# crowsonkb/style_transfer2

Hardware: AMD Instinct MI355X
Metric: style-transfer iters/sec @1024px VGG19 (higher is better)
Workload: dtype f32; 1 GPU; configs[1]: 1024x1024 single image per GPU, VGG19 to conv5_1, content conv4_2 + 5 style layers, adam fp32, 500 iterations per image; jobs=1, parallelism=independent jobs, 1 per GPU, no collective (replicas)

## Files before the change

style_transfer2_amd/csrc/engine.cpp:

```cpp
#include "engine.h"

#include <atomic>

namespace st2e {
static thread_local char g_err[1024] = "";
int fail(int code, const char* fmt, ...)
{
    va_list ap;
    va_start(ap, fmt);
    vsnprintf(g_err, sizeof g_err, fmt, ap);
    va_end(ap);
    return code;
}
const char* const kProfNames[P_COUNT] = {"conv3x3_fwd_mfma_f32", "conv3x3_dgrad_mfma_f32", "maxpool_fwd", "maxpool_bwd",
                                          "gram_partial_mfma_f32", "gram_reduce", "style_grad_mfma_f32", "layer_elem",
                                          "image_pass", "finalize", "vector_ops", "misc", "conv3x3_fwd_wino_f32", "conv3x3_dgrad_wino_f32",
                                          "conv3x3_fwd_mfma_bf16", "conv3x3_dgrad_mfma_bf16", "tile_comm",
                                          "gram_partial_mfma_bf16", "style_grad_mfma_bf16", "conv3x3_fwd_wino_split_bf16x6", "conv3x3_dgrad_wino_split_bf16x6",
                                          "style_grad_fused_in_conv_dgrad_bf16", "avepool_fwd", "avepool_bwd",
                                          "gram_partial_split_bf16x6", "style_grad_split_bf16x6", "avepool_bwd_map16"};

static const struct { int kind; const char* name; int cin, cout; } kVgg19[] = {
    {0, "conv1_1", 3, 64}, {0, "conv1_2", 64, 64}, {1, "pool1", 0, 0},
    {0, "conv2_1", 64, 128}, {0, "conv2_2", 128, 128}, {1, "pool2", 0, 0},
// ... 142 lines not shown
            }
            if (r.pack16) ST_TRY(pack16(c, a.data[i], a.data16[i], C, hw));
            break;
        }
        case F_BY_CONV_BELOW:
            break;
        case F_AVEPOOL: {
            if (!plan[i - 1].out32) return fail(ST_ERR_STATE, "internal: the input blob of average pool %s is not materialised", L.name.c_str());
            ProfScope ps(c, P_AVEPOOL_FWD, 0, 4.0 * n_in + (r.out32 ? 4.0 * C * hw : 0.0) + (r.out16 ? 2.0 * act16_elems(C, hw) : 0.0));
            HIP_TRY(launch_avepool_fwd(a.data[i - 1], r.out32 ? a.data[i] : nullptr, r.out16 ? a.data16[i] : nullptr, C, a.h[i - 1], a.w[i - 1], c->stream));
            break;
        }
        case F_MAXPOOL: {
            { ProfScope ps(c, P_POOL_FWD, 0, 4.0 * n_in * 1.25);
              HIP_TRY(launch_maxpool_fwd(a.data[i - 1], a.data[i], C, a.h[i - 1], a.w[i - 1], c->stream)); }
            if (r.pack16) ST_TRY(pack16(c, a.data[i], a.data16[i], C, hw));
            break;
        }
        case F_NONE:
            return fail(ST_ERR_STATE, "internal: no route for layer %s", L.name.c_str());
        }
    }
    a.valid_to = last;
    return ST_OK;
}

int backward_chain(st_ctx* c, int top, const float* top_diff, const std::vector<const float*>& inj, const float** out, bool lean)
{
    ActSet& a = c->act;
    plan_backward(c, a, top, inj, c->sf_w, lean, a.plan.bwd);
    const std::vector<FwdRoute>& fwd = a.plan.fwd;
    const float* cur = top_diff;
    const unsigned short* cur16 = nullptr;
    if (c->bf16 && !c->diff16A) {
        const size_t cap = c->max_blob + 8 * (size_t)a.h[0] * a.w[0];
        ST_TRY(c->diff16A.alloc(cap)); ST_TRY(c->diff16B.alloc(cap));
    }
    for (int i = top; i >= 1; --i) {
        const Layer& L = c->topo[i - 1];
        const BwdRoute& r = a.plan.bwd[i];
        const int below = i - 1;
        const int Cb = a.C[below], Hb = a.h[below], Wb = a.w[below];
        const int H = a.h[i], W = a.w[i];
        const size_t hw = (size_t)H * W;
        const double px = (double)hw, n_below = (double)Cb * Hb * Wb;
        float* dst = (cur == c->diffA) ? c->diffB : c->diffA;
        const float* inject = inj[below];
        if (r.in16 ? !(cur16 || cur) : !cur) return fail(ST_ERR_STATE, "internal: no %s diff above %s", r.in16 ? "bf16 or fp32" : "fp32", L.name.c_str());
        if (r.pack_in16) {
            unsigned short* tmp16 = (cur16 == c->diff16A) ? c->diff16B : c->diff16A;
            ST_TRY(pack16(c, cur, tmp16, a.C[i], hw));
            cur16 = tmp16;
        }
        unsigned short* dst16 = (cur16 == c->diff16A) ? c->diff16B : c->diff16A;
        if ((r.mask == MASK_F32 || r.kind == B_POOL_CLASSIC) && !fwd[below].out32)
            return fail(ST_ERR_STATE, "internal: blob %d, which the backward of %s reads, is not materialised in fp32", below, L.name.c_str());
        const unsigned char* unpool_amap = r.unpool ? a.amap[i + 1] : nullptr;
        const bool unpool_ave = r.unpool && fwd[i + 1].amap == AMAP_BLOCKED16_AVE;
        const double conv_flops = 2.0 * 9 * L.cin * L.cout * px;
        switch (r.kind) {
        case B_SMALLM16: {
            ProfScope ps(c, P_CONV_DGRAD, conv_flops, px * (2.0 * L.cout + 4.0 * L.cin));
            HIP_TRY(launch_conv3x3_dgrad_smallM16(cur16, L.w_raw_r, dst, inject, L.cout, L.cin, H, W, c->stream));
            break;
        }
        case B_SMALLM: {
            ProfScope ps(c, P_CONV_DGRAD, conv_flops, 4.0 * px * (L.cin + L.cout));
            HIP_TRY(launch_conv3x3_dgrad_smallM(cur, L.w_raw, dst, inject, L.cout, L.cin, H, W, c->stream));
            break;
        }
        case B_CONV16: {
            Conv16Problem p{};
            p.in16 = cur16; p.wpack16 = L.w16_bwd; p.bias = nullptr;
            p.out = r.out32 ? dst : nullptr; p.out16 = r.out16 ? dst16 : nullptr;
            p.inject = inject;
            if (r.mask == MASK_F32) p.mask_src = a.data[below];
            if (r.mask == MASK_BF16) p.mask16 = a.data16[below];
            if (r.mask == MASK_BITS) p.mask_bits = a.bits[below];
            if (r.style) {
                p.s_in16 = c->sf_in[below]; p.s_wpack16 = c->sf_w[below];
                prof_note(c, P_STYLE_FUSED_BF16, 2.0 * L.cin * L.cin * px);
            }
            p.K = L.cout; p.M = L.cin; p.MPad = conv_mpad(L.cin); p.H = H; p.W = W; p.relu = 0;
            p.unpool_amap = unpool_amap;
            p.unpool_ave = unpool_ave;
            const double mask_bytes = r.mask == MASK_BITS ? 0.125 : r.mask == MASK_BF16 ? 2.0 : r.mask == MASK_F32 ? 4.0 : 0.0;
            ProfScope ps(c, P_CONV_DGRAD_BF16, conv_flops,
                         px * ((r.unpool ? 0.75 : 2.0) * L.cout + (r.style ? 2.0 : 0.0) * L.cin + (r.out32 ? 4.0 : 0.0) * L.cin + (r.out16 ? 2.0 : 0.0) * L.cin + mask_bytes * L.cin));
            HIP_TRY(launch_conv3x3_bf16(p, c->stream));
            break;
        }
        case B_WINO: case B_WINO_SPLIT: case B_DIRECT: {
            ConvProblem p{};
            p.in = cur; p.wpack = L.w_bwd; p.bias = nullptr; p.out = dst;
            p.mask_src = r.mask == MASK_F32 ? a.data[below] : nullptr; p.inject = inject;
            p.K = L.cout; p.M = L.cin; p.MPad = conv_mpad(L.cin); p.H = H; p.W = W; p.relu = 0;
            p.unpool_amap = unpool_amap;
            ProfScope ps(c, r.kind == B_WINO_SPLIT ? P_CONV_DGRAD_WSPLIT : r.kind == B_WINO ? P_CONV_DGRAD_WINO : P_CONV_DGRAD, conv_flops,
                         4.0 * px * (L.cin + (r.unpool ? 0.3125 : 1.0) * L.cout));
            if (r.kind == B_WINO_SPLIT) { p.wpack = reinterpret_cast<const float*>(L.us_bwd.get()); ST_TRY(wino_scratch(c, p, wino_split_resolve(p.K, p.M, H, W).splits)); HIP_TRY(launch_conv3x3_wino_split(p, c->stream)); }
            else if (r.kind == B_WINO) { p.wpack = L.u_bwd; ST_TRY(wino_scratch(c, p, wino_resolve(p.K, p.M, H, W).splits)); HIP_TRY(launch_conv3x3_wino(p, c->stream)); }
            else HIP_TRY(launch_conv3x3(p, c->stream));
            break;
        }
        case B_AVEPOOL: {
            ProfScope ps(c, P_AVEPOOL_BWD, 0, 4.0 * (double)Cb * H * W +
                         n_below * (4.0 * ((r.mask != MASK_NONE ? 1 : 0) + (inject ? 1 : 0) + (r.out32 ? 1 : 0)) + (r.out16 ? 2.0 : 0.0)));
            HIP_TRY(launch_avepool_bwd(cur, r.mask != MASK_NONE ? a.data[below] : nullptr, inject, r.out32 ? dst : nullptr, r.out16 ? dst16 : nullptr, Cb, Hb, Wb, c->stream));
            break;
        }
        case B_POOL_IDX16: {
            ProfScope ps(c, P_POOL_BWD, 0, (double)Cb * (hw * 3.0 + (size_t)Hb * Wb * 2.0));
            HIP_TRY(launch_maxpool_bwd_idx16(cur16, a.amap[i], dst16, Cb, Hb, Wb, c->stream));
            break;
        }
        case B_AVEPOOL_MAP16: {
            if (fwd[i].amap != AMAP_BLOCKED16_AVE) return fail(ST_ERR_STATE, "internal: the forward of %s wrote no sign map", L.name.c_str());
            ProfScope ps(c, P_AVEPOOL_BWD_MAP16, 0, (double)Cb * (hw * 3.0 + (size_t)Hb * Wb * 2.0));
            HIP_TRY(launch_avepool_bwd_map16(cur16, a.amap[i], dst16, Cb, Hb, Wb, c->stream));
            break;
        }
        case B_POOL_AMAP: {
            ProfScope ps(c, P_POOL_BWD, 0, (double)Cb * (px * 5.0 + (double)Hb * Wb * 4.0));
            HIP_TRY(launch_maxpool_bwd_amap(cur, a.amap[i], dst, Cb, Hb, Wb, c->stream));
            break;
        }
        case B_POOL_CLASSIC: {
            ProfScope ps(c, P_POOL_BWD, 0, 4.0 * n_below * 2.25);
            HIP_TRY(launch_maxpool_bwd(cur, a.data[below], dst, inject, r.mask != MASK_NONE, Cb, Hb, Wb, c->stream));
            break;
        }
        case B_IN_DGRAD_BELOW:
            continue;
        case B_NONE:
            return fail(ST_ERR_STATE, "internal: no route for the backward of layer %s", L.name.c_str());
        }
        cur = r.out32 ? dst : nullptr;
        cur16 = r.out16 ? dst16 : nullptr;
    }
    if (!cur) return fail(ST_ERR_STATE, "internal: the backward chain ended without an fp32 image gradient");
    *out = cur;
    return ST_OK;
}

int ensure_input_buffers(st_ctx* c, int H, int W)
{
    if (c->H == H && c->W == W && c->x[0]) return ST_OK;
    c->act.valid_to = -1;
    if (c->lt.any) { c->lt.any = false; c->lt.resized = true; }
    const size_t n3 = (size_t)3 * H * W;
    for (int i = 0; i < 2; ++i) ST_TRY(c->x[i].alloc(n3));
    ST_TRY(c->grad.alloc(n3));
    c->m.reset(); c->v.reset();
    ST_TRY(c->m.alloc(n3)); ST_TRY(c->v.alloc(n3));
    c->g_cur.reset(); c->pvec.reset();
    for (int i = 0; i <= st_ctx::kCorr; ++i) { c->hs[i].reset(); c->hy[i].reset(); }
    ST_TRY(c->hwc_dev.alloc(n3));
    c->avg.reset(); c->avg_items = 0;
    if (c->avg_decay > 0) ST_TRY(c->avg.alloc(n3));
    c->H = H; c->W = W; c->cur = 0;
    for (auto& p : c->inject) p.reset();
    std::fill(c->inject_roi_zero.begin(), c->inject_roi_zero.end(), 0);
    c->diffA.reset(); c->diffB.reset(); c->stmp.reset(); c->diff16A.reset(); c->diff16B.reset();
    std::vector<int> C, h, w;
    shapes_for(c, H, W, C, h, w);
    c->max_blob = 0;
    for (int i = 0; i < c->nb; ++i) c->max_blob = std::max(c->max_blob, (size_t)C[i] * h[i] * w[i]);
    return ST_OK;
}

int stage_upload(st_ctx* c, const void* host, size_t bytes)
{
    ST_TRY(c->stage_dev.reserve(bytes));
    HIP_TRY(hipMemcpyAsync(c->stage_dev, host, bytes, hipMemcpyHostToDevice, c->stream));
    return ST_OK;
}

int preprocess_into(st_ctx* c, const void* hwc, int H, int W, int is_u8, float* dst)
{
    if (!hwc || H <= 0 || W <= 0) return fail(ST_ERR_ARG, "bad image (%p, %d x %d)", hwc, H, W);
    const size_t n = (size_t)H * W * 3;
    ST_TRY(stage_upload(c, hwc, n * (is_u8 ? 1 : 4)));
    ProfScope ps(c, P_MISC, 0, 0);
    if (is_u8) HIP_TRY(launch_preprocess_u8(c->stage_dev, dst, H, W, c->stream));
    else HIP_TRY(launch_preprocess_f32((const float*)c->stage_dev.get(), dst, H, W, c->stream));
    return ST_OK;
}

void iterate_overwritten(st_ctx* c)
{
    if (!c->act.data.empty() && c->act.data[0] && (c->act.data[0] == c->x[0] || c->act.data[0] == c->x[1])) c->act.valid_to = -1;
}

int set_input_common(st_ctx* c, int H, int W)
{
    const bool reshaped = !(c->H == H && c->W == W && c->x[0]);
    ST_TRY(ensure_input_buffers(c, H, W));
    if (reshaped) {
        c->m_zero = c->v_zero = true;
        c->lb_clear = true;
        c->have_cur = false;
    }
    return ST_OK;
}
int content_from_device(st_ctx* c, const float* xdev, int H, int W)
{
    ST_TRY(act_ensure(c, c->act, H, W));
    std::vector<char> used(c->nb, 0);
    int deepest = -1;
    for (const ActiveLayer& al : c->active) if (al.c) { used[al.blob] = 1; deepest = std::max(deepest, al.blob); }
    if (deepest > 0) ST_TRY(forward_range(c, c->act, xdev, deepest));
    for (int i = 0; i < c->nb; ++i) {
        if (!used[i]) { c->content_feat[i].reset(); continue; }
        const size_t n = (size_t)c->act.C[i] * c->act.h[i] * c->act.w[i];
        if (c->cH != H || c->cW != W || !c->content_feat[i]) ST_TRY(c->content_feat[i].alloc(n));
        HIP_TRY(hipMemcpyAsync(c->content_feat[i], i == 0 ? xdev : c->act.data[i], n * sizeof(float), hipMemcpyDeviceToDevice, c->stream));
    }
    c->act.valid_to = -1;
    if (xdev != c->content_x) {
        if (c->cH != H || c->cW != W || !c->content_x) ST_TRY(c->content_x.alloc((size_t)3 * H * W));
        HIP_TRY(hipMemcpyAsync(c->content_x, xdev, (size_t)3 * H * W * sizeof(float), hipMemcpyDeviceToDevice, c->stream));
    }
    c->cH = H; c->cW = W;
    c->have_content = true;
    HIP_TRY(hipStreamSynchronize(c->stream));
    return ST_OK;
}

int ensure_content_features(st_ctx* c)
{
    int need = -1;
    for (const ActiveLayer& al : c->active) if (al.c && !c->content_feat[al.blob]) need = std::max(need, al.blob);
    if (need < 0) return ST_OK;
    if (!c->have_content || !c->content_x) return fail(ST_ERR_STATE, "content image missing");
    ST_TRY(act_ensure(c, c->act, c->cH, c->cW));
    if (need > 0) ST_TRY(forward_range(c, c->act, c->content_x, need));
    for (const ActiveLayer& al : c->active) {
        const int b = al.blob;
        if (!al.c || c->content_feat[b]) continue;
        const size_t n = (size_t)c->act.C[b] * c->act.h[b] * c->act.w[b];
        ST_TRY(c->content_feat[b].alloc(n));
        HIP_TRY(hipMemcpyAsync(c->content_feat[b], b == 0 ? c->content_x : c->act.data[b], n * sizeof(float), hipMemcpyDeviceToDevice, c->stream));
    }
    c->act.valid_to = -1;
    return ST_OK;
}
}

extern "C" const char* st_last_error(void) { return st2e::g_err; }

extern "C" {

int st_create(st_ctx** out, int device_id, const st_layer_desc* layers, int n_layers)
{
    if (!out) return fail(ST_ERR_ARG, "out is NULL");
    int ndev = 0;
    HIP_TRY(hipGetDeviceCount(&ndev));
    if (ndev <= 0) return fail(ST_ERR_HIP, "no HIP device visible");
    if (device_id < 0 || device_id >= ndev) return fail(ST_ERR_ARG, "device %d out of range (%d visible)", device_id, ndev);
    HIP_TRY(hipSetDevice(device_id));
    std::unique_ptr<st_ctx, int (*)(st_ctx*)> c(new st_ctx(), st_destroy);
    c->device = device_id;
    c->wino = env_int("ST2_WINO", c->wino) != 0;
    c->graphs = env_int("ST2_GRAPH", c->graphs) != 0;
    { const size_t side = (size_t)env_int("ST2_GRAPH_MAX_PX", 768); c->graph_max_px = side * side; }
    if (n_layers <= 0) {
        for (const auto& l : kVgg19) {
            Layer L; L.is_conv = l.kind == 0; L.name = l.name; L.cin = l.cin; L.cout = l.cout;
            c->topo.push_back(std::move(L));
        }
    } else {
        int cprev = 3;
        for (int i = 0; i < n_layers; ++i) {
            const int kind = layers[i].kind;
            if (kind != ST_LAYER_CONV && kind != ST_LAYER_POOL && kind != ST_LAYER_AVEPOOL)
                return fail(ST_ERR_ARG, "layer %d (%s): unknown kind %d", i, layers[i].name ? layers[i].name : "", kind);
            Layer L; L.is_conv = kind == ST_LAYER_CONV; L.ave = kind == ST_LAYER_AVEPOOL; L.name = layers[i].name ? layers[i].name : "";
            if (L.is_conv) {
                L.cin = layers[i].cin; L.cout = layers[i].cout;
                if (L.cin != cprev || L.cout <= 0) return fail(ST_ERR_ARG, "layer %s: cin %d does not follow %d", L.name.c_str(), L.cin, cprev);
                cprev = L.cout;
            }
            c->topo.push_back(std::move(L));
        }
    }
    if ((int)c->topo.size() + 1 > kMaxTraceLayers) return fail(ST_ERR_ARG, "too many layers");
    c->blob_names.push_back("data");
    for (const Layer& L : c->topo) c->blob_names.push_back(L.name);
    c->nb = (int)c->blob_names.size();
    HIP_TRY(hipStreamCreate(&c->stream));
    c->content_feat.resize(c->nb);
    c->style_gram.resize(c->nb);
    c->style_valid.assign(c->nb, 0);
    c->inject.resize(c->nb);
    c->inject_roi_zero.assign(c->nb, 0);
    c->layer_part.resize(c->nb);
    c->s2_part.resize(c->nb);
    c->sfuse_w.resize(c->nb);
    c->cnt.assign(c->nb * 6, 0);
    c->norm_valid.assign(c->nb * 3, 0);
    ST_TRY(c->norms.alloc(c->nb * 3));
    ST_TRY(c->image_part.alloc(6 * kMaxPartials));
    ST_TRY(c->trace_dev.alloc(kMaxTraceLayers * 6 + 8));
    ST_TRY(c->trace_sums.alloc(kMaxTraceLayers * kLayerSlots + kImageSlots));
    ST_TRY(c->lb_dev.alloc(1));
    HIP_TRY(hipMemset(c->lb_dev, 0, sizeof(LbfgsDev)));
    ST_TRY(c->lb_part.alloc(4 * kMaxPartials));
    ST_TRY(c->trace_host.alloc(kMaxTraceLayers * 6 + 8));
    for (int b = 0; b < c->nb; ++b) c->rows.push_back(ActiveLayer{b, 1.f, 1.f, 1.f, true, true, true});
    c->active = c->rows;
    *out = c.release();
    return ST_OK;
}

int st_destroy(st_ctx* c)
{
    if (!c) return ST_OK;
    (void)hipSetDevice(c->device);
    if (c->stream) (void)hipStreamSynchronize(c->stream);
    if (c->pipe.copy) (void)hipStreamSynchronize(c->pipe.copy);
    for (int i = 0; i < 2; ++i) if (c->gexec[i]) (void)hipGraphExecDestroy(c->gexec[i]);
    for (int i = 0; i < st_ctx::Pipe::kSlots; ++i) {
        if (c->pipe.ready[i]) (void)hipEventDestroy(c->pipe.ready[i]);
        if (c->pipe.done[i]) (void)hipEventDestroy(c->pipe.done[i]);
    }
    for (hipEvent_t e : c->ev_pool) (void)hipEventDestroy(e);
    comm_free(c);
    const hipStream_t stream = c->stream, copy = c->pipe.copy;
    delete c;
    if (copy) (void)hipStreamDestroy(copy);
    if (stream) (void)hipStreamDestroy(stream);
    return ST_OK;
}

static int make_split_packs(Layer& L, const float* w)
{
    for (int dir = 0; dir < 2; ++dir) {
        const int K = dir ? L.cout : L.cin, M = dir ? L.cin : L.cout;
        DevBuf<unsigned short>& dst = dir ? L.us_bwd : L.us_fwd;
        if (dst || !wino_split_resolve(K, M, 4, 4).ok) continue;
        std::vector<unsigned short> hu(wino_split_pack_elems(K, M), 0);
        if (dir) pack_wino_split_weights_dgrad(w, L.cout, L.cin, hu.data()); else pack_wino_split_weights_fwd(w, L.cout, L.cin, hu.data());
        ST_TRY(dst.alloc(hu.size()));
        HIP_TRY(hipMemcpy(dst, hu.data(), hu.size() * 2, hipMemcpyHostToDevice));
    }
    return ST_OK;
}

int st_load_conv_weights(st_ctx* c, const char* layer, const float* w, const float* bias)
{
    if (c) c->epoch++;
    if (!c || !layer || !w) return fail(ST_ERR_ARG, "NULL argument");
    HIP_TRY(hipSetDevice(c->device));
    for (Layer& L : c->topo) {
        if (!L.is_conv || L.name != layer) continue;
        const size_t nf = conv_pack_floats(L.cin, L.cout), nb = conv_pack_floats(L.cout, L.cin);
        std::vector<float> pf(nf), pb(nb), bp(conv_mpad(L.cout), 0.f);
        pack_conv_weights_fwd(w, L.cout, L.cin, pf.data());
        pack_conv_weights_dgrad(w, L.cout, L.cin, pb.data());
        if (bias) memcpy(bp.data(), bias, L.cout * sizeof(float));
        L.loaded = false;
        static_cast<LayerPacks&>(L) = LayerPacks{};
        for (int dir = 0; dir < 2; ++dir) {
            const int K = dir ? L.cout : L.cin, M = dir ? L.cin : L.cout;
            if (!wino_resolve(K, M, 4, 4).ok) continue;
            std::vector<float> hu(wino_pack_floats(K, M));
            if (dir) pack_wino_weights_dgrad(w, L.cout, L.cin, hu.data()); else pack_wino_weights_fwd(w, L.cout, L.cin, hu.data());
            DevBuf<float>& dst = dir ? L.u_bwd : L.u_fwd;
            ST_TRY(dst.alloc(hu.size()));
            HIP_TRY(hipMemcpy(dst, hu.data(), hu.size() * sizeof(float), hipMemcpyHostToDevice));
        }
        {
            const size_t n16f = conv16_pack_elems(L.cin, L.cout), n16b = conv16_pack_elems(L.cout, L.cin);
            std::vector<unsigned short> hf(n16f), hb(n16b);
            pack_conv_weights16_fwd(w, L.cout, L.cin, hf.data());
            pack_conv_weights16_dgrad(w, L.cout, L.cin, hb.data());
            ST_TRY(L.w16_fwd.alloc(n16f)); ST_TRY(L.w16_bwd.alloc(n16b));
            HIP_TRY(hipMemcpy(L.w16_fwd, hf.data(), n16f * 2, hipMemcpyHostToDevice));
            HIP_TRY(hipMemcpy(L.w16_bwd, hb.data(), n16b * 2, hipMemcpyHostToDevice));
        }
        if (L.cin == 3 && L.cout % 32 == 0) {
            std::vector<unsigned short> hs(conv_first_split_pack_elems(L.cout));
            pack_conv_first_split(w, bias, L.cout, L.cin, hs.data());
            ST_TRY(L.w_split.alloc(hs.size()));
            HIP_TRY(hipMemcpy(L.w_split, hs.data(), hs.size() * 2, hipMemcpyHostToDevice));
        }
        ST_TRY(L.w_fwd.alloc(nf)); ST_TRY(L.w_bwd.alloc(nb));
        ST_TRY(L.w_raw.alloc((size_t)L.cout * L.cin * 9)); ST_TRY(L.bias.alloc(bp.size()));
        HIP_TRY(hipMemcpy(L.w_fwd, pf.data(), nf * sizeof(float), hipMemcpyHostToDevice));
        HIP_TRY(hipMemcpy(L.w_bwd, pb.data(), nb * sizeof(float), hipMemcpyHostToDevice));
        HIP_TRY(hipMemcpy(L.w_raw, w, (size_t)L.cout * L.cin * 9 * sizeof(float), hipMemcpyHostToDevice));
        if (conv_dgrad_smallM_ok(L.cout, L.cin) && L.cout % 8 == 0) {
            std::vector<float> wr((size_t)L.cout * L.cin * 9);
            for (size_t k = 0; k < wr.size(); ++k) {
                unsigned u; memcpy(&u, &w[k], 4);
                u = (u + 0x7fffu + ((u >> 16) & 1u)) & 0xffff0000u;
                memcpy(&wr[k], &u, 4);
            }
            ST_TRY(L.w_raw_r.alloc(wr.size()));
            HIP_TRY(hipMemcpy(L.w_raw_r, wr.data(), wr.size() * sizeof(float), hipMemcpyHostToDevice));
        }
        HIP_TRY(hipMemcpy(L.bias, bp.data(), bp.size() * sizeof(float), hipMemcpyHostToDevice));
        if (c->wino_split) ST_TRY(make_split_packs(L, w));
        L.loaded = true;
        return ST_OK;
    }
    return fail(ST_ERR_ARG, "no conv layer named %s", layer);
}

int st_set_conv_algo(st_ctx* c, int winograd)
{
    if (c) c->epoch++;
    if (!c) return fail(ST_ERR_ARG, "ctx is NULL");
    if (winograd < 0 || winograd > 2) return fail(ST_ERR_ARG, "conv algorithm %d: 0 direct, 1 Winograd (fp32 matrix cores), 2 split-operand Winograd (bf16 matrix cores, fp32 results)", winograd);
    c->wino = winograd != 0;
    c->wino_split = winograd == 2;
    if (c->wino_split) {
        HIP_TRY(hipSetDevice(c->device));
        for (Layer& L : c->topo) {
            if (!L.is_conv || !L.loaded || !L.w_raw) continue;
            std::vector<float> w((size_t)L.cout * L.cin * 9);
            HIP_TRY(hipMemcpy(w.data(), L.w_raw, w.size() * sizeof(float), hipMemcpyDeviceToHost));
            ST_TRY(make_split_packs(L, w.data()));
        }
    }
    return ST_OK;
}

int st_set_gram_algo(st_ctx* c, int algo)
{
    if (!c) return fail(ST_ERR_ARG, "ctx is NULL");
    if (algo != 0 && algo != 1) return fail(ST_ERR_ARG, "gram algorithm %d: 0 fp32 matrix cores, 1 split operands (bf16 matrix cores, fp32 results)", algo);
    if (algo == 1) {
        std::vector<int> C, h, w;
        shapes_for(c, 16, 16, C, h, w);
        size_t need = 0;
        for (int i = 0; i < c->nb; ++i) need = std::max(need, style_split_scratch(C[i], 4));
        if (need > c->dsplit.cap()) {
            HIP_TRY(hipSetDevice(c->device));
            DevBuf<unsigned short> p;
            ST_TRY(p.alloc(need));
            HIP_TRY(hipStreamSynchronize(c->stream));
            c->dsplit = std::move(p);
        }
    }
    c->epoch++;
    c->gram_split = algo == 1;
    return ST_OK;
}

int st_set_pool_algo(st_ctx* c, int algo)
{
    if (!c) return fail(ST_ERR_ARG, "ctx is NULL");
    if (algo != 0 && algo != 1) return fail(ST_ERR_ARG, "pool algorithm %d: 0 every average pool a stand-alone pass, 1 fused into the bf16 conv launches around it where a build exists", algo);
    c->epoch++;
    c->pool_algo = algo;
    return ST_OK;
}

int st_get_pool_algo(st_ctx* c, int* algo)
{
    if (!c || !algo) return fail(ST_ERR_ARG, "NULL argument");
    *algo = c->pool_algo;
    return ST_OK;
}

int st_get_algos(st_ctx* c, int* conv, int* gram)
{
    if (!c) return fail(ST_ERR_ARG, "ctx is NULL");
    if (conv) *conv = c->wino_split ? 2 : c->wino ? 1 : 0;
    if (gram) *gram = c->gram_split ? 1 : 0;
    return ST_OK;
}

int st_set_precision(st_ctx* c, int bf16_features)
{
    if (c) c->epoch++;
    if (!c) return fail(ST_ERR_ARG, "ctx is NULL");
    c->bf16 = bf16_features != 0;
    c->lean = bf16_features == 1 && !env_off("ST2_BF16_LEAN");
    return ST_OK;
}

int st_num_blobs(st_ctx* c) { return c ? c->nb : 0; }
const char* st_blob_name(st_ctx* c, int i) { return (c && i >= 0 && i < c->nb) ? c->blob_names[i].c_str() : nullptr; }

int st_blob_shape(st_ctx* c, int index, int H, int W, int* oc, int* oh, int* ow)
{
    if (!c || index < 0 || index >= c->nb) return fail(ST_ERR_ARG, "bad blob index %d", index);
    std::vector<int> C, h, w;
    shapes_for(c, H, W, C, h, w);
    if (oc) *oc = C[index];
    if (oh) *oh = h[index];
    if (ow) *ow = w[index];
    return ST_OK;
}

int st_forward(st_ctx* c, const float* x_nchw, int H, int W, int last_blob)
{
    if (c) c->epoch++;
    if (!c || !x_nchw || H <= 0 || W <= 0) return fail(ST_ERR_ARG, "bad argument");
    HIP_TRY(hipSetDevice(c->device));
    ST_TRY(set_input_common(c, H, W));
    ST_TRY(act_ensure(c, c->act, H, W));
    const size_t n3 = (size_t)3 * H * W;
    ST_TRY(c->fwd_x.reserve(n3));
    HIP_TRY(hipMemcpyAsync(c->fwd_x, x_nchw, n3 * sizeof(float), hipMemcpyHostToDevice, c->stream));
    if (last_blob < 0 || last_blob >= c->nb) last_blob = c->nb - 1;
    ST_TRY(forward_range(c, c->act, c->fwd_x, last_blob));
    HIP_TRY(hipStreamSynchronize(c->stream));
    return ST_OK;
}

int st_get_blob(st_ctx* c, int index, float* out)
{
    if (!c || index < 0 || index >= c->nb || !out) return fail(ST_ERR_ARG, "bad argument");
    if (index > c->act.valid_to) return fail(ST_ERR_STATE, "blob %d was not computed by the last forward", index);
    if (!c->act.plan.fwd[index].out32) return fail(ST_ERR_STATE, "blob %d (%s) is not materialised in fp32 by the lean evaluation of an iteration (st_opfunc / st_forward write every fp32 blob; bf16: st_set_precision(ctx, 2))", index, c->blob_names[index].c_str());
    const size_t n = (size_t)c->act.C[index] * c->act.h[index] * c->act.w[index];
    HIP_TRY(hipMemcpy(out, c->act.data[index], n * sizeof(float), hipMemcpyDeviceToHost));
    return ST_OK;
}

int st_backward(st_ctx* c, int n, const int* blob_index, const float* const* diffs, float* out_grad)
{
    if (c) c->epoch++;
    if (!c || !out_grad || n < 0) return fail(ST_ERR_ARG, "bad argument");
    if (c->act.valid_to < 0) return fail(ST_ERR_STATE, "st_forward first");
    HIP_TRY(hipSetDevice(c->device));
    const size_t n3 = (size_t)3 * c->H * c->W;
    std::vector<const float*> inj(c->nb, nullptr);
    int top = -1;
    for (int i = 0; i < n; ++i) {
        const int b = blob_index[i];
        if (b < 0 || b > c->act.valid_to) return fail(ST_ERR_ARG, "diff for blob %d which the last forward did not reach", b);
        const size_t nb = (size_t)c->act.C[b] * c->act.h[b] * c->act.w[b];
        if (!c->inject[b]) ST_TRY(c->inject[b].alloc(nb));
        HIP_TRY(hipMemcpyAsync(c->inject[b], diffs[i], nb * sizeof(float), hipMemcpyHostToDevice, c->stream));
        c->inject_roi_zero[b] = 0;
        if ((int)c->lt.diff.size() == c->nb) c->lt.diff[b] = LT_OVERWRITTEN;
        inj[b] = c->inject[b];
        top = std::max(top, b);
    }
    if (top < 0) { memset(out_grad, 0, n3 * sizeof(float)); return ST_OK; }
    if (!c->diffA) { ST_TRY(c->diffA.alloc(c->max_blob)); ST_TRY(c->diffB.alloc(c->max_blob)); }
    const float* g = inj[0];
    if (top > 0) ST_TRY(backward_chain(c, top, inj[top], inj, &g));
    HIP_TRY(hipMemcpyAsync(out_grad, g, n3 * sizeof(float), hipMemcpyDeviceToHost, c->stream));
    HIP_TRY(hipStreamSynchronize(c->stream));
    return ST_OK;
}

int st_gram(st_ctx* c, int index, float* out)
{
    if (c) c->epoch++;
    if (!c || index < 0 || index >= c->nb || !out) return fail(ST_ERR_ARG, "bad argument");
    if (index > c->act.valid_to) return fail(ST_ERR_STATE, "blob %d was not computed by the last forward", index);
    if (!c->act.plan.fwd[index].out32) return fail(ST_ERR_STATE, "blob %d (%s) is not materialised in fp32 by the lean evaluation of an iteration: no Gram of it (st_opfunc / st_forward write every fp32 blob; bf16: st_set_precision(ctx, 2))", index, c->blob_names[index].c_str());
    HIP_TRY(hipSetDevice(c->device));
    const int C = c->act.C[index], hw = c->act.h[index] * c->act.w[index];
    DevBuf<float> g;
    ST_TRY(g.alloc((size_t)C * C));
    int r = style_gram(c, c->act, style_term(c, c->act, index, nullptr, true), nullptr, g, C, (double)C * hw, nullptr, nullptr);
    if (r == ST_OK) {
        hipError_t e = hipMemcpyAsync(out, g, (size_t)C * C * sizeof(float), hipMemcpyDeviceToHost, c->stream);
        if (e == hipSuccess) e = hipStreamSynchronize(c->stream);
        if (e != hipSuccess) r = fail(ST_ERR_HIP, "gram copy: %s", hipGetErrorString(e));
    }
    return r;
}

int st_set_input(st_ctx* c, const void* hwc, int H, int W, int is_u8)
{
    if (c) c->epoch++;
    if (!c) return fail(ST_ERR_ARG, "ctx is NULL");
    HIP_TRY(hipSetDevice(c->device));
    ST_TRY(set_input_common(c, H, W));
    iterate_overwritten(c);
    c->avg_items = 0;
    ST_TRY(preprocess_into(c, hwc, H, W, is_u8, c->x[c->cur]));
    HIP_TRY(hipStreamSynchronize(c->stream));
    return ST_OK;
}

int st_set_input_nchw(st_ctx* c, const float* x, int H, int W)
{
    if (c) c->epoch++;
    if (!c || !x || H <= 0 || W <= 0) return fail(ST_ERR_ARG, "bad argument");
    HIP_TRY(hipSetDevice(c->device));
    ST_TRY(set_input_common(c, H, W));
    iterate_overwritten(c);
    c->avg_items = 0;
    HIP_TRY(hipMemcpy(c->x[c->cur], x, (size_t)3 * H * W * sizeof(float), hipMemcpyHostToDevice));
    return ST_OK;
}

int st_get_input_nchw(st_ctx* c, float* out)
{
    if (!c || !out || !c->x[0]) return fail(ST_ERR_STATE, "no input image");
    HIP_TRY(hipStreamSynchronize(c->stream));
    HIP_TRY(hipMemcpy(out, c->x[c->cur], (size_t)3 * c->H * c->W * sizeof(float), hipMemcpyDeviceToHost));
    return ST_OK;
}

int st_input_shape(st_ctx* c, int* H, int* W)
{
    if (!c) return fail(ST_ERR_ARG, "ctx is NULL");
// ... 132 lines not shown
```

style_transfer2_amd/csrc/engine.h:

```cpp
#pragma once
#include "../../include/st2.h"
#include "st2_kernels.h"
#include "env.h"
#include "devbuf.h"

#include <hip/hip_runtime.h>
#include <math.h>
#include <stdarg.h>
#include <stdio.h>
#include <string.h>

#include <algorithm>
#include <memory>
#include <string>
#include <vector>

namespace st2e {
using namespace st2;

int fail(int code, const char* fmt, ...);
#define HIP_TRY(expr)                                                                               \
    do {                                                                                            \
        hipError_t e_ = (expr);                                                                     \
        if (e_ != hipSuccess)                                                                       \
            return st2e::fail(ST_ERR_HIP, "%s failed: %s (%s:%d)", #expr, hipGetErrorString(e_), __FILE__, __LINE__); \
    } while (0)
#define ST_TRY(expr)                    \
    do {                                \
        int r_ = (expr);                \
        if (r_ != ST_OK) return r_;     \
    } while (0)

enum ProfClass { P_CONV_FWD, P_CONV_DGRAD, P_POOL_FWD, P_POOL_BWD, P_GRAM, P_GRAM_REDUCE, P_STYLE_GRAD,
                 P_LAYER_ELEM, P_IMAGE_PASS, P_FINALIZE, P_VECTOR, P_MISC, P_CONV_FWD_WINO, P_CONV_DGRAD_WINO,
                 P_CONV_FWD_BF16, P_CONV_DGRAD_BF16, P_COMM, P_GRAM_BF16, P_STYLE_GRAD_BF16, P_CONV_FWD_WSPLIT, P_CONV_DGRAD_WSPLIT, P_STYLE_FUSED_BF16,
                 P_AVEPOOL_FWD, P_AVEPOOL_BWD, P_GRAM_SPLIT, P_STYLE_GRAD_SPLIT, P_AVEPOOL_BWD_MAP16, P_COUNT };
extern const char* const kProfNames[P_COUNT];
struct ProfRec { int cls; hipEvent_t a, b; double flops, bytes; };

struct LayerPacks {
    DevBuf<float> w_fwd, w_bwd, w_raw, w_raw_r, bias;
    DevBuf<unsigned short> w16_fwd, w16_bwd;
    DevBuf<unsigned short> w_split;
    DevBuf<float> u_fwd, u_bwd;
    DevBuf<unsigned short> us_fwd, us_bwd;
};
struct Layer : LayerPacks {
    bool is_conv = false;
    bool ave = false;
    std::string name;
    int cin = 0, cout = 0;
    bool loaded = false;
};

enum FwdKind : unsigned char { F_NONE, F_CONV16, F_WINO, F_WINO_SPLIT, F_DIRECT, F_FIRST_SPLIT, F_MAXPOOL, F_AVEPOOL,
                               F_BY_CONV_BELOW };
enum AmapLayout : unsigned char { AMAP_NONE, AMAP_BLOCKED16,
                                  AMAP_PLANAR32,
                                  AMAP_BLOCKED16_AVE };
enum BwdKind : unsigned char { B_NONE, B_SMALLM, B_SMALLM16, B_CONV16, B_WINO, B_WINO_SPLIT, B_DIRECT, B_AVEPOOL, B_POOL_IDX16,
                               B_POOL_AMAP, B_POOL_CLASSIC,
                               B_IN_DGRAD_BELOW,
                               B_AVEPOOL_MAP16 };
enum MaskSrc : unsigned char { MASK_NONE, MASK_F32, MASK_BF16, MASK_BITS };

struct FwdRoute {
    FwdKind kind = F_NONE;
    bool out32 = false, out16 = false, bits = false;
    AmapLayout amap = AMAP_NONE;
    bool pack16 = false;
    bool pools_next = false;
    bool style16 = false;
    bool style_all16 = false;
};
struct BwdRoute {
    BwdKind kind = B_NONE;
    bool in16 = false;
    bool pack_in16 = false;
    bool out32 = false, out16 = false;
    MaskSrc mask = MASK_NONE;
    bool unpool = false;
    bool style = false;
};
struct RoutePlan { std::vector<FwdRoute> fwd; std::vector<BwdRoute> bwd; };

struct ActSet {
    int H = 0, W = 0;
    std::vector<int> C, h, w;
    std::vector<DevBuf<float>> own;
    std::vector<float*> data;
    std::vector<DevBuf<unsigned short>> data16;
    std::vector<DevBuf<unsigned char>> amap;
    std::vector<DevBuf<unsigned short>> bits;
    RoutePlan plan;
    int valid_to = -1;
};

struct ActiveLayer { int blob; float cw, sw, dw; bool c, s, d; };

inline bool nonzero(float w) { return fabsf(w) > 1e-15f; }

struct TileGeom { int gH = 0, gW = 0, wy0 = 0, wx0 = 0, ty0 = 0, tx0 = 0, ty1 = 0, tx1 = 0; };
struct BlobRoi { int y0, x0, y1, x1; double n_global; };
struct BlobSize { int h, w, stride; double n; };

struct ObjTerm {
    ActiveLayer al; int b, C;
    size_t n;
    double n_norm;
    BlobRoi roi; bool has_roi;
    size_t sums;
    size_t gram;
    int k;
    const BlobRoi* region() const { return has_roi ? &roi : nullptr; }
};
constexpr size_t kNoSlot = ~(size_t)0;
struct ObjTerms { std::vector<ObjTerm> t; int last = -1; size_t n1 = 0; int n_style = 0; };

struct StyleShape { bool grad16, gram16; };
enum StyleOps : unsigned char { OPS_F32, OPS_SPLIT, OPS_BF16,
                                OPS_FUSED };
struct StyleLaunch { StyleOps ops; int cls; double flops, bytes; };
struct StyleTerm {
    int b, C, hw;
    bool roi; GramRoi groi; PixRoi proi;
    StyleLaunch gram, grad, pack;
    GramPlan plan;
    int slots;
    size_t d16, sfuse;
    bool reads32, reads16, missing32;
    bool book;
};

enum LtDiff : char { LT_NONE, LT_WRITTEN, LT_RODE_ON_CONV, LT_OVERWRITTEN };
struct LayerTerms {
    bool any = false;
    bool resized = false;
    int style_blob = -1;
    int raw_blob = -1;
    std::vector<size_t> n;
    std::vector<int> C;
    std::vector<char> diff;
    std::vector<char> norm_ok;
    void begin(int nb) { any = resized = false; style_blob = raw_blob = -1; n.assign(nb, 0); C.assign(nb, 0); diff.assign(nb, LT_NONE); norm_ok.assign((size_t)nb * 3, 0); }
};
}

using namespace st2e;

struct st_ctx {
    int device = 0;
    hipStream_t stream = nullptr;
    bool bf16 = false;
    bool lean = false;
    bool in_step = false;
    bool wino = true;
    bool wino_split = false;
    int pool_algo = 0;
    bool gram_split = false;
    DevBuf<unsigned short> dsplit;
    DevBuf<unsigned short> diff16A, diff16B;
    std::vector<Layer> topo;
    std::vector<std::string> blob_names;
    int nb = 0;

    ActSet act;
    int H = 0, W = 0;
    DevBuf<float> x[2];
    int cur = 0;
    DevBuf<float> fwd_x;
    DevBuf<float> grad;
    int cH = 0, cW = 0;
    std::vector<DevBuf<float>> content_feat;
    DevBuf<float> content_x;
    std::vector<DevBuf<float>> style_gram;
    std::vector<char> style_valid;
    bool have_content = false, have_style = false;
    std::vector<ActiveLayer> rows;
    std::vector<ActiveLayer> active;
    float tv_w = 1, tv_pow = 1, p_w = 1, p_pow = 1;
    DevBuf<float> norms;
    std::vector<char> norm_valid;
    std::vector<DevBuf<float>> inject;
    std::vector<char> inject_roi_zero;
    DevBuf<float> diffA, diffB, stmp;
    size_t max_blob = 0;
    DevBuf<float> gram_slabs, gram_fold, dbuf;
    DevBuf<unsigned short> d16;
    std::vector<DevBuf<unsigned short>> sfuse_w;
    std::vector<const unsigned short*> sf_in, sf_w;
    LayerTerms lt;
    DevBuf<float> conv_scratch;
    unsigned long long epoch = 0;
    hipGraphExec_t gexec[2] = {nullptr, nullptr};
    unsigned long long gepoch[2] = {0, 0};
    DevBuf<float> adam_dyn;
    bool capturing = false, graphs = false;
    int plain_steps = 0;
    unsigned long long plain_epoch = ~0ull;
    size_t graph_max_px = 768 * 768;
    long long graph_replays = 0;
    std::vector<DevBuf<float>> layer_part;
    std::vector<DevBuf<float>> s2_part;
    std::vector<int> cnt;
    DevBuf<float> image_part;
    int image_cnt = 0;
    DevBuf<float> trace_dev;
    DevBuf<double> trace_sums;
    PinBuf<float> trace_host;
    int trace_len_last = 8;
    DevBuf<float> hwc_dev;
    struct Pipe {
        static constexpr int kSlots = 6;
        hipStream_t copy = nullptr;
        DevBuf<float> hwc[kSlots]; float* img_pin[kSlots] = {}; PinBuf<float> trace_pin[kSlots];
        PinBuf<char> pin_base[kSlots];
        hipEvent_t ready[kSlots] = {}, done[kSlots] = {};
        size_t cap = 0; long long head = 0; int count = 0, tlen[kSlots] = {}, H[kSlots] = {}, W[kSlots] = {};
        size_t want_head = 0, want_tail = 0, have_head = 0, have_tail = 0;
        struct Retired { PinBuf<char> buf; long long at; };
        std::vector<Retired> retired;
        long long begins = 0;
    } pipe;
    DevBuf<unsigned char> stage_dev;
    int opt_kind = ST_OPT_NONE;
    double step_size = 1.0;
    DevBuf<float> m, v;
    int items1 = 0, items2 = 0;
    bool m_zero = true, v_zero = true;
    static const int kCorr = kLbfgsCorr;
    DevBuf<float> hs[kLbfgsSlots];
    DevBuf<float> hy[kLbfgsSlots];
    DevBuf<LbfgsDev> lb_dev;
    bool lb_clear = true;
    DevBuf<float> lb_part;
    DevBuf<LbfgsGram> lb_gram;
    DevBuf<float> lb_gpart;
    DevBuf<float> lb_dots;
    bool lb_gram_form = false;
    DevBuf<float> g_cur, pvec;
    bool have_cur = false;
    float last_loss = 0.f;
    DevBuf<float> avg;
    double avg_decay = 0.0;
    int avg_items = 0;
    bool orig_colors = false;
    int style_match = 0;
    float xf_A[9] = {1, 0, 0, 0, 1, 0, 0, 0, 1}, xf_b[3] = {0, 0, 0};
    DevBuf<double> mom_part, mom_out;
    struct Tile : TileGeom {
        bool on = false;
        DevBuf<float> p1, p2, p3, pd;
        bool s2_in_p2 = false;
        bool evaluated = false;
        DevBuf<float> wgrad;
        bool fused = false;
        DevBuf<float> lb_x, lb_sums;
        DevBuf<float> sp; int sp_n = 0, sp_last = -1, sp_gH = 0, sp_gW = 0;
    } tile;
    struct Comm {
        void* lib = nullptr;
        void* comm = nullptr;
        int rank = 0, world = 1;
        bool set = false;
        st_allreduce_fn ar = nullptr; st_exchange_fn ex = nullptr; void* user = nullptr;
        struct Peer { int peer = 0; std::vector<int> send, recv; DevBuf<float> sbuf, rbuf; size_t sn = 0, rn = 0; };
        std::vector<Peer> plan[3];
        bool planned[3] = {false, false, false};
        bool self_via_rccl = false;
        DevBuf<float> ring;
        long long steps = 0;
        std::vector<float> h1, h2, h3, hd, hn;
        DevBuf<float> tile_chw, tile_hwc;
        DevBuf<float> tile_cx;
    } comm;
    bool prof_on = false;
    std::vector<ProfRec> prof;
    std::vector<hipEvent_t> ev_pool;
    size_t ev_used = 0;

    int blob_c(int i) const { return act.C[i]; }
    int blob_c_topo(int i) const
    {
        for (int k = i; k >= 1; --k) if (topo[k - 1].is_conv) return topo[k - 1].cout;
        return 3;
    }
};

namespace st2e {
inline size_t act16_elems(int C, size_t hw) { return (size_t)((C + 7) / 8) * hw * 8; }
inline bool conv16_ok(const st_ctx* c, int K) { (void)c; return K >= 8 && K % 8 == 0; }
int wino_scratch(st_ctx* c, ConvProblem& p, int splits);

struct ProfScope {
    st_ctx* c; int idx = -1;
    ProfScope(st_ctx* ctx, int cls, double flops, double bytes, bool book = true) : c(ctx)
    {
        if (!c->prof_on || !book) return;
        auto get = [&]() {
            if (c->ev_used == c->ev_pool.size()) {
                hipEvent_t e;
                (void)hipEventCreate(&e);
                c->ev_pool.push_back(e);
            }
            return c->ev_pool[c->ev_used++];
        };
        ProfRec r{cls, get(), get(), flops, bytes};
        (void)hipEventRecord(r.a, c->stream);
        c->prof.push_back(r);
        idx = (int)c->prof.size() - 1;
    }
    ~ProfScope()
    {
        if (idx >= 0) (void)hipEventRecord(c->prof[idx].b, c->stream);
    }
};

inline void prof_note(st_ctx* c, int cls, double flops)
{
    if (!c->prof_on) return;
    if (c->ev_used == c->ev_pool.size()) { hipEvent_t e; (void)hipEventCreate(&e); c->ev_pool.push_back(e); }
    hipEvent_t e = c->ev_pool[c->ev_used++];
    (void)hipEventRecord(e, c->stream);
    c->prof.push_back(ProfRec{cls, e, e, flops, 0.0});
}

void shapes_for(const st_ctx* c, int H, int W, std::vector<int>& C, std::vector<int>& h, std::vector<int>& w);
int act_ensure(st_ctx* c, ActSet& a, int H, int W);
int forward_range(st_ctx* c, ActSet& a, const float* x, int last, bool lean = false);
int backward_chain(st_ctx* c, int top, const float* top_diff, const std::vector<const float*>& inj, const float** out, bool lean = false);
int ensure_input_buffers(st_ctx* c, int H, int W);
int stage_upload(st_ctx* c, const void* host, size_t bytes);
int preprocess_into(st_ctx* c, const void* hwc, int H, int W, int is_u8, float* dst);
int set_input_common(st_ctx* c, int H, int W);
void iterate_overwritten(st_ctx* c);
int content_from_device(st_ctx* c, const float* xdev, int H, int W);
int style_from_device(st_ctx* c, const float* xdev, int H, int W);
int ensure_content_features(st_ctx* c);
void plan_forward(const st_ctx* c, const ActSet& a, int last, bool lean, std::vector<FwdRoute>& fwd);
void plan_backward(const st_ctx* c, const ActSet& a, int top, const std::vector<const float*>& inj,
                   const std::vector<const unsigned short*>& fused_w, bool lean, std::vector<BwdRoute>& bwd);
bool lean32_enabled();
StyleShape style_shape(const st_ctx* c, const ActSet& a, int b);
StyleTerm style_term(const st_ctx* c, const ActSet& a, int b, const BlobRoi* roi = nullptr, bool target = false, int fuse_last = -1);
size_t style_split_scratch(int C, int hw);
int style_gram(st_ctx* c, const ActSet& a, const StyleTerm& t, const float* target, float* out, int out_ld, double divisor, float* partial, int* n_partial);
int style_grad(st_ctx* c, const ActSet& a, const StyleTerm& t, float* dst, float c2, int fused, float sw, int accumulate, int* np);
int ensure_dbuf(st_ctx* c);
int ensure_layer_part(st_ctx* c, int b);
LayerElemArgs layer_elem_args(const st_ctx* c, const ActiveLayer& al, double n_norm, int write, float* part, const BlobRoi* roi = nullptr);
int objective_terms(const st_ctx* c, const ActSet& a, const TileGeom* tile, ObjTerms& terms);
BlobSize blob_size(const st_ctx* c, int b, int gH, int gW);
BlobRoi tile_roi(const st_ctx* c, const ActSet& a, const TileGeom& t, int b);
ImagePassArgs image_pass_args(const st_ctx* c, const float* x, const float* scd, float* grad, bool adam, float* x_next);
int eval_objective(st_ctx* c, const float* x, bool want_grad, float* grad_out, bool adam, float* x_next);
int read_trace(st_ctx* c, double* trace, float* loss);
int lbfgs_alloc(st_ctx* c);
LbfgsArgs lbfgs_args(st_ctx* c, int apply);
int lbfgs_clear_history(st_ctx* c, bool gram_form);
float average_corr(const st_ctx* c);
int emit_preflight(const st_ctx* c, int reader, bool want_image, EmitPlan* plan);
int emit_enqueue(st_ctx* c, const EmitPlan& plan, float* hwc, const float* staged_v, const float* staged_cx, int h, int w);
int style_color_check(const st_ctx* c);
int style_recolor_enqueue(st_ctx* c, float* x, int H, int W);
int strips(st_ctx* c, float* tensor, int C, int h, int w, const std::vector<int>& rects, float* buf, int mode);
void comm_free(st_ctx* c);
int comm_allreduce(st_ctx* c, float* buf, int n);
}
```

style_transfer2_amd/csrc/engine_objective.cpp:

```cpp
#include "engine.h"

namespace st2e {
int objective_terms(const st_ctx* c, const ActSet& a, const TileGeom* tile, ObjTerms& terms)
{
    terms = ObjTerms{};
    if (!c->active.empty() && ((int)a.C.size() != c->nb || a.H != c->H || a.W != c->W))
        return fail(ST_ERR_STATE, "no forward of the current input has sized the activations");
    size_t pos = 0;
    for (const ActiveLayer& al : c->active) {
        if (al.c && (!c->have_content || c->cH != c->H || c->cW != c->W))
            return fail(ST_ERR_STATE, "content features missing or of a different size than the input");
        if (al.s && !c->have_style) return fail(ST_ERR_STATE, "style Gram matrices missing");
        if (al.s && !c->style_valid[al.blob])
            return fail(ST_ERR_STATE, "blob %d (%s) carries a style weight but has no style target: the sharded style pass (st_tile_set_style) stopped below it", al.blob, c->blob_names[al.blob].c_str());
        ObjTerm t{};
        t.al = al; t.b = al.blob; t.C = a.C[t.b];
        t.n = (size_t)t.C * a.h[t.b] * a.w[t.b];
        t.has_roi = tile != nullptr;
        t.roi = tile ? tile_roi(c, a, *tile, t.b) : BlobRoi{0, 0, a.h[t.b], a.w[t.b], (double)t.n};
        t.n_norm = t.roi.n_global;
        t.sums = pos;
        pos += 4;
        t.gram = kNoSlot; t.k = -1;
        if (al.s) { t.gram = pos; pos += (size_t)t.C * t.C; t.k = terms.n_style++; }
        terms.last = std::max(terms.last, t.b);
        terms.t.push_back(t);
    }
    terms.n1 = pos;
    return ST_OK;
}

ImagePassArgs image_pass_args(const st_ctx* c, const float* x, const float* scd, float* grad, bool adam, float* x_next)
{
    ImagePassArgs ip{};
    ip.x = x; ip.scd = scd; ip.grad = grad;
    ip.C = 3; ip.H = c->H; ip.W = c->W;
    ip.tv_w = c->tv_w; ip.tv_beta = c->tv_pow; ip.p_w = c->p_w; ip.p_pow = c->p_pow;
    ip.partial = c->image_part;
    if (adam) {
        ip.x_out = x_next; ip.m = c->m; ip.v = c->v;
        ip.d1 = (float)0.9; ip.c1 = (float)(1 - 0.9); ip.d2 = (float)0.999; ip.c2 = (float)(1 - 0.999);
        ip.corr1 = (float)(1 - pow(0.9, c->items1)); ip.corr2 = (float)(1 - pow(0.999, c->items2));
        ip.step = (float)c->step_size;
        ip.m_is_zero = c->m_zero; ip.v_is_zero = c->v_zero;
        if (c->capturing) ip.dyn = c->adam_dyn;
    }
    return ip;
}

int eval_objective(st_ctx* c, const float* x, bool want_grad, float* grad_out, bool adam, float* x_next)
{
    if (!c->x[0]) return fail(ST_ERR_STATE, "no input image");
    ST_TRY(act_ensure(c, c->act, c->H, c->W));
    ActSet& a = c->act;
    ObjTerms terms;
    ST_TRY(objective_terms(c, a, nullptr, terms));
    const int last = std::max(terms.last, 0);
    const bool lean = c->bf16 && c->lean && !c->tile.on;
    bool lean32 = false;
    if (!c->bf16 && c->in_step && !c->tile.on) lean32 = lean32_enabled();
    ST_TRY(ensure_content_features(c));
    ST_TRY(forward_range(c, a, x, last, lean || lean32));

    std::vector<const float*> inj(c->nb, nullptr);
    std::fill(c->cnt.begin(), c->cnt.end(), 0);
    c->sf_in.assign(c->nb, nullptr); c->sf_w.assign(c->nb, nullptr);
    c->lt.begin(c->nb);
    for (const ObjTerm& ot : terms.t) {
        const ActiveLayer& al = ot.al;
        const int b = ot.b, C = ot.C;
        const size_t n = ot.n;
        if (!c->inject[b]) ST_TRY(c->inject[b].alloc(n));
        c->inject_roi_zero[b] = 0;
        ST_TRY(ensure_layer_part(c, b));
        float* part = c->layer_part[b];
        float* nrm = c->norms + b * 3;
        int* cnt = &c->cnt[b * 6];
        bool wrote = false;
        if (al.c || al.d) {
            LayerElemArgs e = layer_elem_args(c, al, (double)n, 1, part);
            const bool need_norm = (al.c && !c->norm_valid[b * 3 + 0]) || (al.d && !c->norm_valid[b * 3 + 2]);
            int np = 0;
            if (need_norm) {
                e.write = 0;
                { ProfScope ps(c, P_LAYER_ELEM, 0, 4.0 * n * (al.c ? 2 : 1)); HIP_TRY(launch_layer_elem(e, &np, c->stream)); }
                ProfScope ps(c, P_FINALIZE, 0, 0);
                if (al.c && !c->norm_valid[b * 3 + 0]) { HIP_TRY(launch_finalize_norm(e.part_gc2, np, (double)n, nrm + 0, c->stream)); c->norm_valid[b * 3 + 0] = 1; }
                if (al.d && !c->norm_valid[b * 3 + 2]) { HIP_TRY(launch_finalize_norm(e.part_gd2, np, (double)n, nrm + 2, c->stream)); c->norm_valid[b * 3 + 2] = 1; }
            }
            e.write = 1;
            { ProfScope ps(c, P_LAYER_ELEM, 0, 4.0 * n * (al.c ? 3 : 2)); HIP_TRY(launch_layer_elem(e, &np, c->stream)); }
            cnt[0] = cnt[1] = cnt[2] = cnt[3] = np;
            wrote = true;
        }
        if (al.s) {
            ST_TRY(ensure_dbuf(c));
            const StyleTerm t = style_term(c, a, b, nullptr, false, want_grad ? last : -1);
            ST_TRY(style_gram(c, a, t, c->style_gram[b], c->dbuf, conv_mpad(C), (double)n, part + 4 * kMaxPartials, &cnt[4]));
            const float c2 = (float)(2.0 / ((double)C * C * (double)n));
            if (c->norm_valid[b * 3 + 1]) {
                ST_TRY(style_grad(c, a, t, c->inject[b], c2, 1, al.sw, wrote, &cnt[5]));
            } else {
                if (!c->stmp) ST_TRY(c->stmp.alloc(c->max_blob));
                ST_TRY(style_grad(c, a, t, c->stmp, c2, 0, al.sw, 0, &cnt[5]));
                { ProfScope ps(c, P_FINALIZE, 0, 0);
                  HIP_TRY(launch_finalize_norm(c->s2_part[b], cnt[5], (double)n, nrm + 1, c->stream)); }
                c->norm_valid[b * 3 + 1] = 1;
                ProfScope ps(c, P_VECTOR, 0, 4.0 * n * 3);
                HIP_TRY(launch_scaled_accumulate(c->stmp, c->inject[b], al.sw, nrm + 1, wrote, n, c->stream));
                c->lt.raw_blob = b;
            }
            c->lt.style_blob = b;
            if (c->lt.raw_blob != b) c->lt.raw_blob = -1;
        }
        c->lt.n[b] = n; c->lt.C[b] = C;
        c->lt.diff[b] = c->sf_w[b] ? LT_RODE_ON_CONV : LT_WRITTEN;
        for (int k = 0; k < 3; ++k) c->lt.norm_ok[b * 3 + k] = c->norm_valid[b * 3 + k];
        inj[b] = (c->sf_w[b] && !wrote) ? nullptr : c->inject[b];
    }

    const float* scd = nullptr;
    if (want_grad && !c->active.empty()) {
        if (!c->diffA) { ST_TRY(c->diffA.alloc(c->max_blob)); ST_TRY(c->diffB.alloc(c->max_blob)); }
        if (last == 0) scd = inj[0];
        else {
            std::vector<const float*> below = inj;
            const int rc = backward_chain(c, last, inj[last], below, &scd, lean);
            c->sf_in.assign(c->nb, nullptr); c->sf_w.assign(c->nb, nullptr);
            ST_TRY(rc);
        }
    }

    {
        const ImagePassArgs ip = image_pass_args(c, x, scd, want_grad ? grad_out : nullptr, adam, x_next);
        const double n3 = 3.0 * c->H * c->W;
        ProfScope ps(c, P_IMAGE_PASS, 0, 4.0 * n3 * (adam ? 7 : 3));
        HIP_TRY(launch_image_pass(ip, &c->image_cnt, c->stream));
    }

    {
        TraceArgs t{};
        t.n_layers = (int)terms.t.size();
        for (int l = 0; l < t.n_layers; ++l) {
            const ActiveLayer& al = terms.t[l].al;
            const int b = al.blob;
            TraceLayer& L = t.layer[l];
            L.content = al.c; L.style = al.s; L.deepdream = al.d;
            L.cw = al.cw; L.sw = al.sw; L.dw = al.dw;
            L.n = (double)terms.t[l].n;
            L.gram_n = (double)a.C[b] * a.C[b];
            for (int k = 0; k < 5; ++k) { L.part[k] = c->layer_part[b] + k * kMaxPartials; L.count[k] = c->cnt[b * 6 + k]; }
            L.part[5] = c->s2_part[b]; L.count[5] = c->cnt[b * 6 + 5];
            L.norm = c->norms + b * 3;
        }
        t.image_part = c->image_part; t.image_count = c->image_cnt; t.image_n = 3.0 * c->H * c->W;
        t.tv_w = c->tv_w; t.p_w = c->p_w; t.p_pow = c->p_pow; t.have_grad = want_grad;
        t.out = c->trace_dev;
        t.sums = c->trace_sums;
        c->trace_len_last = t.n_layers * 6 + 8;
        ProfScope ps(c, P_FINALIZE, 0, 0);
        HIP_TRY(launch_finalize_trace(t, c->stream));
    }
    c->lt.any = true;
    return ST_OK;
}

int read_trace(st_ctx* c, double* trace, float* loss)
{
    const int n = c->trace_len_last;
    HIP_TRY(hipMemcpyAsync(c->trace_host, c->trace_dev, n * sizeof(float), hipMemcpyDeviceToHost, c->stream));
    HIP_TRY(hipStreamSynchronize(c->stream));
    if (trace) for (int i = 0; i < n; ++i) trace[i] = c->trace_host[i];
    c->last_loss = c->trace_host[n - 2];
    if (loss) *loss = c->last_loss;
    return ST_OK;
}
}

extern "C" {

int st_set_weights(st_ctx* c, int n_rows, const int* blob_index, const float* content, const float* style,
                   const float* deepdream, const double params[4])
{
    if (c) c->epoch++;
    if (!c || n_rows < 0 || (n_rows && (!blob_index || !content || !style || !deepdream)) || !params)
        return fail(ST_ERR_ARG, "bad argument");
    std::vector<ActiveLayer> rows;
    for (int i = 0; i < n_rows; ++i) {
        const int b = blob_index[i];
        if (b < 0 || b >= c->nb) return fail(ST_ERR_ARG, "row %d names blob %d", i, b);
        rows.push_back(ActiveLayer{b, content[i], style[i], deepdream[i], nonzero(content[i]), nonzero(style[i]), nonzero(deepdream[i])});
    }
    c->rows = rows;
    c->active.clear();
    for (const ActiveLayer& r : rows) if (r.c || r.s || r.d) c->active.push_back(r);
    c->tile.evaluated = false;
    c->tv_w = (float)params[0]; c->tv_pow = (float)params[1]; c->p_w = (float)params[2]; c->p_pow = (float)params[3];
    if (c->have_content) {
        std::vector<char> used(c->nb, 0);
        for (const ActiveLayer& al : c->active) if (al.c) used[al.blob] = 1;
        HIP_TRY(hipSetDevice(c->device));
        HIP_TRY(hipStreamSynchronize(c->stream));
        for (int b = 0; b < c->nb; ++b) if (!used[b]) c->content_feat[b].reset();
    }
    return ST_OK;
}

int st_clear_norms(st_ctx* c)
{
    if (c) c->epoch++;
    if (!c) return fail(ST_ERR_ARG, "ctx is NULL");
    std::fill(c->norm_valid.begin(), c->norm_valid.end(), 0);
    return ST_OK;
}

int st_get_layer_terms(st_ctx* c, int index, float* D, float* raw_S, float* diff, float norms[3])
{
    if (!c || index < 0 || index >= c->nb) return fail(ST_ERR_ARG, "bad argument");
    const LayerTerms& lt = c->lt;
    const char* name = c->blob_names[index].c_str();
    if (!lt.any)
        return fail(ST_ERR_STATE, lt.resized ? "the iterate was resized after the last evaluation: its work buffers are gone; evaluate again"
                                             : "no objective evaluation has completed on this context");
    if (!lt.n[index]) return fail(ST_ERR_STATE, "blob %d (%s) carried no weight in the last evaluation", index, name);
    if ((D || raw_S) && lt.style_blob != index) {
        if (lt.style_blob < 0) return fail(ST_ERR_STATE, "the last evaluation had no style term: no D and no style gradient of blob %d (%s)", index, name);
        return fail(ST_ERR_STATE, "D and the unscaled style gradient are one buffer each for all layers: they hold those of blob %d (%s), the style layer evaluated last, not of blob %d (%s)",
                    lt.style_blob, c->blob_names[lt.style_blob].c_str(), index, name);
    }
    if (raw_S && lt.raw_blob != index)
        return fail(ST_ERR_STATE, "the last evaluation of blob %d (%s) knew its style norm and scaled the gradient in the kernel's epilogue: the unscaled one exists only after the first evaluation since reset() / st_clear_norms", index, name);
    if (diff && lt.diff[index] == LT_RODE_ON_CONV)
        return fail(ST_ERR_STATE, "the style term of blob %d (%s) rode on the data-gradient conv above it: nothing was written into its diff (ST2_STYLE_FUSE=0, or an evaluation without gradient, materialises it)", index, name);
    if (diff && lt.diff[index] == LT_OVERWRITTEN)
        return fail(ST_ERR_STATE, "st_backward has overwritten the diff of blob %d (%s) since the last evaluation", index, name);
    if (diff && (lt.diff[index] != LT_WRITTEN || !c->inject[index])) return fail(ST_ERR_STATE, "blob %d (%s) has no diff of the last evaluation", index, name);
    if ((D && !c->dbuf) || (raw_S && !c->stmp)) return fail(ST_ERR_STATE, "internal: the buffer of blob %d (%s) is gone", index, name);
    HIP_TRY(hipSetDevice(c->device));
    HIP_TRY(hipStreamSynchronize(c->stream));
    const size_t C = (size_t)lt.C[index], n = lt.n[index];
    if (D) HIP_TRY(hipMemcpy2D(D, C * sizeof(float), c->dbuf, (size_t)conv_mpad((int)C) * sizeof(float), C * sizeof(float), C, hipMemcpyDeviceToHost));
    if (raw_S) HIP_TRY(hipMemcpy(raw_S, c->stmp, n * sizeof(float), hipMemcpyDeviceToHost));
    if (diff) HIP_TRY(hipMemcpy(diff, c->inject[index], n * sizeof(float), hipMemcpyDeviceToHost));
    if (norms) {
        HIP_TRY(hipMemcpy(norms, c->norms + index * 3, 3 * sizeof(float), hipMemcpyDeviceToHost));
        for (int k = 0; k < 3; ++k) if (!lt.norm_ok[index * 3 + k]) norms[k] = 0.f;
    }
    return ST_OK;
}

int st_trace_len(st_ctx* c) { return c ? (int)c->active.size() * 6 + 8 : 0; }

int st_opfunc(st_ctx* c, float* out_loss, float* out_grad, double* trace)
{
    if (c) c->epoch++;
    if (!c) return fail(ST_ERR_ARG, "ctx is NULL");
    HIP_TRY(hipSetDevice(c->device));
    ST_TRY(eval_objective(c, c->x[c->cur], out_grad != nullptr, c->grad, false, nullptr));
    if (out_grad) HIP_TRY(hipMemcpyAsync(out_grad, c->grad, (size_t)3 * c->H * c->W * sizeof(float), hipMemcpyDeviceToHost, c->stream));
    return read_trace(c, trace, out_loss);
}

}
```

style_transfer2_amd/csrc/engine_style.cpp:

```cpp
#include "engine.h"

namespace st2e {
StyleShape style_shape(const st_ctx* c, const ActSet& a, int b)
{
    StyleShape s{};
    if (!c->bf16 || b < 1 || !c->topo[b - 1].is_conv) return s;
    const int C = a.C[b], hw = a.h[b] * a.w[b];
    s.grad16 = conv16_ok(c, C) && style_grad16_ok(C, (size_t)hw);
    s.gram16 = s.grad16 && (c->tile.on ? !env_off("ST2_TILE_STYLE16") : hw % 64 == 0 && gram16_ok(C, hw, gram_plan16(C, hw)));
    return s;
}

size_t style_split_scratch(int C, int hw) { return gram_split_ok(C, hw) && style_grad_split_ok(C, hw) ? style_grad_split_pack_elems(C) : 0; }

static bool style_fuse_ok(const st_ctx* c, const ActSet& a, int b, int last)
{
    if (env_off("ST2_STYLE_FUSE") || b + 1 > last || a.C[b] % 32 != 0) return false;
    const Layer& up = c->topo[b];
    return up.is_conv && up.loaded && conv16_ok(c, up.cout) && up.cin == a.C[b];
}

StyleTerm style_term(const st_ctx* c, const ActSet& a, int b, const BlobRoi* roi, bool target, int fuse_last)
{
    const FwdRoute& fr = a.plan.fwd[b];
    StyleTerm t{};
    const int C = t.C = a.C[b];
    t.b = b; t.roi = roi != nullptr; t.book = target || !roi;
    const size_t plane = (size_t)a.h[b] * a.w[b];
    if (roi) { t.groi = GramRoi{roi->y0, roi->x0, roi->x1 - roi->x0, a.w[b], plane}; t.proi = PixRoi{roi->y0, roi->x0, roi->y1, roi->x1}; }
    const int hw = t.hw = roi ? t.groi.rw * (roi->y1 - roi->y0) : (int)plane;
    const bool may16 = !target && (roi || !c->tile.on);
    const bool gram16 = may16 && fr.style_all16, grad16 = may16 && (roi ? fr.style_all16 : fr.style16);
    const size_t split_elems = style_split_scratch(C, hw);
    const bool split = c->gram_split && !c->bf16 && !c->tile.on && !roi && split_elems > 0;
    const double fl = 2.0 * C * C * (double)hw, n = (double)C * hw;
    t.plan = gram16 ? gram_plan16(C, hw) : gram_plan(C, hw);
    t.gram = gram16 ? StyleLaunch{OPS_BF16, P_GRAM_BF16, fl, 2.0 * C * (double)hw}
             : StyleLaunch{split ? OPS_SPLIT : OPS_F32, split ? P_GRAM_SPLIT : P_GRAM, fl, 4.0 * C * (double)hw};
    if (gram16 && fuse_last >= 0 && c->norm_valid[b * 3 + 1] && style_fuse_ok(c, a, b, fuse_last)) {
        t.sfuse = style_fuse_pack_elems(C, conv_mpad(C));
        t.pack = StyleLaunch{OPS_FUSED, P_MISC, 0, 4.0 * C * C + 2.0 * t.sfuse};
        t.grad = StyleLaunch{OPS_FUSED, P_STYLE_GRAD, 2.0 * C * C * (double)C, 12.0 * C * C};
        t.slots = style_s2_trace_blocks(C);
    } else if (grad16) {
        t.grad = StyleLaunch{OPS_BF16, P_STYLE_GRAD_BF16, fl, n * 6.0};
        t.slots = style_grad16_blocks(C, (size_t)hw);
    } else if (split && split_elems <= c->dsplit.cap()) {
        t.grad = StyleLaunch{OPS_SPLIT, P_STYLE_GRAD_SPLIT, fl, n * 8.0};
        t.slots = style_grad_split_blocks(C, hw);
    } else {
        t.grad = StyleLaunch{OPS_F32, P_STYLE_GRAD, fl, n * 8.0};
        t.slots = style_grad_blocks(C, a.h[b], a.w[b]);
    }
    if (grad16) t.d16 = style_grad16_pack_elems(C);
    t.reads16 = grad16; t.reads32 = !gram16 || !grad16; t.missing32 = t.reads32 && !fr.out32;
    return t;
}

static int missing_copy(const StyleTerm& t) { return fail(ST_ERR_STATE, t.roi ? "internal: style blob %d has no fp32 copy" : "internal: style blob %d has neither an fp32 nor a usable bf16 copy", t.b); }

int style_gram(st_ctx* c, const ActSet& a, const StyleTerm& t, const float* target, float* out, int out_ld, double divisor, float* partial, int* n_partial)
{
    if (t.missing32) return missing_copy(t);
    const int b = t.b, C = t.C;
    const GramRoi* roi = t.roi ? &t.groi : nullptr;
    ST_TRY(c->gram_slabs.reserve(t.plan.slab_floats));
    ST_TRY(c->gram_fold.reserve((size_t)gram_fold_groups(t.plan) * C * C));
    {
        ProfScope ps(c, t.gram.cls, t.gram.flops, t.gram.bytes, t.book);
        if (t.gram.ops == OPS_BF16) HIP_TRY(launch_gram16_partial(a.data16[b], c->gram_slabs, C, t.hw, t.plan, c->stream, roi));
        else if (t.gram.ops == OPS_SPLIT) HIP_TRY(launch_gram_split_partial(a.data[b], c->gram_slabs, C, t.hw, t.plan, c->stream));
        else HIP_TRY(launch_gram_partial(a.data[b], c->gram_slabs, C, t.hw, t.plan, c->stream, roi));
    }
    ProfScope ps(c, P_GRAM_REDUCE, 0, 4.0 * (double)t.plan.slab_floats, t.book);
    HIP_TRY(launch_gram_reduce(c->gram_slabs, c->gram_fold, target, out, out_ld, partial, n_partial, C, divisor, t.plan, c->stream));
    return ST_OK;
}

int style_grad(st_ctx* c, const ActSet& a, const StyleTerm& t, float* dst, float c2, int fused, float sw, int accumulate, int* np)
{
    if (t.missing32) return missing_copy(t);
    const int b = t.b, C = t.C, ld = conv_mpad(C);
    const float* norm = c->norms + b * 3 + 1;
    ST_TRY(c->s2_part[b].reserve(t.slots));
    if (t.d16) ST_TRY(c->d16.reserve(t.d16));
    float* part = c->s2_part[b];
    if (t.grad.ops == OPS_FUSED) {
        ST_TRY(c->sfuse_w[b].reserve(t.sfuse));
        { ProfScope ps(c, t.pack.cls, t.pack.flops, t.pack.bytes, t.book);
          HIP_TRY(launch_style_fuse_pack(c->dbuf, ld, C, ld, c2, sw, norm, c->sfuse_w[b], c->stream)); }
        ProfScope ps(c, t.grad.cls, t.grad.flops, t.grad.bytes, t.book);
        HIP_TRY(launch_style_s2_trace(c->dbuf, ld, c->style_gram[b], C, (double)C * t.hw, c2, part, np, c->stream));
        c->sf_in[b] = a.data16[b]; c->sf_w[b] = c->sfuse_w[b];
        return ST_OK;
    }
    if (t.roi && t.grad.ops == OPS_BF16 && dst == c->inject[b] && !accumulate && !c->inject_roi_zero[b]) {
        HIP_TRY(hipMemsetAsync(dst, 0, (size_t)C * t.groi.plane * sizeof(float), c->stream));
        c->inject_roi_zero[b] = 1;
    }
    ProfScope ps(c, t.grad.cls, t.grad.flops, t.grad.bytes, t.book);
    if (t.grad.ops == OPS_SPLIT) HIP_TRY(launch_style_grad_split(c->dbuf, ld, c->dsplit, a.data[b], dst, c2, fused, sw, norm, accumulate, part, np, C, t.hw, c->stream));
    else if (t.grad.ops == OPS_BF16) HIP_TRY(launch_style_grad16(c->dbuf, ld, c->d16, a.data16[b], dst, c2, fused, sw, norm, accumulate, part, np, C, (size_t)t.hw, c->stream, t.roi ? &t.groi : nullptr));
    else HIP_TRY(launch_style_grad(c->dbuf, a.data[b], dst, c2, fused, sw, norm, accumulate, part, np, C, a.h[b], a.w[b], c->stream, t.roi ? &t.proi : nullptr));
    return ST_OK;
}

int ensure_dbuf(st_ctx* c)
{
    if (c->dbuf) return ST_OK;
    size_t cc = 1;
    for (int i = 0; i < c->nb; ++i) cc = std::max(cc, (size_t)c->act.C[i] * conv_mpad(c->act.C[i]));
    ST_TRY(c->dbuf.alloc(cc));
    HIP_TRY(hipMemsetAsync(c->dbuf, 0, cc * sizeof(float), c->stream));
    return ST_OK;
}

int ensure_layer_part(st_ctx* c, int b) { return c->layer_part[b] ? ST_OK : c->layer_part[b].alloc(5 * kMaxPartials); }

LayerElemArgs layer_elem_args(const st_ctx* c, const ActiveLayer& al, double n_norm, int write, float* part, const BlobRoi* roi)
{
    const ActSet& a = c->act;
    const int b = al.blob;
    float* nrm = c->norms + b * 3;
    LayerElemArgs e{};
    e.feat = a.data[b]; e.target = al.c ? c->content_feat[b].get() : nullptr; e.inject = c->inject[b];
    e.n = (size_t)a.C[b] * a.h[b] * a.w[b]; e.cn_coef = (float)(2.0 / n_norm); e.dn_coef = (float)(-2.0 / n_norm);
    e.cw = al.cw; e.dw = al.dw; e.content = al.c; e.deepdream = al.d; e.write = write;
    e.norm_c = nrm + 0; e.norm_d = nrm + 2;
    if (part) { e.part_d2 = part; e.part_gc2 = part + kMaxPartials; e.part_f2 = part + 2 * kMaxPartials; e.part_gd2 = part + 3 * kMaxPartials; }
    if (roi) { e.h = a.h[b]; e.w = a.w[b]; e.ry0 = roi->y0; e.rx0 = roi->x0; e.ry1 = roi->y1; e.rx1 = roi->x1; }
    return e;
}
}
```

style_transfer2_amd/csrc/engine_tile.cpp:

```cpp
#include "engine.h"

namespace st2e {
BlobSize blob_size(const st_ctx* c, int b, int gH, int gW)
{
    int s = 1, gh = gH, gw = gW;
    for (int i = 1; i <= b; ++i)
        if (!c->topo[i - 1].is_conv) { gh = pooled_size(gh); gw = pooled_size(gw); s *= 2; }
    return BlobSize{gh, gw, s, (double)c->blob_c_topo(b) * gh * gw};
}

BlobRoi tile_roi(const st_ctx* c, const ActSet& a, const TileGeom& t, int b)
{
    const BlobSize g = blob_size(c, b, t.gH, t.gW);
    const int s = g.stride;
    BlobRoi r;
    r.y0 = (t.ty0 - t.wy0) / s; r.x0 = (t.tx0 - t.wx0) / s;
    r.y1 = t.ty1 == t.gH ? a.h[b] : (t.ty1 - t.wy0) / s;
    r.x1 = t.tx1 == t.gW ? a.w[b] : (t.tx1 - t.wx0) / s;
    r.n_global = g.n;
    return r;
}

int tile_style_D(st_ctx* c, int b, const float* graw, double n_global, float* pd_slot)
{
    const ActSet& a = c->act;
    const int C = a.C[b];
    ST_TRY(ensure_layer_part(c, b));
    float* part = c->layer_part[b] + 4 * kMaxPartials;
    int np = 0;
    GramPlan one{}; one.splits = 1;
    HIP_TRY(launch_gram_reduce(graw, nullptr, c->style_gram[b], c->dbuf, conv_mpad(C), part, &np, C, n_global, one, c->stream));
    HIP_TRY(launch_sum_partials(part, np, pd_slot, c->stream));
    return ST_OK;
}

static int tile_sync(st_ctx* c)
{
    if (!c->tile.fused) HIP_TRY(hipStreamSynchronize(c->stream));
    return ST_OK;
}

static int tile_begin(st_ctx* c, ObjTerms& terms)
{
    if (c) c->epoch++;
    if (!c || !c->tile.on) return fail(ST_ERR_STATE, "st_tile_configure first");
    HIP_TRY(hipSetDevice(c->device));
    ST_TRY(act_ensure(c, c->act, c->H, c->W));
    return objective_terms(c, c->act, &c->tile, terms);
}

static int tile_image_pass(st_ctx* c, const float* ring_dev, bool adam, float** dev_ptr, int* n_floats)
{
    HIP_TRY(hipSetDevice(c->device));
    ObjTerms terms;
    ST_TRY(objective_terms(c, c->act, &c->tile, terms));
    const st_ctx::Tile& t = c->tile;
    ST_TRY(c->tile.p3.reserve(6 + kMaxTraceLayers));
    if (adam) { c->items1 += 1; c->items2 += 1; }
    ImageTileArgs ta{};
    ta.base = image_pass_args(c, c->x[c->cur], c->tile.wgrad, adam ? nullptr : c->grad.get(), adam, c->x[c->cur ^ 1]);
    ta.ring = ring_dev; ta.ty = t.ty0 - t.wy0; ta.tx = t.tx0 - t.wx0; ta.th = t.ty1 - t.ty0; ta.tw = t.tx1 - t.tx0;
    if (adam) HIP_TRY(hipMemcpyAsync(c->x[c->cur ^ 1], c->x[c->cur], (size_t)3 * c->H * c->W * sizeof(float), hipMemcpyDeviceToDevice, c->stream));
    int np = 0;
    HIP_TRY(launch_image_pass_tile(ta, &np, c->stream));
    for (int k = 0; k < 6; ++k) HIP_TRY(launch_sum_partials(c->image_part + k * kMaxPartials, np, c->tile.p3 + k, c->stream));
    if (adam) c->m_zero = c->v_zero = false;
    ST_TRY(tile_sync(c));
    c->tile.evaluated = true;
    if (dev_ptr) *dev_ptr = c->tile.p3;
    if (n_floats) *n_floats = 6 + (c->tile.s2_in_p2 ? 0 : terms.n_style);
    return ST_OK;
}

int strips(st_ctx* c, float* tensor, int C, int h, int w, const std::vector<int>& rects, float* buf, int mode)
{
    const int n = (int)rects.size() / 4;
    size_t off = 0;
    for (int r0 = 0; r0 < n; r0 += kMaxStripRects) {
        StripTable t{};
        t.n = std::min(kMaxStripRects, n - r0);
        int total = 0;
        for (int r = 0; r < t.n; ++r) {
            const int* q = &rects[4 * (r0 + r)];
            t.y0[r] = q[0]; t.x0[r] = q[1]; t.h[r] = q[2]; t.w[r] = q[3];
            if (q[0] < 0 || q[1] < 0 || q[2] <= 0 || q[3] <= 0 || q[0] + q[2] > h || q[1] + q[3] > w)
                return fail(ST_ERR_ARG, "strip %d lies outside the %dx%d tensor", r0 + r, h, w);
            t.off[r] = total;
            total += C * q[2] * q[3];
        }
        t.total = total;
        HIP_TRY(launch_strip_copy(tensor, buf + off, t, C, h, w, mode, c->stream));
        off += (size_t)total;
    }
    return ST_OK;
}
}

extern "C" {

int st_tile_configure(st_ctx* c, int gH, int gW, int wy0, int wx0, int ty0, int tx0, int ty1, int tx1)
{
    if (c) c->epoch++;
    if (c)
        for (const Layer& L : c->topo)
            if (L.ave) return fail(ST_ERR_ARG, "tile-sharded mode does not run average pools (layer %s); use a single-context job", L.name.c_str());
    if (!c || !c->x[0]) return fail(ST_ERR_STATE, "set the window image first (st_set_input)");
    if (wy0 < 0 || wx0 < 0 || wy0 + c->H > gH || wx0 + c->W > gW || ty0 < wy0 || tx0 < wx0 ||
        ty1 > wy0 + c->H || tx1 > wx0 + c->W || ty1 <= ty0 || tx1 <= tx0)
        return fail(ST_ERR_ARG, "tile/window geometry is inconsistent with the %dx%d window", c->H, c->W);
    st_ctx::Tile& t = c->tile;
    t.on = true; t.gH = gH; t.gW = gW; t.wy0 = wy0; t.wx0 = wx0; t.ty0 = ty0; t.tx0 = tx0; t.ty1 = ty1; t.tx1 = tx1;
    t.evaluated = false;
    return ST_OK;
}

int st_tile_forward(st_ctx* c, float** dev_ptr, int* n_floats)
{
    ObjTerms terms;
    ST_TRY(tile_begin(c, terms));
    ActSet& a = c->act;
    c->tile.evaluated = false;
    c->lt.begin(c->nb);
    ST_TRY(ensure_content_features(c));
    ST_TRY(c->tile.p1.reserve(std::max<size_t>(terms.n1, 1)));
    HIP_TRY(hipMemsetAsync(c->tile.p1, 0, std::max<size_t>(terms.n1, 1) * sizeof(float), c->stream));
    bool lean32 = false;
    if (!c->bf16 && c->tile.fused) lean32 = lean32_enabled();
    ST_TRY(forward_range(c, a, c->x[c->cur], std::max(terms.last, 0), (c->bf16 && c->lean) || lean32));
    for (const ObjTerm& t : terms.t) {
        ST_TRY(ensure_layer_part(c, t.b));
        float* part = c->layer_part[t.b];
        if (t.al.c || t.al.d) {
            int np = 0;
            HIP_TRY(launch_layer_elem(layer_elem_args(c, t.al, t.n_norm, 0, part, t.region()), &np, c->stream));
            for (int k = 0; k < 4; ++k) HIP_TRY(launch_sum_partials(part + k * kMaxPartials, np, c->tile.p1 + t.sums + k, c->stream));
        }
        if (t.al.s) ST_TRY(style_gram(c, a, style_term(c, a, t.b, t.region()), nullptr, c->tile.p1 + t.gram, t.C, 1.0, nullptr, nullptr));
    }
    if (dev_ptr) *dev_ptr = c->tile.p1;
    if (n_floats) *n_floats = (int)terms.n1;
    return ST_OK;
}

int st_tile_losses(st_ctx* c, float** dev_ptr, int* n_floats)
{
    ObjTerms terms;
    ST_TRY(tile_begin(c, terms));
    bool missing = false;
    for (const ObjTerm& t : terms.t) if (t.al.s) missing = missing || !c->norm_valid[t.b * 3 + 1];
    ST_TRY(c->tile.p2.reserve(std::max(terms.n_style, 1)));
    ST_TRY(c->tile.pd.reserve(std::max(terms.n_style, 1)));
    c->tile.s2_in_p2 = missing;
    ST_TRY(ensure_dbuf(c));
    for (const ObjTerm& t : terms.t) {
        const int b = t.b;
        const float* sums = c->tile.p1 + t.sums;
        float* nrm = c->norms + b * 3;
        if (t.al.c && !c->norm_valid[b * 3 + 0]) { HIP_TRY(launch_finalize_norm(sums + 1, 1, t.n_norm, nrm + 0, c->stream)); c->norm_valid[b * 3 + 0] = 1; }
        if (t.al.d && !c->norm_valid[b * 3 + 2]) { HIP_TRY(launch_finalize_norm(sums + 3, 1, t.n_norm, nrm + 2, c->stream)); c->norm_valid[b * 3 + 2] = 1; }
    }
    if (dev_ptr) *dev_ptr = missing ? c->tile.p2 : nullptr;
    if (n_floats) *n_floats = missing ? terms.n_style : 0;
    return ST_OK;
}

int st_tile_losses_finish(st_ctx* c)
{
    ObjTerms terms;
    ST_TRY(tile_begin(c, terms));
    ActSet& a = c->act;
    const bool two_step = c->tile.s2_in_p2;
    if ((int)c->lt.n.size() != c->nb) c->lt.begin(c->nb);
    for (const ObjTerm& t : terms.t) {
        const ActiveLayer& al = t.al;
        const int b = t.b, C = t.C;
        if (!c->inject[b]) ST_TRY(c->inject[b].alloc(t.n));
        float* nrm = c->norms + b * 3;
        bool wrote = false;
        if (al.c || al.d) {
            int np = 0;
            HIP_TRY(launch_layer_elem(layer_elem_args(c, al, t.n_norm, 1, nullptr, t.region()), &np, c->stream));
            wrote = true;
        }
        if (al.s) {
            ST_TRY(tile_style_D(c, b, c->tile.p1 + t.gram, t.n_norm, c->tile.pd + t.k));
            const float c2 = (float)(2.0 / ((double)C * C * t.n_norm));
            int np = 0;
            if (two_step && !c->norm_valid[b * 3 + 1]) {
                HIP_TRY(launch_finalize_norm(c->tile.p2 + t.k, 1, t.n_norm, nrm + 1, c->stream));
                c->norm_valid[b * 3 + 1] = 1;
            }
            ST_TRY(style_grad(c, a, style_term(c, a, b, t.region()), c->inject[b], c2, 1, al.sw, wrote, &np));
            if (!two_step) {
                ST_TRY(c->tile.p3.reserve(6 + kMaxTraceLayers));
                HIP_TRY(launch_sum_partials(c->s2_part[b], np, c->tile.p3 + 6 + t.k, c->stream));
            }
            c->lt.style_blob = b;
            if (c->lt.raw_blob != b) c->lt.raw_blob = -1;
        }
        c->lt.n[b] = t.n; c->lt.C[b] = C; c->lt.diff[b] = LT_WRITTEN;
        for (int k = 0; k < 3; ++k) c->lt.norm_ok[b * 3 + k] = c->norm_valid[b * 3 + k];
    }
    c->lt.any = true;
    return ST_OK;
}

int st_tile_style_raw(st_ctx* c)
{
    ObjTerms terms;
    ST_TRY(tile_begin(c, terms));
    ActSet& a = c->act;
    for (const ObjTerm& t : terms.t) {
        if (!t.al.s) continue;
        ST_TRY(tile_style_D(c, t.b, c->tile.p1 + t.gram, t.n_norm, c->tile.pd + t.k));
        const float c2 = (float)(2.0 / ((double)t.C * t.C * t.n_norm));
        if (!c->stmp) ST_TRY(c->stmp.alloc(c->max_blob));
        int np = 0;
        ST_TRY(style_grad(c, a, style_term(c, a, t.b, t.region()), c->stmp, c2, 0, t.al.sw, 0, &np));
        HIP_TRY(launch_sum_partials(c->s2_part[t.b], np, c->tile.p2 + t.k, c->stream));
        c->lt.style_blob = c->lt.raw_blob = t.b;
    }
    return ST_OK;
}

int st_tile_backward(st_ctx* c, float** dev_grad)
{
    ObjTerms terms;
    ST_TRY(tile_begin(c, terms));
    const size_t n3 = (size_t)3 * c->H * c->W;
    if (!c->tile.wgrad) ST_TRY(c->tile.wgrad.alloc(n3));
    std::vector<const float*> inj(c->nb, nullptr);
    const int last = terms.last;
    for (const ObjTerm& t : terms.t) inj[t.b] = c->inject[t.b];
    if (last < 0) HIP_TRY(hipMemsetAsync(c->tile.wgrad, 0, n3 * sizeof(float), c->stream));
    else {
        if (!c->diffA) { ST_TRY(c->diffA.alloc(c->max_blob)); ST_TRY(c->diffB.alloc(c->max_blob)); }
        const float* g = inj[0];
        if (last > 0) ST_TRY(backward_chain(c, last, inj[last], inj, &g, c->bf16 && c->lean));
        HIP_TRY(hipMemcpyAsync(c->tile.wgrad, g, n3 * sizeof(float), hipMemcpyDeviceToDevice, c->stream));
    }
    ST_TRY(tile_sync(c));
    if (dev_grad) *dev_grad = c->tile.wgrad;
    return ST_OK;
}

int st_tile_update(st_ctx* c, const float* ring_dev, float** dev_ptr, int* n_floats)
{
    if (c) c->epoch++;
    if (!c || !c->tile.on || !ring_dev) return fail(ST_ERR_STATE, "st_tile_configure first");
    if (c->opt_kind != ST_OPT_ADAM) return fail(ST_ERR_STATE, "the tile-sharded mode implements Adam");
    return tile_image_pass(c, ring_dev, true, dev_ptr, n_floats);
}

int st_tile_gradient(st_ctx* c, const float* ring_dev, float** dev_ptr, int* n_floats)
{
    if (c) c->epoch++;
    if (!c || !c->tile.on || !ring_dev) return fail(ST_ERR_STATE, "st_tile_configure first");
    return tile_image_pass(c, ring_dev, false, dev_ptr, n_floats);
}

int st_vec_dot(st_ctx* c, const float* a_dev, const float* b_dev, long long n, float* out_dev)
{
    if (!c || !a_dev || !b_dev || !out_dev || n < 0) return fail(ST_ERR_ARG, "bad argument");
    HIP_TRY(hipSetDevice(c->device));
    HIP_TRY(launch_vec_dot(a_dev, b_dev, (size_t)n, c->image_part, out_dev, c->stream));
    ST_TRY(tile_sync(c));
    return ST_OK;
}

int st_vec_axpy(st_ctx* c, float alpha, const float* x_dev, float* y_dev, long long n)
{
    if (!c || !x_dev || !y_dev || n < 0) return fail(ST_ERR_ARG, "bad argument");
    HIP_TRY(hipSetDevice(c->device));
    HIP_TRY(launch_vec_axpy(alpha, x_dev, y_dev, (size_t)n, c->stream));
    ST_TRY(tile_sync(c));
    return ST_OK;
}

int st_vec_div(st_ctx* c, double divisor, float* y_dev, long long n)
{
    if (!c || !y_dev || n < 0 || !(divisor != 0.0)) return fail(ST_ERR_ARG, "bad argument");
    HIP_TRY(hipSetDevice(c->device));
    HIP_TRY(launch_vec_div(divisor, y_dev, (size_t)n, c->stream));
    ST_TRY(tile_sync(c));
    return ST_OK;
}

int st_tile_buffer(st_ctx* c, int which, float** dev_ptr)
{
    if (c) c->epoch++;
    if (!c || !dev_ptr) return fail(ST_ERR_ARG, "bad argument");
    ST_TRY(tile_sync(c));
    if (which == 0) *dev_ptr = c->x[c->cur];
    else if (which == 1) *dev_ptr = c->x[c->cur ^ 1];
    else if (which == 2) *dev_ptr = c->tile.pd;
    else if (which == 3) *dev_ptr = c->norms;
    else if (which == 4) *dev_ptr = c->grad;
    else return fail(ST_ERR_ARG, "unknown buffer %d", which);
    return ST_OK;
}

int st_tile_strips(st_ctx* c, void* tensor_dev, int C, int wh, int ww, int n, const int* rects, void* buf_dev, int mode)
{
    if (!c || !tensor_dev || !buf_dev || n < 0 || n > kMaxStripRects || (n && !rects) || mode < 0 || mode > 2) return fail(ST_ERR_ARG, "bad argument");
    HIP_TRY(hipSetDevice(c->device));
    ST_TRY(strips(c, (float*)tensor_dev, C, wh, ww, std::vector<int>(rects, rects + 4 * n), (float*)buf_dev, mode));
    ST_TRY(tile_sync(c));
    return ST_OK;
}

int st_tile_style_partials(st_ctx* c, const void* hwc, int H, int W, int is_u8, int gH, int gW, int wy0, int wx0, int ty0, int tx0, int ty1, int tx1,
                           int last_blob, float** dev_ptr, int* n_floats)
{
    if (c) c->epoch++;
    if (!c) return fail(ST_ERR_ARG, "ctx is NULL");
    if (last_blob < 0 || last_blob >= c->nb) return fail(ST_ERR_ARG, "last_blob %d is not a blob of this net (0 .. %d)", last_blob, c->nb - 1);
    if (gH <= 0 || gW <= 0) return fail(ST_ERR_ARG, "bad style image size %d x %d", gH, gW);
    for (int i = 0; i < last_blob; ++i)
        if (c->topo[i].ave) return fail(ST_ERR_ARG, "tile-sharded mode does not run average pools (layer %s); use st_set_style", c->topo[i].name.c_str());
    const int stride = blob_size(c, last_blob, gH, gW).stride;
    if (hwc) {
        if (H <= 0 || W <= 0 || wy0 < 0 || wx0 < 0 || wy0 + H > gH || wx0 + W > gW || ty0 < wy0 || tx0 < wx0 || ty1 > wy0 + H || tx1 > wx0 + W ||
            ty1 <= ty0 || tx1 <= tx0)
            return fail(ST_ERR_ARG, "style tile/window geometry is inconsistent with the %dx%d window of the %dx%d style image", H, W, gH, gW);
        if (wy0 % stride || wx0 % stride || ty0 % stride || tx0 % stride || (ty1 != gH && ty1 % stride) || (tx1 != gW && tx1 % stride))
            return fail(ST_ERR_ARG, "style tile/window edges must be multiples of the total stride %d of blob %d (or the image's far edge)", stride, last_blob);
    }
    HIP_TRY(hipSetDevice(c->device));
    size_t total = 0;
    for (int b = 0; b <= last_blob; ++b) { const size_t C = c->blob_c_topo(b); total += C * C; }
    if (hwc) ST_TRY(style_color_check(c));
    if (total > 0x7fffffffu) return fail(ST_ERR_ARG, "the style partials exceed 2^31 floats");
    c->tile.sp_last = -1;
    ST_TRY(c->tile.sp.reserve(total));
    HIP_TRY(hipMemsetAsync(c->tile.sp, 0, total * sizeof(float), c->stream));
    int r = ST_OK;
    if (hwc) {
        DevBuf<float> tmp;
        ST_TRY(tmp.alloc((size_t)3 * H * W));
        ActSet aux;
        ActSet* a = &aux;
        const bool same = c->act.H == H && c->act.W == W && !c->act.data.empty();
        if (same) a = &c->act;
        r = preprocess_into(c, hwc, H, W, is_u8, tmp);
        if (r == ST_OK && c->style_match) r = style_recolor_enqueue(c, tmp, H, W);
        if (r == ST_OK) r = act_ensure(c, *a, H, W);
        if (r == ST_OK) r = forward_range(c, *a, tmp, last_blob);
        TileGeom g;
        g.gH = gH; g.gW = gW; g.wy0 = wy0; g.wx0 = wx0; g.ty0 = ty0; g.tx0 = tx0; g.ty1 = ty1; g.tx1 = tx1;
        size_t pos = 0;
        for (int b = 0; b <= last_blob && r == ST_OK; ++b) {
            const int C = a->C[b];
            const BlobRoi roi = tile_roi(c, *a, g, b);
            const int rw = roi.x1 - roi.x0, rh = roi.y1 - roi.y0;
            if (roi.y0 < 0 || roi.x0 < 0 || roi.y1 > a->h[b] || roi.x1 > a->w[b] || rw <= 0 || rh <= 0) {
                r = fail(ST_ERR_ARG, "the style tile has no region in blob %d of its window", b);
                break;
            }
            r = style_gram(c, *a, style_term(c, *a, b, &roi, true), nullptr, c->tile.sp + pos, C, 1.0, nullptr, nullptr);
            pos += (size_t)C * C;
        }
        (void)hipStreamSynchronize(c->stream);
        if (same) c->act.valid_to = -1;
    } else {
        HIP_TRY(hipStreamSynchronize(c->stream));
    }
    if (r != ST_OK) return r;
    c->tile.sp_n = (int)total; c->tile.sp_last = last_blob; c->tile.sp_gH = gH; c->tile.sp_gW = gW;
    if (dev_ptr) *dev_ptr = c->tile.sp;
    if (n_floats) *n_floats = (int)total;
    return ST_OK;
}

int st_tile_style_commit(st_ctx* c)
{
    if (c) c->epoch++;
    if (!c) return fail(ST_ERR_ARG, "ctx is NULL");
    if (c->tile.sp_last < 0 || !c->tile.sp) return fail(ST_ERR_STATE, "st_tile_style_partials first");
    HIP_TRY(hipSetDevice(c->device));
    size_t pos = 0;
    GramPlan one{}; one.bt = 128; one.splits = 1;
    for (int b = 0; b <= c->tile.sp_last; ++b) {
        const int C = c->blob_c_topo(b);
        if (!c->style_gram[b]) ST_TRY(c->style_gram[b].alloc((size_t)C * C));
        ProfScope ps(c, P_GRAM_REDUCE, 0, 8.0 * C * C);
        HIP_TRY(launch_gram_reduce(c->tile.sp + pos, nullptr, nullptr, c->style_gram[b], C, nullptr, nullptr, C, blob_size(c, b, c->tile.sp_gH, c->tile.sp_gW).n, one, c->stream));
        pos += (size_t)C * C;
    }
    HIP_TRY(hipStreamSynchronize(c->stream));
    for (int b = 0; b < c->nb; ++b) c->style_valid[b] = b <= c->tile.sp_last;
    c->have_style = true;
    c->tile.sp_last = -1;
    return ST_OK;
}

int st_get_style_gram(st_ctx* c, int blob, float* out)
{
    if (!c || blob < 0 || blob >= c->nb || !out) return fail(ST_ERR_ARG, "bad argument");
    if (!c->have_style || !c->style_valid[blob] || !c->style_gram[blob])
        return fail(ST_ERR_STATE, "blob %d (%s) has no style target", blob, c->blob_names[blob].c_str());
    HIP_TRY(hipSetDevice(c->device));
    const size_t C = c->blob_c_topo(blob);
    HIP_TRY(hipStreamSynchronize(c->stream));
    HIP_TRY(hipMemcpy(out, c->style_gram[blob], C * C * sizeof(float), hipMemcpyDeviceToHost));
    return ST_OK;
}

int st_tile_swap(st_ctx* c)
{
    if (c) c->epoch++;
    if (!c) return fail(ST_ERR_ARG, "ctx is NULL");
    c->cur ^= 1;
    return ST_OK;
}

}
```

style_transfer2_amd/csrc/gram.hip:

```cpp
#include "st2_kernels.h"
#include "env.h"
#include "wave_reduce.h"
#include <stdint.h>
#include <stdlib.h>

namespace st2 {

typedef float f32x16 __attribute__((ext_vector_type(16)));

constexpr int GKT = 32;
constexpr int GLD = GKT + 1;

GramPlan gram_plan(int C, int hw)
{
    GramPlan p;
    p.bt = C > 64 ? 128 : 64;
    const int t = (C + p.bt - 1) / p.bt;
    p.tiles = t * (t + 1) / 2;
    const int target128 = (int)env_int("ST2_GRAM_BLOCKS", 512), target64 = (int)env_int("ST2_GRAM_BLOCKS64", 1024);
    int want = p.bt == 128 ? target128 / p.tiles : (target64 + p.tiles - 1) / p.tiles;
    const int max_splits = (hw + 4 * GKT - 1) / (4 * GKT);
    if (want > max_splits) want = max_splits;
    if (want < 1) want = 1;
    int kslab = (hw + want - 1) / want;
    kslab = (kslab + GKT - 1) / GKT * GKT;
    p.kslab = kslab;
    p.splits = (hw + kslab - 1) / kslab;
    p.slab_floats = (size_t)p.splits * C * C;
    return p;
}

GramPlan gram_plan16(int C, int hw)
{
    GramPlan p = gram_plan(C, hw);
    p.kslab = (p.kslab + 63) / 64 * 64;
    p.splits = (hw + p.kslab - 1) / p.kslab;
    p.slab_floats = (size_t)p.splits * C * C;
    return p;
}

template <int BT>
__global__ __launch_bounds__(256) void gram_partial_k(const float* __restrict__ F, float* __restrict__ slabs,
                                                      int C, int hw, int tiles_1d, int kslab, GramRoi roi)
{
    constexpr int T = BT / 64;
    constexpr int ROWS_PER_T = BT / 8;
    __shared__ float As[BT * GLD];
    __shared__ float Bs[BT * GLD];

    const int tid = threadIdx.x, lane = tid & 63, wave = tid >> 6;
    const int wm = wave >> 1, wn = wave & 1;
    const int n_ut = tiles_1d * (tiles_1d + 1) / 2;
    int tile = blockIdx.x % n_ut;
    const int split = blockIdx.x / n_ut;
    int ti = 0;
    while (tile >= tiles_1d - ti) { tile -= tiles_1d - ti; ++ti; }
    const int tj = ti + tile;
    const int i0 = ti * BT, j0 = tj * BT;
    const bool diag = ti == tj;
    const int kbeg = split * kslab;
    const int kend = min(hw, kbeg + kslab);

    const int sk = tid & 31, sr = tid >> 5;
    float ra[ROWS_PER_T], rb[ROWS_PER_T];

    auto load = [&](int k0) {
        const int k = k0 + sk;
        const int ky = k / roi.rw, kx = k - ky * roi.rw;
        const size_t pix = (size_t)(roi.y0 + ky) * roi.pitch + roi.x0 + kx;
#pragma unroll
        for (int it = 0; it < ROWS_PER_T; ++it) {
            const int r = sr + it * 8;
            ra[it] = (i0 + r < C && k < kend) ? F[(size_t)(i0 + r) * roi.plane + pix] : 0.f;
            if (!diag) rb[it] = (j0 + r < C && k < kend) ? F[(size_t)(j0 + r) * roi.plane + pix] : 0.f;
        }
    };
    auto store = [&]() {
#pragma unroll
        for (int it = 0; it < ROWS_PER_T; ++it) {
            const int r = sr + it * 8;
            As[r * GLD + sk] = ra[it];
            if (!diag) Bs[r * GLD + sk] = rb[it];
        }
    };

    f32x16 acc[T][T];
#pragma unroll
    for (int i = 0; i < T; ++i)
#pragma unroll
        for (int j = 0; j < T; ++j)
#pragma unroll
            for (int e = 0; e < 16; ++e) acc[i][j][e] = 0.f;

    const float* bsrc = diag ? As : Bs;
    const int khalf = lane >> 5, l31 = lane & 31;
    const float* a_base = As + (wm * (T * 32) + l31) * GLD + khalf;
    const float* b_base = bsrc + (wn * (T * 32) + l31) * GLD + khalf;

    load(kbeg);
    for (int k0 = kbeg; k0 < kend; k0 += GKT) {
        __syncthreads();
        store();
        __syncthreads();
        if (k0 + GKT < kend) load(k0 + GKT);
#pragma unroll
        for (int ks = 0; ks < GKT / 2; ++ks) {
            float av[T], bv[T];
#pragma unroll
            for (int i = 0; i < T; ++i) av[i] = a_base[i * 32 * GLD + 2 * ks];
#pragma unroll
            for (int j = 0; j < T; ++j) bv[j] = b_base[j * 32 * GLD + 2 * ks];
#pragma unroll
            for (int i = 0; i < T; ++i)
#pragma unroll
                for (int j = 0; j < T; ++j)
                    acc[i][j] = __builtin_amdgcn_mfma_f32_32x32x2f32(av[i], bv[j], acc[i][j], 0, 0, 0);
        }
    }

    float* dst = slabs + (size_t)split * C * C;
#pragma unroll
    for (int i = 0; i < T; ++i)
#pragma unroll
        for (int j = 0; j < T; ++j) {
            const int col = j0 + wn * (T * 32) + j * 32 + l31;
#pragma unroll
            for (int e = 0; e < 16; ++e) {
                const int row = i0 + wm * (T * 32) + i * 32 + (e & 3) + 8 * (e >> 2) + 4 * khalf;
                if (row < C && col < C) dst[(size_t)row * C + col] = acc[i][j][e];
            }
        }
}

typedef __attribute__((address_space(3))) void* gram_lptr_t;
typedef float gf32x4 __attribute__((ext_vector_type(4)));

template <int BT>
__device__ __forceinline__ void gram_partial_dma_body(const float* __restrict__ F, unsigned f_bytes, float* __restrict__ slabs,
                                                      int C, int hw, int tiles_1d, int kslab)
{
    constexpr int T = BT / 64;
    constexpr int IMG = BT * 32;
    constexpr int PIECES = IMG / 256;
    constexpr int PPW = PIECES / 4;
    __shared__ __attribute__((aligned(16))) float smem[2][2][IMG];

    const int tid = threadIdx.x, lane = tid & 63;
    const int wave = __builtin_amdgcn_readfirstlane(tid >> 6);
    const int wm = wave >> 1, wn = wave & 1;
    const int n_ut = tiles_1d * (tiles_1d + 1) / 2;
    int tile = blockIdx.x % n_ut;
    const int split = blockIdx.x / n_ut;
    int ti = 0;
    while (tile >= tiles_1d - ti) { tile -= tiles_1d - ti; ++ti; }
    const int tj = ti + tile;
    const int i0 = ti * BT, j0 = tj * BT;
    const bool diag = ti == tj;
    const int kbeg = split * kslab;
    const int kend = min(hw, kbeg + kslab);
    const int nsteps = (kend - kbeg) / 32;

    const __amdgpu_buffer_rsrc_t rs = __builtin_amdgcn_make_buffer_rsrc((void*)F, 0, f_bytes, 0x00020000);
    unsigned aoff[PPW], boff[PPW];
#pragma unroll
    for (int t = 0; t < PPW; ++t) {
        const int slot = (wave + 4 * t) * 64 + lane;
        const int r = slot >> 3, q = (slot & 7) ^ ((r >> 1) & 7);
        aoff[t] = i0 + r < C ? ((unsigned)(i0 + r) * (unsigned)hw + (unsigned)kbeg + 4u * q) * 4u : 0xffffffffu;
        boff[t] = j0 + r < C ? ((unsigned)(j0 + r) * (unsigned)hw + (unsigned)kbeg + 4u * q) * 4u : 0xffffffffu;
    }
    auto dma = [&](int step, int stage) {
        const unsigned so = (unsigned)step * 128u;
#pragma unroll
        for (int t = 0; t < PPW; ++t) {
            __builtin_amdgcn_raw_ptr_buffer_load_lds(rs, (gram_lptr_t)(smem[stage][0] + (wave + 4 * t) * 256), 16,
                                                     aoff[t] == 0xffffffffu ? aoff[t] : aoff[t] + so, 0, 0, 0);
            if (!diag)
                __builtin_amdgcn_raw_ptr_buffer_load_lds(rs, (gram_lptr_t)(smem[stage][1] + (wave + 4 * t) * 256), 16,
                                                         boff[t] == 0xffffffffu ? boff[t] : boff[t] + so, 0, 0, 0);
        }
    };

    f32x16 acc[T][T];
#pragma unroll
    for (int i = 0; i < T; ++i)
#pragma unroll
        for (int j = 0; j < T; ++j)
#pragma unroll
            for (int e = 0; e < 16; ++e) acc[i][j][e] = 0.f;

    const int l31 = lane & 31;
    const bool hi = lane >= 32;
    int arow[T], brow[T];
#pragma unroll
    for (int i = 0; i < T; ++i) { arow[i] = wm * (T * 32) + i * 32 + l31; brow[i] = wn * (T * 32) + i * 32 + l31; }

    if (nsteps > 0) dma(0, 0);
    for (int st = 0; st < nsteps; ++st) {
        const int cur = st & 1;
        asm volatile("s_waitcnt vmcnt(0)" ::: "memory");
        __syncthreads();
        if (st + 1 < nsteps) dma(st + 1, cur ^ 1);
        const float* As = smem[cur][0];
        const float* Bs = diag ? smem[cur][0] : smem[cur][1];
#pragma unroll
        for (int q = 0; q < 8; ++q) {
            float a0[T], a1[T], b0[T], b1[T];
#pragma unroll
            for (int i = 0; i < T; ++i) {
                const gf32x4 v = *reinterpret_cast<const gf32x4*>(As + (arow[i] * 8 + (q ^ ((arow[i] >> 1) & 7))) * 4);
                a0[i] = hi ? v.y : v.x; a1[i] = hi ? v.w : v.z;
            }
#pragma unroll
            for (int j = 0; j < T; ++j) {
                const gf32x4 v = *reinterpret_cast<const gf32x4*>(Bs + (brow[j] * 8 + (q ^ ((brow[j] >> 1) & 7))) * 4);
                b0[j] = hi ? v.y : v.x; b1[j] = hi ? v.w : v.z;
            }
#pragma unroll
            for (int i = 0; i < T; ++i)
#pragma unroll
                for (int j = 0; j < T; ++j) {
                    acc[i][j] = __builtin_amdgcn_mfma_f32_32x32x2f32(a0[i], b0[j], acc[i][j], 0, 0, 0);
                    acc[i][j] = __builtin_amdgcn_mfma_f32_32x32x2f32(a1[i], b1[j], acc[i][j], 0, 0, 0);
                }
        }
    }

    const int khalf = lane >> 5;
    float* dst = slabs + (size_t)split * C * C;
#pragma unroll
    for (int i = 0; i < T; ++i)
#pragma unroll
        for (int j = 0; j < T; ++j) {
            const int col = j0 + wn * (T * 32) + j * 32 + l31;
#pragma unroll
            for (int e = 0; e < 16; ++e) {
                const int row = i0 + wm * (T * 32) + i * 32 + (e & 3) + 8 * (e >> 2) + 4 * khalf;
                if (row < C && col < C) dst[(size_t)row * C + col] = acc[i][j][e];
            }
        }
}

__global__ __launch_bounds__(256, 2) void gram_partial_dma_128(const float* F, unsigned f_bytes, float* slabs, int C, int hw, int tiles_1d, int kslab)
{ gram_partial_dma_body<128>(F, f_bytes, slabs, C, hw, tiles_1d, kslab); }
__global__ __launch_bounds__(256, 2) void gram_partial_dma_64(const float* F, unsigned f_bytes, float* slabs, int C, int hw, int tiles_1d, int kslab)
{ gram_partial_dma_body<64>(F, f_bytes, slabs, C, hw, tiles_1d, kslab); }

hipError_t launch_gram_partial(const float* F, float* slabs, int C, int hw, const GramPlan& pl, hipStream_t s,
                               const GramRoi* roi_in)
{
    const int t1 = (C + pl.bt - 1) / pl.bt;
    const unsigned grid = (unsigned)(pl.tiles * pl.splits);
    GramRoi roi = roi_in ? *roi_in : GramRoi{0, 0, hw, hw, (size_t)hw};
    if (!roi_in && !env_off("ST2_GRAM_DMA") && hw % 32 == 0 && pl.kslab % 32 == 0 && (reinterpret_cast<uintptr_t>(F) & 15) == 0 &&
        4ull * C * hw < 0xfffffff0ull) {
        const unsigned fb = (unsigned)(4ull * C * hw);
        if (pl.bt == 128) gram_partial_dma_128<<<grid, 256, 0, s>>>(F, fb, slabs, C, hw, t1, pl.kslab);
        else gram_partial_dma_64<<<grid, 256, 0, s>>>(F, fb, slabs, C, hw, t1, pl.kslab);
        return hipGetLastError();
    }
    if (pl.bt == 128) gram_partial_k<128><<<grid, 256, 0, s>>>(F, slabs, C, hw, t1, pl.kslab, roi);
    else gram_partial_k<64><<<grid, 256, 0, s>>>(F, slabs, C, hw, t1, pl.kslab, roi);
    return hipGetLastError();
}

__global__ __launch_bounds__(256) void gram_reduce_k(const float* __restrict__ slabs, const float* __restrict__ target,
                                                     float* __restrict__ out, float* __restrict__ partial,
                                                     int cc, int splits, float n, int C, int out_ld, int bt)
{
    __shared__ float scratch[4];
    float acc[1] = {0.f};
    for (int i = blockIdx.x * 256 + threadIdx.x; i < cc; i += gridDim.x * 256) {
        const int r = i / C, c = i - r * C;
        const int tr = r / bt, tc = c / bt;
        if (tr > tc) continue;
        float sum = 0.f;
        for (int s = 0; s < splits; ++s) sum += slabs[(size_t)s * cc + i];
        float v = sum / n;
        if (target) v -= target[i];
        out[r * out_ld + c] = v;
        acc[0] += v * v;
        if (tr < tc) { out[c * out_ld + r] = v; acc[0] += v * v; }
    }
    block_sum(acc, scratch);
    if (threadIdx.x == 0 && partial) partial[blockIdx.x] = acc[0];
}

__global__ __launch_bounds__(256) void gram_fold_k(const float* __restrict__ slabs, float* __restrict__ folded,
                                                   int cc, int splits, int per_group, int C, int bt)
{
    const int i = blockIdx.x * 256 + threadIdx.x;
    const int g = blockIdx.y;
    if (i >= cc) return;
    if ((i / C) / bt > (i % C) / bt) return;
    const int s0 = g * per_group, s1 = min(splits, s0 + per_group);
    float sum = 0.f;
    for (int s = s0; s < s1; ++s) sum += slabs[(size_t)s * cc + i];
    folded[(size_t)g * cc + i] = sum;
}

template <int GR_LANES>
__global__ __launch_bounds__(256) void gram_reduce_wide_k(const float* __restrict__ slabs, const float* __restrict__ target,
                                                          float* __restrict__ out, float* __restrict__ partial,
                                                          int cc, int splits, float n, int C, int out_ld, int bt)
{
    constexpr int GR_QUADS = 256 / GR_LANES, GR_ELEMS = 4 * GR_QUADS;
    __shared__ float4 part_s[GR_LANES][GR_QUADS];
    __shared__ float scratch[4];
    const int q = threadIdx.x % GR_QUADS, ln = threadIdx.x / GR_QUADS;
    float acc[1] = {0.f};
    for (int base = blockIdx.x * GR_ELEMS; base < cc; base += gridDim.x * GR_ELEMS) {
        const int i = base + 4 * q;
        const int r = i < cc ? i / C : 0, c = i < cc ? i - r * C : 0;
        const bool live = i < cc && r / bt <= c / bt;
        float4 sum = make_float4(0.f, 0.f, 0.f, 0.f);
        if (live)
            for (int s = ln; s < splits; s += GR_LANES) {
                const float4 v = *reinterpret_cast<const float4*>(slabs + (size_t)s * cc + i);
                sum.x += v.x; sum.y += v.y; sum.z += v.z; sum.w += v.w;
            }
        __syncthreads();
        part_s[ln][q] = sum;
        __syncthreads();
        if (ln == 0 && live) {
            float4 tot = part_s[0][q];
#pragma unroll
            for (int j = 1; j < GR_LANES; ++j) { const float4 p = part_s[j][q]; tot.x += p.x; tot.y += p.y; tot.z += p.z; tot.w += p.w; }
            float v[4] = {tot.x / n, tot.y / n, tot.z / n, tot.w / n};
            if (target) { const float4 t = *reinterpret_cast<const float4*>(target + i); v[0] -= t.x; v[1] -= t.y; v[2] -= t.z; v[3] -= t.w; }
            const bool mirror = r / bt < c / bt;
#pragma unroll
            for (int k = 0; k < 4; ++k) {
                out[r * out_ld + c + k] = v[k];
                acc[0] += v[k] * v[k];
                if (mirror) { out[(c + k) * out_ld + r] = v[k]; acc[0] += v[k] * v[k]; }
            }
        }
    }
    block_sum(acc, scratch);
    if (threadIdx.x == 0 && partial) partial[blockIdx.x] = acc[0];
}

int gram_fold_groups(const GramPlan& pl) { return pl.splits > 32 ? 32 : 0; }

hipError_t launch_gram_reduce(const float* slabs, float* folded, const float* target, float* out, int out_ld, float* partial,
                              int* n_partial, int C, double divisor, const GramPlan& pl, hipStream_t s)
{
    const int cc = C * C;
    int splits = pl.splits;
    if (splits > 32 && C % 4 == 0 && pl.bt % 4 == 0 && env_int("ST2_GRAM_REDUCE", 1) != 2) {
        const bool small = cc <= 128 * 128;
        const int grid = reduce_grid((size_t)cc, small ? 32 : 128, kMaxPartials);
        if (n_partial) *n_partial = grid;
        if (small) gram_reduce_wide_k<32><<<grid, 256, 0, s>>>(slabs, target, out, partial, cc, splits, (float)divisor, C, out_ld, pl.bt);
        else gram_reduce_wide_k<8><<<grid, 256, 0, s>>>(slabs, target, out, partial, cc, splits, (float)divisor, C, out_ld, pl.bt);
        return hipGetLastError();
    }
    const int groups = gram_fold_groups(pl);
    if (groups) {
        const int per = (pl.splits + groups - 1) / groups;
        gram_fold_k<<<dim3((cc + 255) / 256, groups), 256, 0, s>>>(slabs, folded, cc, pl.splits, per, C, pl.bt);
        slabs = folded;
        splits = (pl.splits + per - 1) / per;
    }
    const int grid = reduce_grid((size_t)cc, 256, kMaxPartials);
    if (n_partial) *n_partial = grid;
    gram_reduce_k<<<grid, 256, 0, s>>>(slabs, target, out, partial, cc, splits, (float)divisor, C, out_ld, pl.bt);
    return hipGetLastError();
}

}
```

style_transfer2_amd/csrc/passes.hip:

```cpp
#include "st2_kernels.h"
#include "channel_mean.h"
#include "wave_reduce.h"
#include <float.h>
#include <math.h>

namespace st2 {

int pooled_size(int n)
{
    int q = (n - 2 + 1) / 2;
    if (n - 2 < 0) q = 0;
    return q + 1;
}

__global__ __launch_bounds__(256) void maxpool_fwd_k(const float* __restrict__ in, float* __restrict__ out,
                                                     int C, int H, int W, int Ho, int Wo)
{
    const size_t total = (size_t)C * Ho * Wo;
    for (size_t idx = (size_t)blockIdx.x * 256 + threadIdx.x; idx < total; idx += (size_t)gridDim.x * 256) {
        const int px = (int)(idx % Wo);
        const int py = (int)((idx / Wo) % Ho);
        const int c = (int)(idx / ((size_t)Wo * Ho));
        const float* p = in + (size_t)c * H * W;
        const int r0 = 2 * py, c0 = 2 * px;
        float best = -FLT_MAX;
#pragma unroll
        for (int dr = 0; dr < 2; ++dr)
#pragma unroll
            for (int dc = 0; dc < 2; ++dc) {
                const int r = r0 + dr, cc = c0 + dc;
                if (r < H && cc < W) {
                    const float v = p[(size_t)r * W + cc];
                    if (v > best) best = v;
                }
            }
        out[idx] = best;
    }
}

__device__ __forceinline__ int first_max4(float a, float b, float c, float d, float* best)
{
    int arg = 0; float m = a;
    if (b > m) { m = b; arg = 1; }
    if (c > m) { m = c; arg = 2; }
    if (d > m) { m = d; arg = 3; }
    *best = m;
    return arg;
}

__global__ __launch_bounds__(256) void maxpool_fwd_v4_k(const float* __restrict__ in, float* __restrict__ out,
                                                        size_t n_patches, int W4, int Ho)
{
    for (size_t idx = (size_t)blockIdx.x * 256 + threadIdx.x; idx < n_patches; idx += (size_t)gridDim.x * 256) {
        const size_t q = idx % W4, pr = idx / W4;
        const float4 r0 = *reinterpret_cast<const float4*>(in + (pr * 2) * (size_t)W4 * 4 + q * 4);
        const float4 r1 = *reinterpret_cast<const float4*>(in + (pr * 2 + 1) * (size_t)W4 * 4 + q * 4);
        float2 o;
        first_max4(r0.x, r0.y, r1.x, r1.y, &o.x);
        first_max4(r0.z, r0.w, r1.z, r1.w, &o.y);
        *reinterpret_cast<float2*>(out + pr * (size_t)W4 * 2 + q * 2) = o;
    }
}

__global__ __launch_bounds__(256) void maxpool_bwd_v4_k(const float* __restrict__ dy, const float* __restrict__ x,
                                                        float* __restrict__ dx, const float* __restrict__ inject,
                                                        int apply_mask, size_t n_patches, int W4)
{
    for (size_t idx = (size_t)blockIdx.x * 256 + threadIdx.x; idx < n_patches; idx += (size_t)gridDim.x * 256) {
        const size_t q = idx % W4, pr = idx / W4;
        const size_t o0 = (pr * 2) * (size_t)W4 * 4 + q * 4, o1 = o0 + (size_t)W4 * 4;
        const float4 r0 = *reinterpret_cast<const float4*>(x + o0);
        const float4 r1 = *reinterpret_cast<const float4*>(x + o1);
        const float2 g = *reinterpret_cast<const float2*>(dy + pr * (size_t)W4 * 2 + q * 2);
        float best;
        const int a0 = first_max4(r0.x, r0.y, r1.x, r1.y, &best);
        const int a1 = first_max4(r0.z, r0.w, r1.z, r1.w, &best);
        float4 d0 = make_float4(a0 == 0 ? g.x : 0.f, a0 == 1 ? g.x : 0.f, a1 == 0 ? g.y : 0.f, a1 == 1 ? g.y : 0.f);
        float4 d1 = make_float4(a0 == 2 ? g.x : 0.f, a0 == 3 ? g.x : 0.f, a1 == 2 ? g.y : 0.f, a1 == 3 ? g.y : 0.f);
        if (apply_mask) {
            d0.x = r0.x > 0.f ? d0.x : 0.f; d0.y = r0.y > 0.f ? d0.y : 0.f; d0.z = r0.z > 0.f ? d0.z : 0.f; d0.w = r0.w > 0.f ? d0.w : 0.f;
            d1.x = r1.x > 0.f ? d1.x : 0.f; d1.y = r1.y > 0.f ? d1.y : 0.f; d1.z = r1.z > 0.f ? d1.z : 0.f; d1.w = r1.w > 0.f ? d1.w : 0.f;
        }
        if (inject) {
            const float4 i0 = *reinterpret_cast<const float4*>(inject + o0);
            const float4 i1 = *reinterpret_cast<const float4*>(inject + o1);
            d0.x += i0.x; d0.y += i0.y; d0.z += i0.z; d0.w += i0.w;
            d1.x += i1.x; d1.y += i1.y; d1.z += i1.z; d1.w += i1.w;
        }
        *reinterpret_cast<float4*>(dx + o0) = d0;
        *reinterpret_cast<float4*>(dx + o1) = d1;
    }
}

__global__ __launch_bounds__(256) void maxpool_bwd_amap_k(const float* __restrict__ dy, const unsigned char* __restrict__ amap,
                                                          float* __restrict__ dx, size_t n_patches, int W4)
{
    for (size_t idx = (size_t)blockIdx.x * 256 + threadIdx.x; idx < n_patches; idx += (size_t)gridDim.x * 256) {
        const size_t q = idx % W4, pr = idx / W4;
        const size_t o0 = (pr * 2) * (size_t)W4 * 4 + q * 4, o1 = o0 + (size_t)W4 * 4;
        const size_t po = pr * (size_t)W4 * 2 + q * 2;
        const float2 g = *reinterpret_cast<const float2*>(dy + po);
        const unsigned short mm = *reinterpret_cast<const unsigned short*>(amap + po);
        const unsigned m0 = mm & 0xffu, m1 = mm >> 8;
        const float g0 = (m0 & 4u) ? g.x : 0.f, g1 = (m1 & 4u) ? g.y : 0.f;
        const unsigned a0 = m0 & 3u, a1 = m1 & 3u;
        *reinterpret_cast<float4*>(dx + o0) = make_float4(a0 == 0 ? g0 : 0.f, a0 == 1 ? g0 : 0.f, a1 == 0 ? g1 : 0.f, a1 == 1 ? g1 : 0.f);
        *reinterpret_cast<float4*>(dx + o1) = make_float4(a0 == 2 ? g0 : 0.f, a0 == 3 ? g0 : 0.f, a1 == 2 ? g1 : 0.f, a1 == 3 ? g1 : 0.f);
    }
}

hipError_t launch_maxpool_bwd_amap(const float* dy, const unsigned char* amap, float* dx, int C, int H, int W, hipStream_t s)
{
    if (H % 2 != 0 || W % 4 != 0 || (reinterpret_cast<uintptr_t>(amap) & 1) != 0) return hipErrorInvalidValue;
    const size_t n_patches = (size_t)C * (H / 2) * (W / 4);
    maxpool_bwd_amap_k<<<reduce_grid(n_patches, 256, 65536), 256, 0, s>>>(dy, amap, dx, n_patches, W / 4);
    return hipGetLastError();
}

hipError_t launch_maxpool_fwd(const float* in, float* out, int C, int H, int W, hipStream_t s)
{
    const int Ho = pooled_size(H), Wo = pooled_size(W);
    const size_t total = (size_t)C * Ho * Wo;
    if (H % 2 == 0 && W % 4 == 0) {
        const size_t n_patches = (size_t)C * Ho * (W / 4);
        maxpool_fwd_v4_k<<<reduce_grid(n_patches, 256, 65536), 256, 0, s>>>(in, out, n_patches, W / 4, Ho);
        return hipGetLastError();
    }
    maxpool_fwd_k<<<reduce_grid(total, 256, 65536), 256, 0, s>>>(in, out, C, H, W, Ho, Wo);
    return hipGetLastError();
}

__global__ __launch_bounds__(256) void maxpool_bwd_k(const float* __restrict__ dy, const float* __restrict__ x,
                                                     float* __restrict__ dx, const float* __restrict__ inject,
                                                     int apply_mask, int C, int H, int W, int Ho, int Wo)
{
    const size_t total = (size_t)C * Ho * Wo;
    for (size_t idx = (size_t)blockIdx.x * 256 + threadIdx.x; idx < total; idx += (size_t)gridDim.x * 256) {
        const int px = (int)(idx % Wo);
        const int py = (int)((idx / Wo) % Ho);
        const int c = (int)(idx / ((size_t)Wo * Ho));
        const size_t base = (size_t)c * H * W;
        const int r0 = 2 * py, c0 = 2 * px;
        float best = -FLT_MAX;
        int arg = -1;
        float vals[4];
#pragma unroll
        for (int k = 0; k < 4; ++k) {
            const int r = r0 + (k >> 1), cc = c0 + (k & 1);
            vals[k] = 0.f;
            if (r < H && cc < W) {
                vals[k] = x[base + (size_t)r * W + cc];
                if (vals[k] > best) { best = vals[k]; arg = k; }
            }
        }
        const float g = dy[idx];
#pragma unroll
        for (int k = 0; k < 4; ++k) {
            const int r = r0 + (k >> 1), cc = c0 + (k & 1);
            if (r < H && cc < W) {
                const size_t o = base + (size_t)r * W + cc;
                float v = (k == arg) ? g : 0.f;
                if (apply_mask) v = vals[k] > 0.f ? v : 0.f;
                if (inject) v += inject[o];
                dx[o] = v;
            }
        }
    }
}

hipError_t launch_maxpool_bwd(const float* dy, const float* x, float* dx, const float* inject,
                              int apply_mask, int C, int H, int W, hipStream_t s)
{
    const int Ho = pooled_size(H), Wo = pooled_size(W);
    const size_t total = (size_t)C * Ho * Wo;
    if (H % 2 == 0 && W % 4 == 0) {
        const size_t n_patches = (size_t)C * Ho * (W / 4);
        maxpool_bwd_v4_k<<<reduce_grid(n_patches, 256, 65536), 256, 0, s>>>(dy, x, dx, inject, apply_mask, n_patches, W / 4);
        return hipGetLastError();
    }
    maxpool_bwd_k<<<reduce_grid(total, 256, 65536), 256, 0, s>>>(dy, x, dx, inject, apply_mask, C, H, W, Ho, Wo);
    return hipGetLastError();
}

typedef __bf16 ap_bf16x8 __attribute__((ext_vector_type(8)));

__device__ __forceinline__ float ave_window_scale(int r0, int c0, int H, int W)
{
    const int n = (min(r0 + 2, H) - r0) * (min(c0 + 2, W) - c0);
    return n == 4 ? 0.25f : n == 2 ? 0.5f : 1.0f;
}

__global__ __launch_bounds__(256) void avepool_fwd_k(const float* __restrict__ in, float* __restrict__ out,
                                                     unsigned short* __restrict__ out16, int C, int H, int W, int Ho, int Wo)
{
    const size_t hwo = (size_t)Ho * Wo, total = (size_t)((C + 7) / 8) * hwo;
    for (size_t idx = (size_t)blockIdx.x * 256 + threadIdx.x; idx < total; idx += (size_t)gridDim.x * 256) {
        const size_t p = idx % hwo, cb = idx / hwo;
        const int py = (int)(p / Wo), px = (int)(p % Wo);
        const int r0 = 2 * py, c0 = 2 * px;
        const bool r1ok = r0 + 1 < H, c1ok = c0 + 1 < W;
        const float scale = ave_window_scale(r0, c0, H, W);
        ap_bf16x8 v;
#pragma unroll
        for (int j = 0; j < 8; ++j) {
            const int c = (int)cb * 8 + j;
            float t = 0.f;
            if (c < C) {
                const float* q = in + (size_t)c * H * W + (size_t)r0 * W + c0;
                t += q[0];
                if (c1ok) t += q[1];
                if (r1ok) t += q[W];
                if (r1ok && c1ok) t += q[W + 1];
                t = t * scale;
                if (out) out[(size_t)c * hwo + p] = t;
            }
            v[j] = (__bf16)t;
        }
        if (out16) *reinterpret_cast<ap_bf16x8*>(out16 + idx * 8) = v;
    }
}

__global__ __launch_bounds__(256) void avepool_fwd_v4_k(const float* __restrict__ in, float* __restrict__ out,
                                                        unsigned short* __restrict__ out16, int C, int W4, int Ho, size_t n_patches)
{
    const size_t rowp = (size_t)Ho * W4;
    const size_t hw = (size_t)Ho * W4 * 8, hwo = (size_t)Ho * W4 * 2;
    for (size_t idx = (size_t)blockIdx.x * 256 + threadIdx.x; idx < n_patches; idx += (size_t)gridDim.x * 256) {
        const size_t pp = idx % rowp, cb = idx / rowp;
        const size_t py = pp / W4, q = pp % W4;
        float4 r0[8], r1[8];
#pragma unroll
        for (int j = 0; j < 8; ++j) {
            const int c = (int)cb * 8 + j;
            if (c < C) {
                const float* base = in + (size_t)c * hw + (2 * py) * (size_t)W4 * 4 + q * 4;
                r0[j] = *reinterpret_cast<const float4*>(base);
                r1[j] = *reinterpret_cast<const float4*>(base + (size_t)W4 * 4);
            } else {
                r0[j] = r1[j] = make_float4(0.f, 0.f, 0.f, 0.f);
            }
        }
        ap_bf16x8 v0, v1;
        const size_t po = py * (size_t)W4 * 2 + q * 2;
#pragma unroll
        for (int j = 0; j < 8; ++j) {
            const int c = (int)cb * 8 + j;
            float2 o;
            o.x = ((((0.f + r0[j].x) + r0[j].y) + r1[j].x) + r1[j].y) * 0.25f;
            o.y = ((((0.f + r0[j].z) + r0[j].w) + r1[j].z) + r1[j].w) * 0.25f;
            if (c >= C) o = make_float2(0.f, 0.f);
            else if (out) *reinterpret_cast<float2*>(out + (size_t)c * hwo + po) = o;
            v0[j] = (__bf16)o.x; v1[j] = (__bf16)o.y;
        }
        if (out16) {
            unsigned short* d = out16 + (cb * hwo + po) * 8;
            *reinterpret_cast<ap_bf16x8*>(d) = v0;
            *reinterpret_cast<ap_bf16x8*>(d + 8) = v1;
        }
    }
}

hipError_t launch_avepool_fwd(const float* in, float* out, unsigned short* out16, int C, int H, int W, hipStream_t s)
{
    if (!out && !out16) return hipErrorInvalidValue;
    const int Ho = pooled_size(H), Wo = pooled_size(W);
    const int CB = (C + 7) / 8;
    if (H % 2 == 0 && W % 4 == 0) {
        const size_t n_patches = (size_t)CB * Ho * (W / 4);
        avepool_fwd_v4_k<<<reduce_grid(n_patches, 256, 65536), 256, 0, s>>>(in, out, out16, C, W / 4, Ho, n_patches);
        return hipGetLastError();
    }
    const size_t total = (size_t)CB * Ho * Wo;
    avepool_fwd_k<<<reduce_grid(total, 256, 65536), 256, 0, s>>>(in, out, out16, C, H, W, Ho, Wo);
    return hipGetLastError();
}

__global__ __launch_bounds__(256) void avepool_bwd_k(const float* __restrict__ dy, const float* __restrict__ x,
                                                     const float* __restrict__ inject, float* __restrict__ dx,
                                                     unsigned short* __restrict__ dx16, int C, int H, int W, int Ho, int Wo)
{
    const size_t hw = (size_t)H * W, hwo = (size_t)Ho * Wo, total = (size_t)((C + 7) / 8) * hw;
    for (size_t idx = (size_t)blockIdx.x * 256 + threadIdx.x; idx < total; idx += (size_t)gridDim.x * 256) {
        const size_t p = idx % hw, cb = idx / hw;
        const int r = (int)(p / W), col = (int)(p % W);
        const int py = r >> 1, px = col >> 1;
        const float scale = ave_window_scale(2 * py, 2 * px, H, W);
        ap_bf16x8 v;
#pragma unroll
        for (int j = 0; j < 8; ++j) {
            const int c = (int)cb * 8 + j;
            float t = 0.f;
            if (c < C) {
                const size_t o = (size_t)c * hw + p;
                t = dy[(size_t)c * hwo + (size_t)py * Wo + px] * scale;
                if (x) t = x[o] > 0.f ? t : 0.f;
                if (inject) t += inject[o];
                if (dx) dx[o] = t;
            }
            v[j] = (__bf16)t;
        }
        if (dx16) *reinterpret_cast<ap_bf16x8*>(dx16 + idx * 8) = v;
    }
}

__global__ __launch_bounds__(256) void avepool_bwd_v4_k(const float* __restrict__ dy, const float* __restrict__ x,
// ... 170 lines not shown

__global__ __launch_bounds__(256) void scaled_accumulate_k(const float* __restrict__ S, float* __restrict__ inject,
                                                           float sw, const float* __restrict__ norm,
                                                           int accumulate, size_t n)
{
    const float coef = sw / *norm;
    for (size_t i = (size_t)blockIdx.x * 256 + threadIdx.x; i < n; i += (size_t)gridDim.x * 256) {
        const float base = accumulate ? inject[i] : 0.f;
        inject[i] = coef * S[i] + base;
    }
}

hipError_t launch_scaled_accumulate(const float* S, float* inject, float sw, const float* norm,
                                    int accumulate, size_t n, hipStream_t s)
{
    scaled_accumulate_k<<<reduce_grid(n, 256 * 4, 8192), 256, 0, s>>>(S, inject, sw, norm, accumulate, n);
    return hipGetLastError();
}

__device__ __forceinline__ float tv_k(float q, float half_beta, int beta_is_2)
{
    return beta_is_2 ? 1.0f : half_beta * powf(q, half_beta - 1.0f);
}

constexpr int IP_TY = 4, IP_TX = 256;
constexpr int IP_LW = IP_TX + 2;

__global__ __launch_bounds__(256) void image_pass_k(const ImagePassArgs a)
{
    __shared__ float scratch[32];
    __shared__ float u_s[(IP_TY + 2) * IP_LW];
    const int H = a.H, W = a.W, tid = threadIdx.x;
    const size_t plane = (size_t)H * W;
    const float half_beta = a.tv_beta * 0.5f;
    const int beta_is_2 = a.tv_beta == 2.0f;
    const float corr1 = a.dyn ? a.dyn[0] : a.corr1, corr2 = a.dyn ? a.dyn[1] : a.corr2, step = a.dyn ? a.dyn[2] : a.step;
    const int p_round = (int)a.p_pow;
    const int p_int = ((float)p_round == a.p_pow && p_round >= 1 && p_round <= 16) ? p_round : 0;
    const int tiles_x = (W + IP_TX - 1) / IP_TX, tiles_y = (H + IP_TY - 1) / IP_TY;
    const int n_tiles = a.C * tiles_y * tiles_x;
    float acc[6] = {0.f, 0.f, 0.f, 0.f, 0.f, 0.f};
    for (int tile = blockIdx.x; tile < n_tiles; tile += gridDim.x) {
        const int tx = tile % tiles_x, rest = tile / tiles_x;
        const int ty = rest % tiles_y, ch = rest / tiles_y;
        const int x0 = tx * IP_TX, y0 = ty * IP_TY;
        const float* p = a.x + (size_t)ch * plane;
        __syncthreads();
        for (int e = tid; e < (IP_TY + 2) * IP_LW; e += 256) {
            const int r = e / IP_LW, c = e - r * IP_LW;
            int gy = y0 - 1 + r, gx = x0 - 1 + c;
            gy = gy < 0 ? H - 1 : (gy >= H ? gy - H : gy);
            gx = gx < 0 ? W - 1 : (gx >= W ? gx - W : gx);
            u_s[e] = (gy < H && gx < W) ? p[(size_t)gy * W + gx] / 255.0f : 0.f;
        }
        __syncthreads();
        const int x = x0 + tid;
        if (x < W) {
#pragma unroll
            for (int ry = 0; ry < IP_TY; ++ry) {
                const int y = y0 + ry;
                if (y >= H) break;
                const float* us = u_s + (ry + 1) * IP_LW + tid + 1;
                const size_t idx = (size_t)ch * plane + (size_t)y * W + x;
                const float xv = a.x[idx];
                const float u = us[0];
                const float u_r = us[1], u_l = us[-1];
                const float u_d = us[IP_LW], u_u = us[-IP_LW];
                const float u_dl = us[IP_LW - 1], u_ur = us[-IP_LW + 1];
                const float a0 = u - u_r, b0 = u - u_d;
                const float q0 = (a0 * a0 + b0 * b0) + 1e-8f;
                const float k0 = tv_k(q0, half_beta, beta_is_2);
                const float da0 = (2.0f * a0) * k0, db0 = (2.0f * b0) * k0;
                const float aL = u_l - u, bL = u_l - u_dl;
                const float qL = (aL * aL + bL * bL) + 1e-8f;
                const float daL = (2.0f * aL) * tv_k(qL, half_beta, beta_is_2);
                const float aU = u_u - u_ur, bU = u_u - u;
                const float qU = (aU * aU + bU * bU) + 1e-8f;
                const float dbU = (2.0f * bU) * tv_k(qU, half_beta, beta_is_2);
                float g_tv = da0 + db0;
                g_tv -= daL;
                g_tv -= dbU;
                acc[0] += beta_is_2 ? q0 : powf(q0, half_beta);
                const float mag = fabsf(u);
                const float sgn = u > 0.f ? 1.f : (u < 0.f ? -1.f : 0.f);
                float pw, pw1;
                if (p_int) {
                    pw1 = p_int > 1 ? mag : 1.0f;
                    for (int k = 2; k < p_int; ++k) pw1 *= mag;
                    pw = pw1 * mag;
                } else {
                    pw = powf(mag, a.p_pow);
                    pw1 = powf(mag, a.p_pow - 1.0f);
                }
                acc[1] += pw;
                const float g_p = sgn * pw1;
                const float scd = a.scd ? a.scd[idx] : 0.f;
                const float tg = a.tv_w * g_tv;
                const float pg = a.p_w * g_p;
                float g = scd + tg;
                g += pg;
                acc[2] += scd * scd;
                acc[3] += tg * tg;
                acc[4] += pg * pg;
                acc[5] += g * g;
                if (a.grad) a.grad[idx] = g;
                if (a.x_out) {
                    const float m_old = a.m_is_zero ? 0.f : a.m[idx];
                    const float v_old = a.v_is_zero ? 0.f : a.v[idx];
                    const float m_new = a.d1 * m_old + a.c1 * g;
                    const float v_new = a.d2 * v_old + a.c2 * (g * g);
                    a.m[idx] = m_new;
                    a.v[idx] = v_new;
                    const float m_hat = m_new / corr1;
                    const float v_hat = v_new / corr2;
                    a.x_out[idx] = xv - (step * m_hat) / (sqrtf(v_hat) + 1e-8f);
                }
            }
        }
    }
    block_sum(acc, scratch);
    if (threadIdx.x == 0) {
#pragma unroll
        for (int i = 0; i < 6; ++i) a.partial[i * kMaxPartials + blockIdx.x] = acc[i];
    }
}

__global__ void set_scalars3_k(float* dst, float a, float b, float c) { dst[0] = a; dst[1] = b; dst[2] = c; }
hipError_t launch_set_scalars3(float* dst, float a, float b, float c, hipStream_t s)
{
    set_scalars3_k<<<1, 1, 0, s>>>(dst, a, b, c);
    return hipGetLastError();
}

hipError_t launch_image_pass(const ImagePassArgs& a, int* n_partial, hipStream_t s)
{
    const long long n_tiles = (long long)a.C * ((a.H + IP_TY - 1) / IP_TY) * ((a.W + IP_TX - 1) / IP_TX);
    const int grid = (int)(n_tiles < kMaxPartials ? (n_tiles < 1 ? 1 : n_tiles) : kMaxPartials);
    *n_partial = grid;
    image_pass_k<<<grid, 256, 0, s>>>(a);
    return hipGetLastError();
}

__global__ __launch_bounds__(256) void image_pass_tile_k(const ImageTileArgs t)
{
    __shared__ float scratch[32];
    const ImagePassArgs& a = t.base;
    const int th = t.th, tw = t.tw, ww = a.W;
    const size_t wplane = (size_t)a.H * a.W, tplane = (size_t)th * tw, rplane = (size_t)(th + 2) * (tw + 2);
    const size_t total = tplane * 3;
    const float half_beta = a.tv_beta * 0.5f;
    const int beta_is_2 = a.tv_beta == 2.0f;
    float acc[6] = {0.f, 0.f, 0.f, 0.f, 0.f, 0.f};
    for (size_t idx = (size_t)blockIdx.x * 256 + threadIdx.x; idx < total; idx += (size_t)gridDim.x * 256) {
        const int x = (int)(idx % tw);
        const int y = (int)((idx / tw) % th);
        const int c = (int)(idx / tplane);
        const float* p = a.x + c * wplane;
        const float* rg = t.ring + c * rplane;
        auto U = [&](int yy, int xx) -> float {
            const bool inside = yy >= 0 && yy < th && xx >= 0 && xx < tw;
            const float v = inside ? p[(size_t)(t.ty + yy) * ww + t.tx + xx] : rg[(size_t)(yy + 1) * (tw + 2) + xx + 1];
            return v / 255.0f;
        };
        const size_t widx = c * wplane + (size_t)(t.ty + y) * ww + t.tx + x;
        const float xv = p[(size_t)(t.ty + y) * ww + t.tx + x];
        const float u = xv / 255.0f;
        const float u_r = U(y, x + 1), u_d = U(y + 1, x), u_l = U(y, x - 1), u_u = U(y - 1, x);
        const float u_dl = U(y + 1, x - 1), u_ur = U(y - 1, x + 1);
        const float a0 = u - u_r, b0 = u - u_d;
        const float q0 = (a0 * a0 + b0 * b0) + 1e-8f;
        const float k0 = tv_k(q0, half_beta, beta_is_2);
        const float da0 = (2.0f * a0) * k0, db0 = (2.0f * b0) * k0;
        const float aL = u_l - u, bL = u_l - u_dl;
        const float qL = (aL * aL + bL * bL) + 1e-8f;
        const float daL = (2.0f * aL) * tv_k(qL, half_beta, beta_is_2);
        const float aU = u_u - u_ur, bU = u_u - u;
        const float qU = (aU * aU + bU * bU) + 1e-8f;
        const float dbU = (2.0f * bU) * tv_k(qU, half_beta, beta_is_2);
        float g_tv = da0 + db0;
        g_tv -= daL;
        g_tv -= dbU;
        acc[0] += beta_is_2 ? q0 : powf(q0, half_beta);
        const float mag = fabsf(u);
        const float sgn = u > 0.f ? 1.f : (u < 0.f ? -1.f : 0.f);
        acc[1] += powf(mag, a.p_pow);
        const float g_p = sgn * powf(mag, a.p_pow - 1.0f);
        const float scd = a.scd ? a.scd[widx] : 0.f;
        const float tg = a.tv_w * g_tv;
        const float pg = a.p_w * g_p;
        float g = scd + tg;
        g += pg;
        acc[2] += scd * scd;
        acc[3] += tg * tg;
        acc[4] += pg * pg;
        acc[5] += g * g;
        if (a.grad) a.grad[widx] = g;
        if (a.x_out) {
            const float m_old = a.m_is_zero ? 0.f : a.m[widx];
            const float v_old = a.v_is_zero ? 0.f : a.v[widx];
            const float m_new = a.d1 * m_old + a.c1 * g;
            const float v_new = a.d2 * v_old + a.c2 * (g * g);
            a.m[widx] = m_new;
            a.v[widx] = v_new;
            const float m_hat = m_new / a.corr1;
            const float v_hat = v_new / a.corr2;
            a.x_out[widx] = xv - (a.step * m_hat) / (sqrtf(v_hat) + 1e-8f);
        }
    }
    block_sum(acc, scratch);
    if (threadIdx.x == 0) {
#pragma unroll
        for (int i = 0; i < 6; ++i) a.partial[i * kMaxPartials + blockIdx.x] = acc[i];
    }
}

hipError_t launch_image_pass_tile(const ImageTileArgs& a, int* n_partial, hipStream_t s)
{
    const size_t total = (size_t)3 * a.th * a.tw;
    const int grid = reduce_grid(total, 256 * 4, kMaxPartials);
    *n_partial = grid;
    image_pass_tile_k<<<grid, 256, 0, s>>>(a);
    return hipGetLastError();
}

__global__ __launch_bounds__(256) void resample_h_k(const float* __restrict__ src, float* __restrict__ dst, size_t rows,
                                                    int w_in, int w_out, ResampleTable t, int clamp0)
{
    const size_t total = rows * w_out;
    for (size_t idx = (size_t)blockIdx.x * 256 + threadIdx.x; idx < total; idx += (size_t)gridDim.x * 256) {
        const int xx = (int)(idx % w_out);
        const size_t row = idx / w_out;
        const float* p = src + row * w_in + t.lo[xx];
        const double* k = t.k + (size_t)xx * t.kmax;
        double ss = 0.0;
        for (int i = 0; i < t.n[xx]; ++i) ss += (double)p[i] * k[i];
        float v = (float)ss;
        if (clamp0) v = v > 0.f ? v : 0.f;
        dst[idx] = v;
    }
}

__global__ __launch_bounds__(256) void resample_v_k(const float* __restrict__ src, float* __restrict__ dst, int planes,
                                                    int h_in, int h_out, int w, ResampleTable t, int clamp0)
{
    const size_t total = (size_t)planes * h_out * w;
    for (size_t idx = (size_t)blockIdx.x * 256 + threadIdx.x; idx < total; idx += (size_t)gridDim.x * 256) {
        const int x = (int)(idx % w);
        const int yy = (int)((idx / w) % h_out);
        const size_t pl = idx / ((size_t)w * h_out);
        const float* p = src + (pl * h_in + t.lo[yy]) * w + x;
        const double* k = t.k + (size_t)yy * t.kmax;
        double ss = 0.0;
        for (int i = 0; i < t.n[yy]; ++i) ss += (double)p[(size_t)i * w] * k[i];
        float v = (float)ss;
        if (clamp0) v = v > 0.f ? v : 0.f;
        dst[idx] = v;
    }
}

__global__ __launch_bounds__(256) void clamp0_copy_k(const float* src, float* dst, size_t n, int clamp0)
{
    for (size_t i = (size_t)blockIdx.x * 256 + threadIdx.x; i < n; i += (size_t)gridDim.x * 256)
        dst[i] = clamp0 ? (src[i] > 0.f ? src[i] : 0.f) : src[i];
}

hipError_t launch_resample(const float* src, float* tmp, float* dst, int planes, int h_in, int w_in, int h_out, int w_out,
                           const ResampleTable& tx, const ResampleTable& ty, int clamp0, hipStream_t s)
{
    const bool need_h = w_in != w_out, need_v = h_in != h_out;
    const float* cur = src;
    if (need_h) {
        float* out = need_v ? tmp : dst;
        const size_t rows = (size_t)planes * h_in;
        resample_h_k<<<reduce_grid(rows * w_out, 256, 16384), 256, 0, s>>>(cur, out, rows, w_in, w_out, tx, need_v ? 0 : clamp0);
        cur = out;
    }
    if (need_v) resample_v_k<<<reduce_grid((size_t)planes * h_out * w_out, 256, 16384), 256, 0, s>>>(cur, dst, planes, h_in, h_out, w_out, ty, clamp0);
    if (!need_h && !need_v) clamp0_copy_k<<<reduce_grid((size_t)planes * h_in * w_in, 1024, 8192), 256, 0, s>>>(src, dst, (size_t)planes * h_in * w_in, clamp0);
    return hipGetLastError();
}

template <typename T>
__global__ __launch_bounds__(256) void preprocess_k(const T* __restrict__ hwc, float* __restrict__ nchw, int H, int W)
{
    const size_t plane = (size_t)H * W;
    for (size_t i = (size_t)blockIdx.x * 256 + threadIdx.x; i < plane * 3; i += (size_t)gridDim.x * 256) {
        const int c = (int)(i / plane);
        const size_t p = i % plane;
        nchw[i] = (float)hwc[p * 3 + c] - kMean[c];
    }
}

hipError_t launch_preprocess_u8(const uint8_t* hwc, float* nchw, int H, int W, hipStream_t s)
{
    preprocess_k<uint8_t><<<reduce_grid((size_t)H * W * 3, 1024, 8192), 256, 0, s>>>(hwc, nchw, H, W);
    return hipGetLastError();
}
hipError_t launch_preprocess_f32(const float* hwc, float* nchw, int H, int W, hipStream_t s)
{
    preprocess_k<float><<<reduce_grid((size_t)H * W * 3, 1024, 8192), 256, 0, s>>>(hwc, nchw, H, W);
    return hipGetLastError();
}

__global__ __launch_bounds__(256) void trace_sums_k(const TraceArgs a)
{
    __shared__ double scratch[256];
    const int slot = blockIdx.x;
    const int nl = a.n_layers * kLayerSlots;
    double v = 0.0;
    if (slot < nl) {
        const TraceLayer& L = a.layer[slot / kLayerSlots];
        const int k = slot % kLayerSlots;
        if (L.part[k] && L.count[k] > 0) v = sum_partials(L.part[k], L.count[k], scratch);
    } else {
        v = sum_partials(a.image_part + (slot - nl) * kMaxPartials, a.image_count, scratch);
    }
    if (threadIdx.x == 0) a.sums[slot] = v;
}

__global__ void finalize_trace_k(const TraceArgs a)
{
    if (threadIdx.x != 0) return;
    const double* sums = a.sums;
    float loss = 0.f;
    for (int l = 0; l < a.n_layers; ++l) {
        const TraceLayer& L = a.layer[l];
        const double* sm = sums + l * kLayerSlots;
        float* o = a.out + l * 6;
        for (int k = 0; k < 6; ++k) o[k] = 0.f;
        if (L.content) {
            const float nc = L.norm[0];
            const float c_loss = (L.cw * (float)(sm[0] / L.n)) / nc;
            loss += c_loss;
            o[0] = c_loss;
            o[1] = (fabsf(L.cw) * sqrtf((float)(sm[1] / L.n))) / nc;
        }
        if (L.style) {
            const float ns = L.norm[1];
            const float s_loss = (L.sw * (float)(sm[4] / L.gram_n)) / ns;
            loss += s_loss;
            o[2] = s_loss;
            o[3] = fabsf(L.sw / ns) * sqrtf((float)(sm[5] / L.n));
        }
        if (L.deepdream) {
            const float nd = L.norm[2];
            const float d_loss = (-L.dw * (float)(sm[2] / L.n)) / nd;
            loss += d_loss;
            o[4] = d_loss;
            o[5] = (fabsf(L.dw) * sqrtf((float)(sm[3] / L.n))) / nd;
        }
    }
    const double* im = sums + a.n_layers * kLayerSlots;
    float* g = a.out + a.n_layers * 6;
    g[0] = loss;
    const float t_loss = a.tv_w * (float)im[0];
    loss += t_loss;
    const float p_loss = a.p_w * ((float)im[1] / a.p_pow);
    loss += p_loss;
    g[1] = t_loss;
    g[2] = p_loss;
    g[3] = a.have_grad ? sqrtf((float)(im[2] / a.image_n)) : 0.f;
    g[4] = a.have_grad ? sqrtf((float)(im[3] / a.image_n)) : 0.f;
    g[5] = a.have_grad ? sqrtf((float)(im[4] / a.image_n)) : 0.f;
    g[6] = loss;
    g[7] = a.have_grad ? sqrtf((float)(im[5] / a.image_n)) : 0.f;
}

hipError_t launch_finalize_trace(const TraceArgs& a, hipStream_t s)
{
    trace_sums_k<<<a.n_layers * kLayerSlots + kImageSlots, 256, 0, s>>>(a);
    finalize_trace_k<<<1, 64, 0, s>>>(a);
    return hipGetLastError();
}

__global__ __launch_bounds__(256) void strip_copy_k(float* __restrict__ tensor, float* __restrict__ buf, const StripTable t, int C, int wh, int ww, int mode)
{
    const size_t plane = (size_t)wh * ww;
    for (size_t idx = (size_t)blockIdx.x * 256 + threadIdx.x; idx < (size_t)t.total; idx += (size_t)gridDim.x * 256) {
        int r = 0;
#pragma unroll
        for (int k = 1; k < kMaxStripRects; ++k) r += (k < t.n && idx >= (size_t)t.off[k]) ? 1 : 0;
        const size_t e = idx - t.off[r];
        const int w = t.w[r], h = t.h[r];
        const int x = (int)(e % w), y = (int)((e / w) % h), c = (int)(e / ((size_t)w * h));
        float* tp = tensor + (size_t)c * plane + (size_t)(t.y0[r] + y) * ww + t.x0[r] + x;
        if (mode == 0) buf[idx] = *tp;
        else if (mode == 1) *tp = buf[idx];
        else *tp += buf[idx];
    }
}

hipError_t launch_strip_copy(float* tensor, float* buf, const StripTable& t, int C, int wh, int ww, int mode, hipStream_t s)
{
    if (t.n <= 0 || t.total <= 0) return hipSuccess;
    const int grid = reduce_grid((size_t)t.total, 256 * 4, 2048);
    strip_copy_k<<<grid, 256, 0, s>>>(tensor, buf, t, C, wh, ww, mode);
    return hipGetLastError();
}

__global__ __launch_bounds__(256) void dot_final_k(const float* part, int n_part, float* out)
{
    __shared__ double scratch[256];
    const double sum = sum_partials(part, n_part, scratch);
    if (threadIdx.x == 0) *out = (float)sum;
}

hipError_t launch_sum_partials(const float* part, int n, float* out, hipStream_t s)
{
    dot_final_k<<<1, 256, 0, s>>>(part, n, out);
    return hipGetLastError();
}

__global__ __launch_bounds__(256) void vec_dot_k(const float* __restrict__ a, const float* __restrict__ b, size_t n, float* __restrict__ part)
{
    __shared__ float scratch[8];
    float acc[1] = {0.f};
    for (size_t i = (size_t)blockIdx.x * 256 + threadIdx.x; i < n; i += (size_t)gridDim.x * 256) acc[0] += a[i] * b[i];
    block_sum(acc, scratch);
    if (threadIdx.x == 0) part[blockIdx.x] = acc[0];
}

hipError_t launch_vec_dot(const float* a, const float* b, size_t n, float* part, float* out, hipStream_t s)
{
    const int grid = reduce_grid(n, 256 * 8, kMaxPartials);
    vec_dot_k<<<grid, 256, 0, s>>>(a, b, n, part);
    dot_final_k<<<1, 256, 0, s>>>(part, grid, out);
    return hipGetLastError();
}

__global__ __launch_bounds__(256) void vec_axpy_k(float alpha, const float* __restrict__ x, float* __restrict__ y, size_t n)
{
    for (size_t i = (size_t)blockIdx.x * 256 + threadIdx.x; i < n; i += (size_t)gridDim.x * 256) y[i] = alpha * x[i] + y[i];
}

hipError_t launch_vec_axpy(float alpha, const float* x, float* y, size_t n, hipStream_t s)
{
    vec_axpy_k<<<reduce_grid(n, 256 * 4, 8192), 256, 0, s>>>(alpha, x, y, n);
    return hipGetLastError();
}

__global__ __launch_bounds__(256) void vec_div_k(double divisor, float* __restrict__ y, size_t n)
{
    for (size_t i = (size_t)blockIdx.x * 256 + threadIdx.x; i < n; i += (size_t)gridDim.x * 256) y[i] = (float)((double)y[i] / divisor);
}

hipError_t launch_vec_div(double divisor, float* y, size_t n, hipStream_t s)
{
    vec_div_k<<<reduce_grid(n, 256 * 4, 8192), 256, 0, s>>>(divisor, y, n);
    return hipGetLastError();
}

__global__ __launch_bounds__(256) void lincomb_k(float a, const float* x, float b, const float* y, float* z, size_t n)
{
    for (size_t i = (size_t)blockIdx.x * 256 + threadIdx.x; i < n; i += (size_t)gridDim.x * 256) {
        float v = a * x[i];
        if (y) v += b * y[i];
        z[i] = v;
    }
}

hipError_t launch_lincomb(float a, const float* x, float b, const float* y, float* z, size_t n, hipStream_t s)
{
    lincomb_k<<<reduce_grid(n, 256 * 4, 8192), 256, 0, s>>>(a, x, b, y, z, n);
    return hipGetLastError();
}

}
```

style_transfer2_amd/csrc/st2_kernels.h:

```cpp
#pragma once
#include <hip/hip_runtime.h>
#include <stddef.h>
#include <stdint.h>

#include "emit_plan.h"

namespace st2 {

constexpr int kMaxPartials = 1024;
constexpr int kConvCC = 4;
constexpr int kCoutQuantum = 64;

struct ConvProblem {
    const float* in;
    const float* wpack;
    const float* bias;
    float* out;
    const float* mask_src;
    const float* inject;
    int K, M, MPad, H, W;
    int relu;
    unsigned long long* stamps = nullptr;
    unsigned short* out16 = nullptr;
    float* pool_out = nullptr;
    unsigned char* pool_amap = nullptr;
    const unsigned char* unpool_amap = nullptr;
    float* scratch = nullptr;
    size_t scratch_floats = 0;
};
size_t conv_pack_floats(int K, int M);
int conv_mpad(int M);
void pack_conv_weights_fwd(const float* w , int Cout, int Cin, float* dst);
void pack_conv_weights_dgrad(const float* w , int Cout, int Cin, float* dst);
hipError_t launch_conv3x3(const ConvProblem& p, hipStream_t s);
int conv_num_configs();
const char* conv_config_name(int cfg);
int conv_pick_config(const ConvProblem& p);
hipError_t launch_conv3x3_cfg(const ConvProblem& p, int cfg, hipStream_t s);
size_t wino_pack_floats(int K, int M);
void pack_wino_weights_fwd(const float* w, int Cout, int Cin, float* dst);
void pack_wino_weights_dgrad(const float* w, int Cout, int Cin, float* dst);
enum WinoVariant {
    WV_128x128 = 0, WV_64x256 = 1, WV_PS64x256 = 3, WV_W8_128x128 = 6, WV_H4_64x128 = 8,
    WV_128x128_STAMPED = 2, WV_64x256_STAMPED = 5, WV_PS64x256_STAMPED = 4, WV_W8_128x128_STAMPED = 7, WV_H4_64x128_STAMPED = 9,
};
struct WinoLaunch {
    bool ok;
    WinoVariant variant;
    bool quad, big;
    int bm, prows;
    long long nblk;
    int splits;
    bool can_pool;
    bool pool_amap;
    bool can_skip_out;
    bool can_unpool;
};
WinoLaunch wino_resolve(int K, int M, int H, int W, int forced_variant = -1);
int wino_splitk(long long nblk, int nch);
hipError_t launch_maxpool_bwd_amap(const float* dy, const unsigned char* amap, float* dx, int C, int H, int W, hipStream_t s);
hipError_t launch_conv3x3_wino(const ConvProblem& p, hipStream_t s);
hipError_t launch_conv3x3_wino_cfg(const ConvProblem& p, int variant, hipStream_t s);
hipError_t launch_wino_combine(const float* scratch, int splits, const float* bias, int relu, const float* mask_src, const float* inject,
                               float* out, int M, int H, int W, hipStream_t s);
size_t wino_split_pack_elems(int K, int M);
void pack_wino_split_weights_fwd(const float* w, int Cout, int Cin, unsigned short* dst);
void pack_wino_split_weights_dgrad(const float* w, int Cout, int Cin, unsigned short* dst);
WinoLaunch wino_split_resolve(int K, int M, int H, int W);
hipError_t launch_conv3x3_wino_split(const ConvProblem& p, hipStream_t s);
bool conv_dgrad_first_ok(int Cout, int Cin, int H, int W, bool bf16);
hipError_t launch_conv3x3_dgrad_first(const float* dy, const float* w, float* dx, const float* inject, int Cout, int Cin, int H, int W, hipStream_t s);
bool conv_dgrad_first_strip_ok(int Cout, int Cin, int H, int W);
hipError_t launch_conv3x3_dgrad_first_strip(const float* dy, const float* w, float* dx, const float* inject, int Cout, int Cin, int H, int W, hipStream_t s);
bool conv_dgrad_first_quad_ok(int Cout, int Cin, int H, int W, const float* dy);
hipError_t launch_conv3x3_dgrad_first_quad(const float* dy, const float* w, float* dx, const float* inject, int Cout, int Cin, int H, int W, hipStream_t s);
hipError_t launch_conv3x3_dgrad_first16(const unsigned short* dy16, const float* w_rounded, float* dx, const float* inject, int Cout, int Cin,
                                        int H, int W, hipStream_t s);
size_t conv_first_split_pack_elems(int Cout);
void pack_conv_first_split(const float* w , const float* bias , int Cout, int Cin, unsigned short* dst);
bool conv_first_split_ok(int Cin, int Cout, int H, int W);
hipError_t launch_conv3x3_first_split(const float* x, const unsigned short* wpk, float* out, unsigned short* out16,
                                      int Cin, int Cout, int H, int W, int relu, hipStream_t s, unsigned short* bits_out = nullptr);
bool conv_dgrad_smallM_ok(int Cout, int Cin);
hipError_t launch_conv3x3_dgrad_smallM(const float* dy, const float* w, float* dx, const float* inject,
                                       int Cout, int Cin, int H, int W, hipStream_t s);
hipError_t launch_conv3x3_dgrad_smallM16(const unsigned short* dy16, const float* w_rounded, float* dx, const float* inject,
                                         int Cout, int Cin, int H, int W, hipStream_t s);

struct Conv16Problem {
    const unsigned short* in16; const unsigned short* wpack16; const float* bias;
    float* out;
    unsigned short* out16; const float* mask_src; const float* inject;
    int K, M, MPad, H, W, relu;
    const unsigned short* mask16 = nullptr;
    unsigned short* pool16 = nullptr;
    float* pool32 = nullptr;
    unsigned char* amap = nullptr;
    bool pool_ave = false;
    const unsigned short* s_in16 = nullptr; const unsigned short* s_wpack16 = nullptr;
    const unsigned char* unpool_amap = nullptr;
    bool unpool_ave = false;
    unsigned short* bits_out = nullptr; const unsigned short* mask_bits = nullptr;
    unsigned long long* stamps = nullptr;
};
inline size_t conv16_bits_elems(int M, size_t hw) { return (size_t)(M / 32) * hw * 2; }
size_t style_fuse_pack_elems(int C, int MPad);
hipError_t launch_style_fuse_pack(const float* D, int ld, int C, int MPad, float c2, float sw, const float* norm, unsigned short* A16, hipStream_t s);
int style_s2_trace_blocks(int C);
hipError_t launch_style_s2_trace(const float* D, int ld, const float* A, int C, double n, float c2, float* partial, int* n_partial, hipStream_t s);
struct Conv16Launch {
    int cfg;
    bool sb;
    int BM, ROWS;
    bool can_pool;
    bool can_unpool;
};
Conv16Launch conv16_resolve(const Conv16Problem& p);
hipError_t launch_maxpool_bwd_idx16(const unsigned short* dy16, const unsigned char* amap, unsigned short* dx16, int C, int H, int W, hipStream_t s);
hipError_t launch_avepool_bwd_map16(const unsigned short* dy16, const unsigned char* map, unsigned short* dx16, int C, int H, int W, hipStream_t s);
size_t conv16_pack_elems(int K, int M);
void pack_conv_weights16_fwd(const float* w, int Cout, int Cin, unsigned short* dst);
void pack_conv_weights16_dgrad(const float* w, int Cout, int Cin, unsigned short* dst);
hipError_t launch_conv3x3_bf16(const Conv16Problem& p, hipStream_t s);
hipError_t launch_pack_act16(const float* src, unsigned short* dst, int C, size_t hw, hipStream_t s);

int pooled_size(int n);
hipError_t launch_maxpool_fwd(const float* in, float* out, int C, int H, int W, hipStream_t s);
hipError_t launch_maxpool_bwd(const float* dy, const float* x, float* dx, const float* inject,
                              int apply_mask, int C, int H, int W, hipStream_t s);

hipError_t launch_avepool_fwd(const float* in, float* out, unsigned short* out16, int C, int H, int W, hipStream_t s);
hipError_t launch_avepool_bwd(const float* dy, const float* x, const float* inject, float* dx, unsigned short* dx16,
                              int C, int H, int W, hipStream_t s);

struct GramPlan { int bt, tiles, splits, kslab; size_t slab_floats; };
GramPlan gram_plan(int C, int hw);
GramPlan gram_plan16(int C, int hw);
bool gram16_ok(int C, int hw, const GramPlan& pl);
struct GramRoi { int y0, x0, rw, pitch; size_t plane; };
bool gram16_roi_ok(int C, int hw, size_t plane, const GramPlan& pl);
hipError_t launch_gram16_partial(const unsigned short* F16, float* slabs, int C, int hw, const GramPlan& pl, hipStream_t s,
                                 const GramRoi* roi = nullptr);
hipError_t launch_gram_partial(const float* F, float* slabs, int C, int hw, const GramPlan& pl, hipStream_t s,
                               const GramRoi* roi = nullptr);
bool gram_split_ok(int C, int hw);
hipError_t launch_gram_split_partial(const float* F, float* slabs, int C, int hw, const GramPlan& pl, hipStream_t s);
int gram_fold_groups(const GramPlan& pl);
hipError_t launch_gram_reduce(const float* slabs, float* folded, const float* target, float* out, int out_ld, float* partial,
                              int* n_partial, int C, double divisor, const GramPlan& pl, hipStream_t s);

int style_grad_blocks(int C, int H, int W);
struct PixRoi { int y0, x0, y1, x1; };
hipError_t launch_style_grad(const float* Dp, const float* F, float* dst, float c2, int fused, float sw, const float* norm,
                             int accumulate, float* partial, int* n_partial, int C, int H, int W, hipStream_t s,
                             const PixRoi* roi = nullptr);
bool style_grad_split_ok(int C, int hw);
size_t style_grad_split_pack_elems(int C);
int style_grad_split_blocks(int C, int hw);
hipError_t launch_style_grad_split(const float* Dp, int ld, unsigned short* A16, const float* F, float* dst, float c2, int fused, float sw,
                                   const float* norm, int accumulate, float* partial, int* n_partial, int C, int hw, hipStream_t s);
bool style_grad16_ok(int C, size_t hw);
size_t style_grad16_pack_elems(int C);
int style_grad16_blocks(int C, size_t hw);
hipError_t launch_style_grad16(const float* Dp, int ld, unsigned short* A16, const unsigned short* F16, float* dst, float c2, int fused,
                               float sw, const float* norm, int accumulate, float* partial, int* n_partial, int C, size_t hw, hipStream_t s,
                               const GramRoi* roi = nullptr);
hipError_t launch_sum_partials(const float* part, int n, float* out, hipStream_t s);
hipError_t launch_scaled_accumulate(const float* S, float* inject, float sw, const float* norm,
                                    int accumulate, size_t n, hipStream_t s);

struct LayerElemArgs {
    const float* feat;
    const float* target;
    float* inject;
    size_t n;
    float cn_coef, dn_coef;
    float cw, dw;
    int content, deepdream, write;
    const float* norm_c;
    const float* norm_d;
    float* part_d2;
    float* part_gc2;
    float* part_f2;
    float* part_gd2;
    int h, w, ry0, rx0, ry1, rx1;
};
hipError_t launch_layer_elem(const LayerElemArgs& a, int* n_partial, hipStream_t s);

hipError_t launch_finalize_norm(const float* partial, int n_partial, double n, float* norm, hipStream_t s);

struct ImagePassArgs {
    const float* x;
    const float* scd;
    float* grad;
    int C, H, W;
    float tv_w, tv_beta, p_w, p_pow;
    float* x_out; float* m; float* v;
    float d1, c1, d2, c2, corr1, corr2, step;
    int m_is_zero;
    int v_is_zero;
    float* partial;
    const float* dyn = nullptr;
};
hipError_t launch_set_scalars3(float* dst, float a, float b, float c, hipStream_t s);
hipError_t launch_image_pass(const ImagePassArgs& a, int* n_partial, hipStream_t s);
struct ImageTileArgs {
    ImagePassArgs base;
    const float* ring;
    int ty, tx, th, tw;
};
hipError_t launch_image_pass_tile(const ImageTileArgs& a, int* n_partial, hipStream_t s);

constexpr int kMaxStripRects = 12;
struct StripTable { int n; int total; int y0[kMaxStripRects], x0[kMaxStripRects], h[kMaxStripRects], w[kMaxStripRects], off[kMaxStripRects]; };
hipError_t launch_strip_copy(float* tensor, float* buf, const StripTable& t, int C, int wh, int ww, int mode, hipStream_t s);

struct ResampleTable { const int* lo; const int* n; const double* k; int kmax; };
hipError_t launch_resample(const float* src, float* tmp, float* dst, int planes, int h_in, int w_in, int h_out, int w_out,
                           const ResampleTable& tx, const ResampleTable& ty, int clamp0, hipStream_t s);

hipError_t launch_preprocess_u8(const uint8_t* hwc, float* nchw, int H, int W, hipStream_t s);
hipError_t launch_preprocess_f32(const float* hwc, float* nchw, int H, int W, hipStream_t s);
struct EmitArgs { int source, colour; const float* x; float* mean; const float* cx; float* hwc; int H, W; float decay, rest, corr; int first; };
hipError_t launch_emit(const EmitArgs& a, hipStream_t s);
constexpr int kMomentSums = 9;
constexpr int kMomentBlocks = 256;
hipError_t launch_image_moments(const float* x, size_t n, double* partials, double* out, hipStream_t s);
struct RecolorArgs { float* x; size_t n; float A[9], b[3]; };
hipError_t launch_recolor(const RecolorArgs& a, hipStream_t s);

constexpr int kMaxTraceLayers = 24;
constexpr int kLayerSlots = 6;
constexpr int kImageSlots = 6;
struct TraceLayer {
    int content, style, deepdream;
    float cw, sw, dw;
    double n;
    double gram_n;
    int count[kLayerSlots];
    const float* part[kLayerSlots];
    const float* norm;
};
struct TraceArgs {
    int n_layers;
    TraceLayer layer[kMaxTraceLayers];
    const float* image_part;
    int image_count;
    double image_n;
    float tv_w, p_w, p_pow;
    int have_grad;
    float* out;
    double* sums;
};
hipError_t launch_finalize_trace(const TraceArgs& a, hipStream_t s);

constexpr int kLbfgsCorr = 10;
constexpr int kLbfgsSlots = kLbfgsCorr + 1;
struct LbfgsDev {
    int count;
    int free_slot;
    int order[kLbfgsSlots];
    int pad_;
    double sy[kLbfgsSlots], yy[kLbfgsSlots];
    double alpha[kLbfgsSlots];
    double last_sy;
};
constexpr int kLbNB = 2 * kLbfgsSlots + 1;
constexpr int kLbGramRows = 2 * kLbNB;
struct LbfgsGram {
    double B[kLbNB][kLbNB];
    double delta[kLbNB];
    double r0;
};
struct LbfgsVecs { float* s[kLbfgsSlots]; float* y[kLbfgsSlots]; };
struct LbfgsArgs {
    LbfgsVecs v;
    LbfgsDev* st;
    LbfgsGram* gm;
    float* gpart;
    float* part;
    float* part2;
    const float* g;
    float* p;
    float* x;
    size_t n;
    float step;
    int apply;
    float* gsums;
    size_t n_global;
};
hipError_t launch_lbfgs_two_loop(const LbfgsArgs& a, hipStream_t s);
hipError_t launch_lbfgs_pair(const LbfgsArgs& a, const float* g_new, int mode, hipStream_t s);
hipError_t launch_lbfgs_gram_pass(const LbfgsArgs& a, const float* g_new, int mode, hipStream_t s);
hipError_t launch_lbfgs_gram_apply(const LbfgsArgs& a, hipStream_t s);
hipError_t launch_lbfgs_gram_pass_local(const LbfgsArgs& a, const float* g_new, int mode, hipStream_t s);
hipError_t launch_lbfgs_gram_commit_global(const LbfgsArgs& a, int mode, hipStream_t s);
int lbfgs_gram_rows();
hipError_t launch_lbfgs_gram_load(const LbfgsArgs& a, const float* dots, hipStream_t s);
hipError_t launch_lincomb(float a, const float* x, float b, const float* y, float* z, size_t n, hipStream_t s);
hipError_t launch_vec_dot(const float* a, const float* b, size_t n, float* part, float* out, hipStream_t s);
hipError_t launch_vec_axpy(float alpha, const float* x, float* y, size_t n, hipStream_t s);
hipError_t launch_vec_div(double divisor, float* y, size_t n, hipStream_t s);

}
```

Baseline: 143.4 it/s.

## Batch Gram reductions across style layers and fuse trace finalize into one kernel

Style Gram partials for all style layers are now written to separate slab regions and reduced by a single batched kernel that maps block ranges to layers. Each layer gets its own D buffer so the gradients can run after the batched reduce. Separately, the trace sum and finalize kernels are merged using an atomic ticket so the last block does the finalize. Both changes aim to cut kernel launch count and small-kernel tail latency, at the cost of extra per-layer D memory and larger slab scratch.

```diff
diff --git a/style_transfer2_amd/csrc/engine.cpp b/style_transfer2_amd/csrc/engine.cpp
--- a/style_transfer2_amd/csrc/engine.cpp
+++ b/style_transfer2_amd/csrc/engine.cpp
@@ -468,7 +468,8 @@
     ST_TRY(c->norms.alloc(c->nb * 3));
     ST_TRY(c->image_part.alloc(6 * kMaxPartials));
     ST_TRY(c->trace_dev.alloc(kMaxTraceLayers * 6 + 8));
-    ST_TRY(c->trace_sums.alloc(kMaxTraceLayers * kLayerSlots + kImageSlots));
+    ST_TRY(c->trace_sums.alloc(kTraceSumSlots + 1));
+    HIP_TRY(hipMemset(c->trace_sums + kTraceSumSlots, 0, sizeof(double)));
     ST_TRY(c->lb_dev.alloc(1));
     HIP_TRY(hipMemset(c->lb_dev, 0, sizeof(LbfgsDev)));
     ST_TRY(c->lb_part.alloc(4 * kMaxPartials));
diff --git a/style_transfer2_amd/csrc/engine.h b/style_transfer2_amd/csrc/engine.h
--- a/style_transfer2_amd/csrc/engine.h
+++ b/style_transfer2_amd/csrc/engine.h
@@ -137,12 +137,13 @@
     bool any = false;
     bool resized = false;
     int style_blob = -1;
+    const float* D = nullptr;
     int raw_blob = -1;
     std::vector<size_t> n;
     std::vector<int> C;
     std::vector<char> diff;
     std::vector<char> norm_ok;
-    void begin(int nb) { any = resized = false; style_blob = raw_blob = -1; n.assign(nb, 0); C.assign(nb, 0); diff.assign(nb, LT_NONE); norm_ok.assign((size_t)nb * 3, 0); }
+    void begin(int nb) { any = resized = false; style_blob = raw_blob = -1; D = nullptr; n.assign(nb, 0); C.assign(nb, 0); diff.assign(nb, LT_NONE); norm_ok.assign((size_t)nb * 3, 0); }
 };
 }
 
@@ -186,6 +187,7 @@
     DevBuf<float> diffA, diffB, stmp;
     size_t max_blob = 0;
     DevBuf<float> gram_slabs, gram_fold, dbuf;
+    std::vector<DevBuf<float>> dterm;
     DevBuf<unsigned short> d16;
     std::vector<DevBuf<unsigned short>> sfuse_w;
     std::vector<const unsigned short*> sf_in, sf_w;
@@ -344,9 +346,11 @@
 StyleShape style_shape(const st_ctx* c, const ActSet& a, int b);
 StyleTerm style_term(const st_ctx* c, const ActSet& a, int b, const BlobRoi* roi = nullptr, bool target = false, int fuse_last = -1);
 size_t style_split_scratch(int C, int hw);
+int style_gram_partial(st_ctx* c, const ActSet& a, const StyleTerm& t, float* slabs);
 int style_gram(st_ctx* c, const ActSet& a, const StyleTerm& t, const float* target, float* out, int out_ld, double divisor, float* partial, int* n_partial);
-int style_grad(st_ctx* c, const ActSet& a, const StyleTerm& t, float* dst, float c2, int fused, float sw, int accumulate, int* np);
+int style_grad(st_ctx* c, const ActSet& a, const StyleTerm& t, const float* D, float* dst, float c2, int fused, float sw, int accumulate, int* np);
 int ensure_dbuf(st_ctx* c);
+int ensure_dterm(st_ctx* c, int b);
 int ensure_layer_part(st_ctx* c, int b);
 LayerElemArgs layer_elem_args(const st_ctx* c, const ActiveLayer& al, double n_norm, int write, float* part, const BlobRoi* roi = nullptr);
 int objective_terms(const st_ctx* c, const ActSet& a, const TileGeom* tile, ObjTerms& terms);
diff --git a/style_transfer2_amd/csrc/engine_objective.cpp b/style_transfer2_amd/csrc/engine_objective.cpp
--- a/style_transfer2_amd/csrc/engine_objective.cpp
+++ b/style_transfer2_amd/csrc/engine_objective.cpp
@@ -66,7 +66,24 @@
     std::fill(c->cnt.begin(), c->cnt.end(), 0);
     c->sf_in.assign(c->nb, nullptr); c->sf_w.assign(c->nb, nullptr);
     c->lt.begin(c->nb);
-    for (const ObjTerm& ot : terms.t) {
+    struct StyleRun { StyleTerm t; size_t slabs; bool wrote; };
+    std::vector<StyleRun> runs(terms.t.size());
+    bool batch = !c->tile.on && !env_off("ST2_GRAM_BATCH") && terms.n_style <= kMaxGramBatch;
+    size_t slab_floats = 0;
+    for (size_t i = 0; i < terms.t.size(); ++i) {
+        const ObjTerm& ot = terms.t[i];
+        if (!ot.al.s) continue;
+        StyleRun& r = runs[i];
+        r.t = style_term(c, a, ot.b, nullptr, false, want_grad ? last : -1);
+        r.slabs = slab_floats;
+        slab_floats += (r.t.plan.slab_floats + 63) / 64 * 64;
+        if (gram_reduce_mode(ot.C, r.t.plan) == GRAM_REDUCE_FOLDED) batch = false;
+    }
+    if (batch && terms.n_style) ST_TRY(c->gram_slabs.reserve(slab_floats));
+    GramReduceBatch red{};
+    const ObjTerm* red_last = nullptr;
+
+    auto term_begin = [&](const ObjTerm& ot, StyleRun& r) -> int {
         const ActiveLayer& al = ot.al;
         const int b = ot.b, C = ot.C;
         const size_t n = ot.n;
@@ -93,16 +110,35 @@
             cnt[0] = cnt[1] = cnt[2] = cnt[3] = np;
             wrote = true;
         }
+        r.wrote = wrote;
+        if (!al.s) return ST_OK;
+        ST_TRY(ensure_dterm(c, b));
+        if (!batch) return style_gram(c, a, r.t, c->style_gram[b], c->dterm[b], conv_mpad(C), (double)n, part + 4 * kMaxPartials, &cnt[4]);
+        ST_TRY(style_gram_partial(c, a, r.t, c->gram_slabs + r.slabs));
+        GramReduceEntry& g = red.e[red.n++];
+        g.slabs = c->gram_slabs + r.slabs; g.target = c->style_gram[b]; g.out = c->dterm[b]; g.partial = part + 4 * kMaxPartials;
+        g.out_ld = conv_mpad(C); g.splits = r.t.plan.splits; g.C = C; g.bt = r.t.plan.bt; g.mode = gram_reduce_mode(C, r.t.plan);
+        g.n = (float)(double)n;
+        cnt[4] = gram_reduce_blocks(C, g.mode);
+        red_last = &ot;
+        return ST_OK;
+    };
+    auto term_end = [&](const ObjTerm& ot, const StyleRun& r) -> int {
+        const ActiveLayer& al = ot.al;
+        const int b = ot.b, C = ot.C;
+        const size_t n = ot.n;
+        float* nrm = c->norms + b * 3;
+        int* cnt = &c->cnt[b * 6];
+        const bool wrote = r.wrote;
         if (al.s) {
-            ST_TRY(ensure_dbuf(c));
-            const StyleTerm t = style_term(c, a, b, nullptr, false, want_grad ? last : -1);
-            ST_TRY(style_gram(c, a, t, c->style_gram[b], c->dbuf, conv_mpad(C), (double)n, part + 4 * kMaxPartials, &cnt[4]));
+            const StyleTerm& t = r.t;
+            const float* D = c->dterm[b];
             const float c2 = (float)(2.0 / ((double)C * C * (double)n));
             if (c->norm_valid[b * 3 + 1]) {
-                ST_TRY(style_grad(c, a, t, c->inject[b], c2, 1, al.sw, wrote, &cnt[5]));
+                ST_TRY(style_grad(c, a, t, D, c->inject[b], c2, 1, al.sw, wrote, &cnt[5]));
             } else {
                 if (!c->stmp) ST_TRY(c->stmp.alloc(c->max_blob));
-                ST_TRY(style_grad(c, a, t, c->stmp, c2, 0, al.sw, 0, &cnt[5]));
+                ST_TRY(style_grad(c, a, t, D, c->stmp, c2, 0, al.sw, 0, &cnt[5]));
                 { ProfScope ps(c, P_FINALIZE, 0, 0);
                   HIP_TRY(launch_finalize_norm(c->s2_part[b], cnt[5], (double)n, nrm + 1, c->stream)); }
                 c->norm_valid[b * 3 + 1] = 1;
@@ -110,13 +146,26 @@
                 HIP_TRY(launch_scaled_accumulate(c->stmp, c->inject[b], al.sw, nrm + 1, wrote, n, c->stream));
                 c->lt.raw_blob = b;
             }
-            c->lt.style_blob = b;
+            c->lt.style_blob = b; c->lt.D = D;
             if (c->lt.raw_blob != b) c->lt.raw_blob = -1;
         }
         c->lt.n[b] = n; c->lt.C[b] = C;
         c->lt.diff[b] = c->sf_w[b] ? LT_RODE_ON_CONV : LT_WRITTEN;
         for (int k = 0; k < 3; ++k) c->lt.norm_ok[b * 3 + k] = c->norm_valid[b * 3 + k];
         inj[b] = (c->sf_w[b] && !wrote) ? nullptr : c->inject[b];
+        return ST_OK;
+    };
+
+    if (!batch) {
+        for (size_t i = 0; i < terms.t.size(); ++i) { ST_TRY(term_begin(terms.t[i], runs[i])); ST_TRY(term_end(terms.t[i], runs[i])); }
+    } else {
+        for (size_t i = 0; i < terms.t.size(); ++i) ST_TRY(term_begin(terms.t[i], runs[i]));
+        for (size_t i = 0; i < terms.t.size(); ++i) {
+            if (!terms.t[i].al.s) continue;
+            ProfScope ps(c, P_GRAM_REDUCE, 0, 4.0 * (double)runs[i].t.plan.slab_floats, runs[i].t.book);
+            if (&terms.t[i] == red_last) HIP_TRY(launch_gram_reduce_batch(red, c->stream));
+        }
+        for (size_t i = 0; i < terms.t.size(); ++i) ST_TRY(term_end(terms.t[i], runs[i]));
     }
 
     const float* scd = nullptr;
@@ -157,6 +206,7 @@
         t.tv_w = c->tv_w; t.p_w = c->p_w; t.p_pow = c->p_pow; t.have_grad = want_grad;
         t.out = c->trace_dev;
         t.sums = c->trace_sums;
+        t.ticket = reinterpret_cast<unsigned*>(c->trace_sums + kTraceSumSlots);
         c->trace_len_last = t.n_layers * 6 + 8;
         ProfScope ps(c, P_FINALIZE, 0, 0);
         HIP_TRY(launch_finalize_trace(t, c->stream));
@@ -235,11 +285,11 @@
     if (diff && lt.diff[index] == LT_OVERWRITTEN)
         return fail(ST_ERR_STATE, "st_backward has overwritten the diff of blob %d (%s) since the last evaluation", index, name);
     if (diff && (lt.diff[index] != LT_WRITTEN || !c->inject[index])) return fail(ST_ERR_STATE, "blob %d (%s) has no diff of the last evaluation", index, name);
-    if ((D && !c->dbuf) || (raw_S && !c->stmp)) return fail(ST_ERR_STATE, "internal: the buffer of blob %d (%s) is gone", index, name);
+    if ((D && !lt.D) || (raw_S && !c->stmp)) return fail(ST_ERR_STATE, "internal: the buffer of blob %d (%s) is gone", index, name);
     HIP_TRY(hipSetDevice(c->device));
     HIP_TRY(hipStreamSynchronize(c->stream));
     const size_t C = (size_t)lt.C[index], n = lt.n[index];
-    if (D) HIP_TRY(hipMemcpy2D(D, C * sizeof(float), c->dbuf, (size_t)conv_mpad((int)C) * sizeof(float), C * sizeof(float), C, hipMemcpyDeviceToHost));
+    if (D) HIP_TRY(hipMemcpy2D(D, C * sizeof(float), lt.D, (size_t)conv_mpad((int)C) * sizeof(float), C * sizeof(float), C, hipMemcpyDeviceToHost));
     if (raw_S) HIP_TRY(hipMemcpy(raw_S, c->stmp, n * sizeof(float), hipMemcpyDeviceToHost));
     if (diff) HIP_TRY(hipMemcpy(diff, c->inject[index], n * sizeof(float), hipMemcpyDeviceToHost));
     if (norms) {
diff --git a/style_transfer2_amd/csrc/engine_style.cpp b/style_transfer2_amd/csrc/engine_style.cpp
--- a/style_transfer2_amd/csrc/engine_style.cpp
+++ b/style_transfer2_amd/csrc/engine_style.cpp
@@ -59,25 +59,31 @@
 
 static int missing_copy(const StyleTerm& t) { return fail(ST_ERR_STATE, t.roi ? "internal: style blob %d has no fp32 copy" : "internal: style blob %d has neither an fp32 nor a usable bf16 copy", t.b); }
 
-int style_gram(st_ctx* c, const ActSet& a, const StyleTerm& t, const float* target, float* out, int out_ld, double divisor, float* partial, int* n_partial)
+int style_gram_partial(st_ctx* c, const ActSet& a, const StyleTerm& t, float* slabs)
 {
     if (t.missing32) return missing_copy(t);
     const int b = t.b, C = t.C;
     const GramRoi* roi = t.roi ? &t.groi : nullptr;
+    ProfScope ps(c, t.gram.cls, t.gram.flops, t.gram.bytes, t.book);
+    if (t.gram.ops == OPS_BF16) HIP_TRY(launch_gram16_partial(a.data16[b], slabs, C, t.hw, t.plan, c->stream, roi));
+    else if (t.gram.ops == OPS_SPLIT) HIP_TRY(launch_gram_split_partial(a.data[b], slabs, C, t.hw, t.plan, c->stream));
+    else HIP_TRY(launch_gram_partial(a.data[b], slabs, C, t.hw, t.plan, c->stream, roi));
+    return ST_OK;
+}
+
+int style_gram(st_ctx* c, const ActSet& a, const StyleTerm& t, const float* target, float* out, int out_ld, double divisor, float* partial, int* n_partial)
+{
+    if (t.missing32) return missing_copy(t);
+    const int C = t.C;
     ST_TRY(c->gram_slabs.reserve(t.plan.slab_floats));
     ST_TRY(c->gram_fold.reserve((size_t)gram_fold_groups(t.plan) * C * C));
-    {
-        ProfScope ps(c, t.gram.cls, t.gram.flops, t.gram.bytes, t.book);
-        if (t.gram.ops == OPS_BF16) HIP_TRY(launch_gram16_partial(a.data16[b], c->gram_slabs, C, t.hw, t.plan, c->stream, roi));
-        else if (t.gram.ops == OPS_SPLIT) HIP_TRY(launch_gram_split_partial(a.data[b], c->gram_slabs, C, t.hw, t.plan, c->stream));
-        else HIP_TRY(launch_gram_partial(a.data[b], c->gram_slabs, C, t.hw, t.plan, c->stream, roi));
-    }
+    ST_TRY(style_gram_partial(c, a, t, c->gram_slabs));
     ProfScope ps(c, P_GRAM_REDUCE, 0, 4.0 * (double)t.plan.slab_floats, t.book);
     HIP_TRY(launch_gram_reduce(c->gram_slabs, c->gram_fold, target, out, out_ld, partial, n_partial, C, divisor, t.plan, c->stream));
     return ST_OK;
 }
 
-int style_grad(st_ctx* c, const ActSet& a, const StyleTerm& t, float* dst, float c2, int fused, float sw, int accumulate, int* np)
+int style_grad(st_ctx* c, const ActSet& a, const StyleTerm& t, const float* D, float* dst, float c2, int fused, float sw, int accumulate, int* np)
 {
     if (t.missing32) return missing_copy(t);
     const int b = t.b, C = t.C, ld = conv_mpad(C);
@@ -88,9 +94,9 @@
     if (t.grad.ops == OPS_FUSED) {
         ST_TRY(c->sfuse_w[b].reserve(t.sfuse));
         { ProfScope ps(c, t.pack.cls, t.pack.flops, t.pack.bytes, t.book);
-          HIP_TRY(launch_style_fuse_pack(c->dbuf, ld, C, ld, c2, sw, norm, c->sfuse_w[b], c->stream)); }
+          HIP_TRY(launch_style_fuse_pack(D, ld, C, ld, c2, sw, norm, c->sfuse_w[b], c->stream)); }
         ProfScope ps(c, t.grad.cls, t.grad.flops, t.grad.bytes, t.book);
-        HIP_TRY(launch_style_s2_trace(c->dbuf, ld, c->style_gram[b], C, (double)C * t.hw, c2, part, np, c->stream));
+        HIP_TRY(launch_style_s2_trace(D, ld, c->style_gram[b], C, (double)C * t.hw, c2, part, np, c->stream));
         c->sf_in[b] = a.data16[b]; c->sf_w[b] = c->sfuse_w[b];
         return ST_OK;
     }
@@ -99,9 +105,9 @@
         c->inject_roi_zero[b] = 1;
     }
     ProfScope ps(c, t.grad.cls, t.grad.flops, t.grad.bytes, t.book);
-    if (t.grad.ops == OPS_SPLIT) HIP_TRY(launch_style_grad_split(c->dbuf, ld, c->dsplit, a.data[b], dst, c2, fused, sw, norm, accumulate, part, np, C, t.hw, c->stream));
-    else if (t.grad.ops == OPS_BF16) HIP_TRY(launch_style_grad16(c->dbuf, ld, c->d16, a.data16[b], dst, c2, fused, sw, norm, accumulate, part, np, C, (size_t)t.hw, c->stream, t.roi ? &t.groi : nullptr));
-    else HIP_TRY(launch_style_grad(c->dbuf, a.data[b], dst, c2, fused, sw, norm, accumulate, part, np, C, a.h[b], a.w[b], c->stream, t.roi ? &t.proi : nullptr));
+    if (t.grad.ops == OPS_SPLIT) HIP_TRY(launch_style_grad_split(D, ld, c->dsplit, a.data[b], dst, c2, fused, sw, norm, accumulate, part, np, C, t.hw, c->stream));
+    else if (t.grad.ops == OPS_BF16) HIP_TRY(launch_style_grad16(D, ld, c->d16, a.data16[b], dst, c2, fused, sw, norm, accumulate, part, np, C, (size_t)t.hw, c->stream, t.roi ? &t.groi : nullptr));
+    else HIP_TRY(launch_style_grad(D, a.data[b], dst, c2, fused, sw, norm, accumulate, part, np, C, a.h[b], a.w[b], c->stream, t.roi ? &t.proi : nullptr));
     return ST_OK;
 }
 
@@ -112,6 +118,16 @@
     for (int i = 0; i < c->nb; ++i) cc = std::max(cc, (size_t)c->act.C[i] * conv_mpad(c->act.C[i]));
     ST_TRY(c->dbuf.alloc(cc));
     HIP_TRY(hipMemsetAsync(c->dbuf, 0, cc * sizeof(float), c->stream));
+    return ST_OK;
+}
+
+int ensure_dterm(st_ctx* c, int b)
+{
+    if ((int)c->dterm.size() != c->nb) c->dterm.resize(c->nb);
+    if (c->dterm[b]) return ST_OK;
+    const size_t ld = (size_t)conv_mpad(c->act.C[b]);
+    ST_TRY(c->dterm[b].alloc(ld * ld));
+    HIP_TRY(hipMemsetAsync(c->dterm[b], 0, ld * ld * sizeof(float), c->stream));
     return ST_OK;
 }
 
diff --git a/style_transfer2_amd/csrc/engine_tile.cpp b/style_transfer2_amd/csrc/engine_tile.cpp
--- a/style_transfer2_amd/csrc/engine_tile.cpp
+++ b/style_transfer2_amd/csrc/engine_tile.cpp
@@ -190,12 +190,12 @@
                 HIP_TRY(launch_finalize_norm(c->tile.p2 + t.k, 1, t.n_norm, nrm + 1, c->stream));
                 c->norm_valid[b * 3 + 1] = 1;
             }
-            ST_TRY(style_grad(c, a, style_term(c, a, b, t.region()), c->inject[b], c2, 1, al.sw, wrote, &np));
+            ST_TRY(style_grad(c, a, style_term(c, a, b, t.region()), c->dbuf, c->inject[b], c2, 1, al.sw, wrote, &np));
             if (!two_step) {
                 ST_TRY(c->tile.p3.reserve(6 + kMaxTraceLayers));
                 HIP_TRY(launch_sum_partials(c->s2_part[b], np, c->tile.p3 + 6 + t.k, c->stream));
             }
-            c->lt.style_blob = b;
+            c->lt.style_blob = b; c->lt.D = c->dbuf;
             if (c->lt.raw_blob != b) c->lt.raw_blob = -1;
         }
         c->lt.n[b] = t.n; c->lt.C[b] = C; c->lt.diff[b] = LT_WRITTEN;
@@ -216,9 +216,9 @@
         const float c2 = (float)(2.0 / ((double)t.C * t.C * t.n_norm));
         if (!c->stmp) ST_TRY(c->stmp.alloc(c->max_blob));
         int np = 0;
-        ST_TRY(style_grad(c, a, style_term(c, a, t.b, t.region()), c->stmp, c2, 0, t.al.sw, 0, &np));
+        ST_TRY(style_grad(c, a, style_term(c, a, t.b, t.region()), c->dbuf, c->stmp, c2, 0, t.al.sw, 0, &np));
         HIP_TRY(launch_sum_partials(c->s2_part[t.b], np, c->tile.p2 + t.k, c->stream));
-        c->lt.style_blob = c->lt.raw_blob = t.b;
+        c->lt.style_blob = c->lt.raw_blob = t.b; c->lt.D = c->dbuf;
     }
     return ST_OK;
 }
diff --git a/style_transfer2_amd/csrc/gram.hip b/style_transfer2_amd/csrc/gram.hip
--- a/style_transfer2_amd/csrc/gram.hip
+++ b/style_transfer2_amd/csrc/gram.hip
@@ -264,13 +264,12 @@
     return hipGetLastError();
 }
 
-__global__ __launch_bounds__(256) void gram_reduce_k(const float* __restrict__ slabs, const float* __restrict__ target,
-                                                     float* __restrict__ out, float* __restrict__ partial,
-                                                     int cc, int splits, float n, int C, int out_ld, int bt)
-{
-    __shared__ float scratch[4];
+__device__ __forceinline__ void gram_reduce_body(const float* __restrict__ slabs, const float* __restrict__ target,
+                                                 float* __restrict__ out, float* __restrict__ partial,
+                                                 int cc, int splits, float n, int C, int out_ld, int bt, int bid, int nblocks, float* scratch )
+{
     float acc[1] = {0.f};
-    for (int i = blockIdx.x * 256 + threadIdx.x; i < cc; i += gridDim.x * 256) {
+    for (int i = bid * 256 + threadIdx.x; i < cc; i += nblocks * 256) {
         const int r = i / C, c = i - r * C;
         const int tr = r / bt, tc = c / bt;
         if (tr > tc) continue;
@@ -283,7 +282,15 @@
         if (tr < tc) { out[c * out_ld + r] = v; acc[0] += v * v; }
     }
     block_sum(acc, scratch);
-    if (threadIdx.x == 0 && partial) partial[blockIdx.x] = acc[0];
+    if (threadIdx.x == 0 && partial) partial[bid] = acc[0];
+}
+
+__global__ __launch_bounds__(256) void gram_reduce_k(const float* __restrict__ slabs, const float* __restrict__ target,
+                                                     float* __restrict__ out, float* __restrict__ partial,
+                                                     int cc, int splits, float n, int C, int out_ld, int bt)
+{
+    __shared__ float scratch[4];
+    gram_reduce_body(slabs, target, out, partial, cc, splits, n, C, out_ld, bt, blockIdx.x, gridDim.x, scratch);
 }
 
 __global__ __launch_bounds__(256) void gram_fold_k(const float* __restrict__ slabs, float* __restrict__ folded,
@@ -300,16 +307,15 @@
 }
 
 template <int GR_LANES>
-__global__ __launch_bounds__(256) void gram_reduce_wide_k(const float* __restrict__ slabs, const float* __restrict__ target,
-                                                          float* __restrict__ out, float* __restrict__ partial,
-                                                          int cc, int splits, float n, int C, int out_ld, int bt)
+__device__ __forceinline__ void gram_reduce_wide_body(const float* __restrict__ slabs, const float* __restrict__ target,
+                                                      float* __restrict__ out, float* __restrict__ partial,
+                                                      int cc, int splits, float n, int C, int out_ld, int bt, int bid, int nblocks,
+                                                      float4 (*part_s)[256 / GR_LANES] , float* scratch )
 {
     constexpr int GR_QUADS = 256 / GR_LANES, GR_ELEMS = 4 * GR_QUADS;
-    __shared__ float4 part_s[GR_LANES][GR_QUADS];
-    __shared__ float scratch[4];
     const int q = threadIdx.x % GR_QUADS, ln = threadIdx.x / GR_QUADS;
     float acc[1] = {0.f};
-    for (int base = blockIdx.x * GR_ELEMS; base < cc; base += gridDim.x * GR_ELEMS) {
+    for (int base = bid * GR_ELEMS; base < cc; base += nblocks * GR_ELEMS) {
         const int i = base + 4 * q;
         const int r = i < cc ? i / C : 0, c = i < cc ? i - r * C : 0;
         const bool live = i < cc && r / bt <= c / bt;
@@ -338,35 +344,88 @@
         }
     }
     block_sum(acc, scratch);
-    if (threadIdx.x == 0 && partial) partial[blockIdx.x] = acc[0];
+    if (threadIdx.x == 0 && partial) partial[bid] = acc[0];
+}
+
+template <int GR_LANES>
+__global__ __launch_bounds__(256) void gram_reduce_wide_k(const float* __restrict__ slabs, const float* __restrict__ target,
+                                                          float* __restrict__ out, float* __restrict__ partial,
+                                                          int cc, int splits, float n, int C, int out_ld, int bt)
+{
+    __shared__ float4 part_s[GR_LANES][256 / GR_LANES];
+    __shared__ float scratch[4];
+    gram_reduce_wide_body<GR_LANES>(slabs, target, out, partial, cc, splits, n, C, out_ld, bt, blockIdx.x, gridDim.x, part_s, scratch);
+}
+
+__global__ __launch_bounds__(256) void gram_reduce_batch_k(const GramReduceBatch t)
+{
+    __shared__ float4 part_s[256];
+    __shared__ float scratch[4];
+    int e = 0;
+    for (int k = 1; k < t.n; ++k) e += (int)blockIdx.x >= t.e[k].first ? 1 : 0;
+    const GramReduceEntry& g = t.e[e];
+    const int bid = (int)blockIdx.x - g.first;
+    if (g.mode == GRAM_REDUCE_WIDE32)
+        gram_reduce_wide_body<32>(g.slabs, g.target, g.out, g.partial, g.cc, g.splits, g.n, g.C, g.out_ld, g.bt, bid, g.grid, reinterpret_cast<float4(*)[8]>(part_s), scratch);
+    else if (g.mode == GRAM_REDUCE_WIDE8)
+        gram_reduce_wide_body<8>(g.slabs, g.target, g.out, g.partial, g.cc, g.splits, g.n, g.C, g.out_ld, g.bt, bid, g.grid, reinterpret_cast<float4(*)[32]>(part_s), scratch);
+    else
+        gram_reduce_body(g.slabs, g.target, g.out, g.partial, g.cc, g.splits, g.n, g.C, g.out_ld, g.bt, bid, g.grid, scratch);
 }
 
 int gram_fold_groups(const GramPlan& pl) { return pl.splits > 32 ? 32 : 0; }
+
+int gram_reduce_mode(int C, const GramPlan& pl)
+{
+    if (pl.splits > 32 && C % 4 == 0 && pl.bt % 4 == 0 && env_int("ST2_GRAM_REDUCE", 1) != 2)
+        return C * C <= 128 * 128 ? GRAM_REDUCE_WIDE32 : GRAM_REDUCE_WIDE8;
+    return gram_fold_groups(pl) ? GRAM_REDUCE_FOLDED : GRAM_REDUCE_PLAIN;
+}
+
+int gram_reduce_blocks(int C, int mode)
+{
+    const size_t cc = (size_t)C * C;
+    return reduce_grid(cc, mode == GRAM_REDUCE_WIDE32 ? 32 : mode == GRAM_REDUCE_WIDE8 ? 128 : 256, kMaxPartials);
+}
 
 hipError_t launch_gram_reduce(const float* slabs, float* folded, const float* target, float* out, int out_ld, float* partial,
                               int* n_partial, int C, double divisor, const GramPlan& pl, hipStream_t s)
 {
     const int cc = C * C;
     int splits = pl.splits;
-    if (splits > 32 && C % 4 == 0 && pl.bt % 4 == 0 && env_int("ST2_GRAM_REDUCE", 1) != 2) {
-        const bool small = cc <= 128 * 128;
-        const int grid = reduce_grid((size_t)cc, small ? 32 : 128, kMaxPartials);
-        if (n_partial) *n_partial = grid;
-        if (small) gram_reduce_wide_k<32><<<grid, 256, 0, s>>>(slabs, target, out, partial, cc, splits, (float)divisor, C, out_ld, pl.bt);
+    const int mode = gram_reduce_mode(C, pl);
+    const int grid = gram_reduce_blocks(C, mode);
+    if (n_partial) *n_partial = grid;
+    if (mode == GRAM_REDUCE_WIDE32 || mode == GRAM_REDUCE_WIDE8) {
+        if (mode == GRAM_REDUCE_WIDE32) gram_reduce_wide_k<32><<<grid, 256, 0, s>>>(slabs, target, out, partial, cc, splits, (float)divisor, C, out_ld, pl.bt);
         else gram_reduce_wide_k<8><<<grid, 256, 0, s>>>(slabs, target, out, partial, cc, splits, (float)divisor, C, out_ld, pl.bt);
         return hipGetLastError();
     }
-    const int groups = gram_fold_groups(pl);
-    if (groups) {
+    if (mode == GRAM_REDUCE_FOLDED) {
+        const int groups = gram_fold_groups(pl);
         const int per = (pl.splits + groups - 1) / groups;
         gram_fold_k<<<dim3((cc + 255) / 256, groups), 256, 0, s>>>(slabs, folded, cc, pl.splits, per, C, pl.bt);
         slabs = folded;
         splits = (pl.splits + per - 1) / per;
     }
-    const int grid = reduce_grid((size_t)cc, 256, kMaxPartials);
-    if (n_partial) *n_partial = grid;
     gram_reduce_k<<<grid, 256, 0, s>>>(slabs, target, out, partial, cc, splits, (float)divisor, C, out_ld, pl.bt);
     return hipGetLastError();
 }
 
-}
+hipError_t launch_gram_reduce_batch(GramReduceBatch& t, hipStream_t s)
+{
+    if (t.n < 1 || t.n > kMaxGramBatch) return hipErrorInvalidValue;
+    int blocks = 0;
+    for (int k = 0; k < t.n; ++k) {
+        GramReduceEntry& g = t.e[k];
+        if (g.mode != GRAM_REDUCE_PLAIN && g.mode != GRAM_REDUCE_WIDE32 && g.mode != GRAM_REDUCE_WIDE8) return hipErrorInvalidValue;
+        g.cc = g.C * g.C;
+        g.grid = gram_reduce_blocks(g.C, g.mode);
+        g.first = blocks;
+        blocks += g.grid;
+    }
+    gram_reduce_batch_k<<<blocks, 256, 0, s>>>(t);
+    return hipGetLastError();
+}
+
+}
diff --git a/style_transfer2_amd/csrc/passes.hip b/style_transfer2_amd/csrc/passes.hip
--- a/style_transfer2_amd/csrc/passes.hip
+++ b/style_transfer2_amd/csrc/passes.hip
@@ -1,6 +1,7 @@
 #include "st2_kernels.h"
 #include "channel_mean.h"
 #include "wave_reduce.h"
+#include "env.h"
 #include <float.h>
 #include <math.h>
 
@@ -777,9 +778,8 @@
     return hipGetLastError();
 }
 
-__global__ __launch_bounds__(256) void trace_sums_k(const TraceArgs a)
-{
-    __shared__ double scratch[256];
+__device__ __forceinline__ void trace_sums_body(const TraceArgs& a, double* scratch )
+{
     const int slot = blockIdx.x;
     const int nl = a.n_layers * kLayerSlots;
     double v = 0.0;
@@ -793,10 +793,14 @@
     if (threadIdx.x == 0) a.sums[slot] = v;
 }
 
-__global__ void finalize_trace_k(const TraceArgs a)
-{
-    if (threadIdx.x != 0) return;
-    const double* sums = a.sums;
+__global__ __launch_bounds__(256) void trace_sums_k(const TraceArgs a)
+{
+    __shared__ double scratch[256];
+    trace_sums_body(a, scratch);
+}
+
+__device__ __forceinline__ void finalize_trace_body(const TraceArgs& a, const double* sums)
+{
     float loss = 0.f;
     for (int l = 0; l < a.n_layers; ++l) {
         const TraceLayer& L = a.layer[l];
@@ -841,9 +845,40 @@
     g[7] = a.have_grad ? sqrtf((float)(im[5] / a.image_n)) : 0.f;
 }
 
+__global__ void finalize_trace_k(const TraceArgs a)
+{
+    if (threadIdx.x != 0) return;
+    finalize_trace_body(a, a.sums);
+}
+
+__global__ __launch_bounds__(256) void trace_one_k(const TraceArgs a)
+{
+    __shared__ double scratch[256];
+    __shared__ unsigned ticket;
+    trace_sums_body(a, scratch);
+    if (threadIdx.x == 0) {
+        __threadfence();
+        ticket = atomicAdd(a.ticket, 1u);
+    }
+    __syncthreads();
+    if (ticket != gridDim.x - 1) return;
+    __threadfence();
+    const int n = (int)gridDim.x;
+    if ((int)threadIdx.x < n) scratch[threadIdx.x] = __hip_atomic_load(a.sums + threadIdx.x, __ATOMIC_RELAXED, __HIP_MEMORY_SCOPE_AGENT);
+    __syncthreads();
+    if (threadIdx.x != 0) return;
+    *a.ticket = 0u;
+    finalize_trace_body(a, scratch);
+}
+
 hipError_t launch_finalize_trace(const TraceArgs& a, hipStream_t s)
 {
-    trace_sums_k<<<a.n_layers * kLayerSlots + kImageSlots, 256, 0, s>>>(a);
+    const int slots = a.n_layers * kLayerSlots + kImageSlots;
+    if (a.ticket && !env_off("ST2_TRACE_ONE")) {
+        trace_one_k<<<slots, 256, 0, s>>>(a);
+        return hipGetLastError();
+    }
+    trace_sums_k<<<slots, 256, 0, s>>>(a);
     finalize_trace_k<<<1, 64, 0, s>>>(a);
     return hipGetLastError();
 }
diff --git a/style_transfer2_amd/csrc/st2_kernels.h b/style_transfer2_amd/csrc/st2_kernels.h
--- a/style_transfer2_amd/csrc/st2_kernels.h
+++ b/style_transfer2_amd/csrc/st2_kernels.h
@@ -148,6 +148,18 @@
 int gram_fold_groups(const GramPlan& pl);
 hipError_t launch_gram_reduce(const float* slabs, float* folded, const float* target, float* out, int out_ld, float* partial,
                               int* n_partial, int C, double divisor, const GramPlan& pl, hipStream_t s);
+enum GramReduceMode { GRAM_REDUCE_PLAIN, GRAM_REDUCE_WIDE32, GRAM_REDUCE_WIDE8, GRAM_REDUCE_FOLDED };
+int gram_reduce_mode(int C, const GramPlan& pl);
+int gram_reduce_blocks(int C, int mode);
+struct GramReduceEntry {
+    const float* slabs; const float* target; float* out; float* partial;
+    int out_ld, splits, C, bt, mode;
+    float n;
+    int cc, grid, first;
+};
+constexpr int kMaxGramBatch = 24;
+struct GramReduceBatch { int n; GramReduceEntry e[kMaxGramBatch]; };
+hipError_t launch_gram_reduce_batch(GramReduceBatch& t, hipStream_t s);
 
 int style_grad_blocks(int C, int H, int W);
 struct PixRoi { int y0, x0, y1, x1; };
@@ -232,6 +244,8 @@
 constexpr int kMaxTraceLayers = 24;
 constexpr int kLayerSlots = 6;
 constexpr int kImageSlots = 6;
+static_assert(kMaxGramBatch == kMaxTraceLayers, "one Gram reduce entry per layer of the trace");
+constexpr int kTraceSumSlots =kMaxTraceLayers * kLayerSlots + kImageSlots;
 struct TraceLayer {
     int content, style, deepdream;
     float cw, sw, dw;
@@ -251,7 +265,9 @@
     int have_grad;
     float* out;
     double* sums;
-};
+    unsigned* ticket;
+};
+static_assert(kTraceSumSlots <= 256, "the finishing workgroup fetches one slot sum per thread");
 hipError_t launch_finalize_trace(const TraceArgs& a, hipStream_t s);
 
 constexpr int kLbfgsCorr = 10;
```

New measurement: 143.6 it/s (median of 6 runs). Within noise of the previous version (+0.2%).
